# Cappucciyes/ViT-With-OpenCL

Measured on AMD Instinct MI355X. Metric: images/sec ViT-B/16 224x224 bs512, higher is better.
Workload: dtype f32

## Files before the change

### include/kernelHandler.h

```cpp
#ifndef VIT_HIP_KERNELHANDLER_H
#define VIT_HIP_KERNELHANDLER_H

#include <stddef.h>
#include <stdio.h>
#include <stdlib.h>

#ifdef __cplusplus
extern "C" {
#endif

typedef void *vh_stream_t;
typedef void *vh_event_t;

#define VH_CHECK(err)                                                          \
    do {                                                                       \
        int vh_check_err_ = (err);                                             \
        if (vh_check_err_ != 0) {                                              \
            printf("[%s:%d] HIP error %d: %s\n", __FILE__, __LINE__,           \
                   vh_check_err_, vh_last_error());                            \
            exit(EXIT_FAILURE);                                                \
        }                                                                      \
    } while (0)

int vh_device_count(void);
int vh_init(int device);
const char *vh_last_error(void);
int vh_set_error(int code, const char *message);
const char *vh_device_name(void);
int vh_set_device(int device);

int vh_stream_create(vh_stream_t *out);
int vh_stream_destroy(vh_stream_t s);
int vh_stream_sync(vh_stream_t s);
int vh_device_sync(void);

int vh_event_create(vh_event_t *out);
int vh_event_destroy(vh_event_t e);
int vh_event_record(vh_event_t e, vh_stream_t s);
int vh_stream_wait_event(vh_stream_t s, vh_event_t e);
int vh_event_sync(vh_event_t e);
int vh_event_elapsed_ms(float *ms, vh_event_t start, vh_event_t stop);

int vh_malloc(void **out, size_t bytes);
int vh_free(void *p);
int vh_host_alloc(void **out, size_t bytes);
int vh_host_free(void *p);
int vh_memset(void *dst, int value, size_t bytes, vh_stream_t s);
int vh_h2d(void *dst, const void *src, size_t bytes, vh_stream_t s);
int vh_d2h(void *dst, const void *src, size_t bytes, vh_stream_t s);
int vh_d2d(void *dst, const void *src, size_t bytes, vh_stream_t s);


int vh_launch_patch_embed(vh_stream_t s, const float *images, const float *conv_w,
                          const float *conv_b, const float *cls_token, const float *pos_embed,
                          float *tokens, int n_images, int in_chans, int img_size,
                          int patch_size, int embed_dim);

size_t vh_patch_embed_workspace(int n_images, int in_chans, int img_size, int patch_size, int embed_dim);
int vh_launch_patch_embed_ws(vh_stream_t s, const float *images, const float *conv_w,
                             const float *conv_b, const float *cls_token, const float *pos_embed,
                             float *tokens, int n_images, int in_chans, int img_size,
                             int patch_size, int embed_dim, void *workspace, size_t workspace_bytes);

int vh_patch_planes_k(int in_chans, int patch_size);
int vh_launch_conv_weight_planes(vh_stream_t s, const float *conv_w, void *planes, int embed_dim, int in_chans, int patch_size);
int vh_launch_conv_weight_planes_parts(vh_stream_t s, const float *conv_w, void *planes, int embed_dim, int in_chans, int patch_size,
                                       int parts);
int vh_launch_patch_embed_planes3(vh_stream_t s, const float *images, const void *conv_w_planes3, const float *conv_b,
                                  const float *cls_token, const float *pos_embed, float *tokens, int n_images, int in_chans,
                                  int img_size, int patch_size, int embed_dim, void *workspace, size_t workspace_bytes);
int vh_launch_patch_embed_planes(vh_stream_t s, const float *images, const void *conv_w_planes, const float *conv_b,
                                 const float *cls_token, const float *pos_embed, float *tokens, int n_images,
                                 int in_chans, int img_size, int patch_size, int embed_dim, void *workspace,
                                 size_t workspace_bytes);

int vh_launch_layer_norm(vh_stream_t s, const float *input, const float *weight,
                         const float *bias, float *output, int rows, int embed_dim,
                         long in_row_stride, long out_row_stride, double eps);

int vh_launch_linear(vh_stream_t s, float *output, const float *weight, const float *input,
                     const float *bias, int rowA, int colA, int colB, int doGelu,
                     const float *residual);
enum { VH_FP32_SPLIT3 = 0, VH_FP32_NATIVE = 1 };
int vh_launch_linear_math(vh_stream_t s, float *output, const float *weight, const float *input, const float *bias,
                          int rowA, int colA, int colB, int doGelu, const float *residual, int fp32_math);
int vh_launch_patch_embed_ws_math(vh_stream_t s, const float *images, const float *conv_w, const float *conv_b,
                                  const float *cls_token, const float *pos_embed, float *tokens, int n_images, int in_chans,
                                  int img_size, int patch_size, int embed_dim, void *workspace, size_t workspace_bytes,
                                  int fp32_math);

int vh_launch_split3_planes(vh_stream_t s, const float *weight, void *planes, int rows, int cols);
int vh_launch_linear_w3(vh_stream_t s, float *output, const void *weight_planes, const float *input,
                        const float *bias, int rowA, int colA, int colB, int doGelu,
                        const float *residual);

int vh_launch_split3_rows(vh_stream_t s, const float *input, void *planes, int rows, int cols);
int vh_launch_merge3_rows(vh_stream_t s, const void *planes, float *output, int rows, int cols);
int vh_launch_split_rows(vh_stream_t s, const float *input, void *planes, int rows, int cols, int parts);
int vh_launch_merge_rows(vh_stream_t s, const void *planes, float *output, int rows, int cols, int parts);
int vh_layer_norm_planes_max_embed(int parts);
int vh_launch_layer_norm_planes(vh_stream_t s, const float *input, const float *weight, const float *bias,
                                void *out_planes, int parts, int rows, int embed_dim, long in_row_stride, double eps);
int vh_launch_attention_planes_bf16(vh_stream_t s, const float *qkv, void *out_planes, int n_images, int tokens,
                                    int embed_dim, int num_heads);
int vh_launch_linear_planes(vh_stream_t s, void *output, int output_planes, const void *weight_planes,
                            const void *input_planes, int parts, const float *bias, int rowA, int colA, int colB,
                            int doGelu, const float *residual);
int vh_launch_layer_norm_p3(vh_stream_t s, const float *input, const float *weight, const float *bias,
                            void *out_planes, int rows, int embed_dim, long in_row_stride, double eps);
int vh_launch_attention_p3(vh_stream_t s, const float *qkv, void *out_planes, int n_images, int tokens,
                           int embed_dim, int num_heads);
int vh_launch_attention_planes(vh_stream_t s, const void *qkv_planes, void *out_planes, int n_images, int tokens,
                               int embed_dim, int num_heads);
int vh_launch_attention_planes_f16(vh_stream_t s, const void *qkv_planes_f16, void *output, int output_planes,
                                   int n_images, int tokens, int embed_dim, int num_heads);
int vh_launch_attention_planes_f16_hd80(vh_stream_t s, const void *qkv_planes_f16, float *output, int n_images,
                                        int tokens, int embed_dim, int num_heads);
int vh_launch_attention_planes_f16_hd80_operand(vh_stream_t s, const void *qkv_planes_f16, void *output, void *out_scales,
                                                int output_kind, int n_images, int tokens, int embed_dim, int num_heads);
int vh_launch_attention_long(vh_stream_t s, const void *qkv_planes, int parts, float *output, int n_images, int tokens,
                             int embed_dim, int num_heads);
int vh_launch_linear_p3(vh_stream_t s, void *output, int output_planes, const void *weight_planes,
                        const void *input_planes, const float *bias, int rowA, int colA, int colB,
                        int doGelu, const float *residual);

int vh_launch_split2h_planes(vh_stream_t s, const float *weight, void *planes, int rows, int cols, float scale);
int vh_launch_linear_h2(vh_stream_t s, float *output, const void *weight_planes, float weight_scale,
                        const float *input, const float *bias, int rowA, int colA, int colB,
                        int doGelu, const float *residual);
int vh_launch_attention_h2(vh_stream_t s, const float *qkv, float *output, int n_images, int tokens,
                           int embed_dim, int num_heads);

int vh_launch_attention(vh_stream_t s, const float *qkv, float *output, int n_images,
                        int tokens, int embed_dim, int num_heads);
enum { VH_ATTN_NATIVE = 0, VH_ATTN_FP16 = 1, VH_ATTN_FP16X2 = 2, VH_ATTN_SPLIT3 = 3 };
enum { VH_ATTN_AUTO = 0, VH_ATTN_STREAMING = 1 };
int vh_launch_attention_rows(vh_stream_t s, const float *qkv, void *output, int out_kind, int arith, int kernel, int n_images,
                             int tokens, int embed_dim, int num_heads);

int vh_launch_gather_rows(vh_stream_t s, const void *src, void *dst, int n_planes, int src_rows, int dst_rows,
                          int row_bytes, int row_stride);

int vh_launch_softmax(vh_stream_t s, const float *input, float *output, int rows, int length);

enum { VIT_TOPK_PROBS = 0, VIT_TOPK_LOGITS = 1 };
int vh_launch_topk(vh_stream_t s, const float *logits, int rows, int length, int k, int score_kind, int *labels, float *scores);

enum { VH_QKV_ROWS_F32 = 0, VH_QKV_PLANES3 = 1, VH_QKV_PLANES_F16 = 2 };
int vh_cls_attention_head_dim_ok(int head_dim);
int vh_launch_cls_attention(vh_stream_t s, const void *qkv, int qkv_form, int n_images, int tokens, int embed_dim,
                            int num_heads, int tap_index, int n_taps, float *heads, float *mean);

int vh_launch_attention_f16(vh_stream_t s, const float *qkv, float *output, int n_images,
                            int tokens, int embed_dim, int num_heads);

int vh_launch_absmax(vh_stream_t s, const float *input, size_t count, float *amax);

int vh_launch_quantize_mx_rows(vh_stream_t s, const float *input, void *values, void *scales, int rows, int cols);
int vh_launch_quantize_mx_act(vh_stream_t s, const float *input, void *values, void *scales, int rows, int cols);
size_t vh_mx_act_scale_bytes(int rows, int cols);
int vh_launch_layer_norm_mx(vh_stream_t s, const float *input, const float *weight, const float *bias,
                            void *out_values, void *out_scales, int rows, int embed_dim, long in_row_stride, double eps);
int vh_launch_linear_mx(vh_stream_t s, void *output, void *output_scales, const void *weight_values,
                        const void *weight_scales, const void *input_values, const void *input_scales,
                        const float *bias, int rowA, int colA, int colB, int doGelu, const float *residual);
int vh_launch_attention_planes_f16_mx(vh_stream_t s, const void *qkv_planes_f16, void *out_values, void *out_scales,
                                      int n_images, int tokens, int embed_dim, int num_heads);
int vh_launch_linear_mx_planes_f16(vh_stream_t s, void *output_planes_f16, const void *weight_values,
                                   const void *weight_scales, const void *input_values, const void *input_scales,
                                   const float *bias, int rowA, int colA, int colB);

int vh_launch_fold_gamma(vh_stream_t s, const float *weight, const float *gamma, float *out, int out_features, int in_features);
int vh_launch_fold_bias(vh_stream_t s, const float *weight, const float *beta, const float *bias, float *out, int out_features,
                        int in_features);
int vh_launch_colsum_operand(vh_stream_t s, const void *values, const void *scales, float *out, int out_features, int in_features);
int vh_launch_patch_embed_planes_norm(vh_stream_t s, const float *images, const void *conv_w_planes, const float *conv_b,
                                      const float *cls_token, const float *pos_embed, float *tokens, int n_images, int in_chans,
                                      int img_size, int patch_size, int embed_dim, void *workspace, size_t workspace_bytes,
                                      void *operand_out, void *operand_scales_out, float *row_stats_out);
int vh_launch_linear_planes_norm(vh_stream_t s, void *output, int output_planes, const void *weight_planes,
                                 const void *input_planes, const float *row_stats, const float *colsum, const float *bias_folded,
                                 double eps, int rowA, int colA, int colB, int doGelu);
int vh_launch_linear_planes_resid_norm(vh_stream_t s, float *output, const void *weight_planes, const void *input_planes,
                                       const float *bias, const float *residual, int rowA, int colA, int colB,
                                       void *operand_out, void *operand_scales_out, float *row_stats_out);
int vh_launch_colsum_planes3(vh_stream_t s, const void *planes3, float *out, int out_features, int in_features);
int vh_launch_patch_embed_planes3_norm(vh_stream_t s, const float *images, const void *conv_w_planes3, const float *conv_b,
                                       const float *cls_token, const float *pos_embed, float *tokens, int n_images, int in_chans,
                                       int img_size, int patch_size, int embed_dim, void *workspace, size_t workspace_bytes,
                                       void *operand_planes3_out, float *row_stats_out);
int vh_launch_linear_p3_norm(vh_stream_t s, void *output, int output_planes, const void *weight_planes3, const void *input_planes3,
                             const float *row_stats, const float *colsum, const float *bias_folded, double eps, int rowA, int colA,
                             int colB, int doGelu);
int vh_launch_linear_p3_resid_norm(vh_stream_t s, float *output, const void *weight_planes3, const void *input_planes3, const float *bias,
                                   const float *residual, int rowA, int colA, int colB, void *operand_planes3_out, float *row_stats_out);
int vh_launch_linear_mx_norm(vh_stream_t s, void *output, void *output_scales, int output_kind, const void *weight_values,
                             const void *weight_scales, const void *input_values, const void *input_scales, const float *row_stats,
                             const float *colsum, const float *bias_folded, double eps, int rowA, int colA, int colB, int doGelu);
int vh_launch_linear_mx_resid_norm(vh_stream_t s, float *output, const void *weight_values, const void *weight_scales,
                                   const void *input_values, const void *input_scales, const float *bias, const float *residual,
                                   int rowA, int colA, int colB, void *operand_values, void *operand_scales, float *row_stats_out);

int vh_launch_patch_embed_planes_u8(vh_stream_t s, const unsigned char *images, int layout, const float *scale, const float *bias,
                                    const void *conv_w_planes, const float *conv_b, const float *cls_token, const float *pos_embed,
                                    float *tokens, int n_images, int in_chans, int img_size, int patch_size, int embed_dim,
                                    void *workspace, size_t workspace_bytes, int parts, void *operand_out, void *operand_scales_out,
                                    float *row_stats_out);
int vh_launch_expand_u8(vh_stream_t s, const unsigned char *images, int layout, const float *scale, const float *bias, float *out,
                        int n_images, int in_chans, int img_size);

typedef struct vh_resize_desc
{
    const unsigned char *data;
    long row_stride;
    long plane_stride;
    int height, width;
    int row0;
    float x0, x1, y0, y1;
    int out_w, out_h;
    int left, top;
    int kx, ky;
    long coef_offset;
} vh_resize_desc;
#define VH_RESIZE_MAX_ROW_BYTES 3072
int vh_launch_resize_crop_u8(vh_stream_t s, const vh_resize_desc *desc, int n, int chans, int layout, int filter, int crop,
                             void *coef, size_t coef_bytes, unsigned char *out);

size_t vh_feature_readout_scratch(int n_images, int tokens, int embed_dim);
int vh_launch_feature_readout(vh_stream_t s, const float *x, const float *cls_rows, long cls_row_stride, const float *gamma,
                              const float *beta, double eps, int final_norm, int l2_normalize, int dtype, int token_layout,
                              int n_images, int tokens, int embed_dim, int tap_index, int n_taps, void *cls, void *pooled,
                              void *tokens_out, void *scratch, size_t scratch_bytes);

#ifdef __cplusplus
}
#endif

#endif
```

### vit-with-opencl_amd/csrc/ViT_hip.c

```c
#include "ViT_opencl.h"

#include <math.h>
#include <pthread.h>
#include <stddef.h>
#include <stdint.h>
#include <stdio.h>
#include <stdlib.h>
#include <string.h>
#include <time.h>

#define TRY(expr)                 \
    do {                          \
        int try_rc_ = (expr);     \
        if (try_rc_ != 0) {       \
            rc = try_rc_;         \
            goto fail;            \
        }                         \
    } while (0)

struct operand
{
    void *w;
    void *scales;
    float pair_scale;
    float *colsum, *bias_folded;
};

enum { SLAB_F32, SLAB_OPERAND, SLAB_CONV, SLAB_FOLD, N_SLABS };

enum { ATTN_STREAMING, ATTN_HD64, ATTN_HD80, ATTN_LONG };

enum { STREAMING_MAX_TOKENS = 512 };

enum { MAX_DEPTH = 256, MAX_TENSORS = 4 + 12 * MAX_DEPTH + 4 };

enum { DESC_RING = 8, RESIZE_MAX_SIDE = 16384 };

enum { FEAT_NONE, FEAT_DEVICE, FEAT_HOST };

struct staged
{
    void *dev, *pinned[2];
    char *host;
    size_t per_image;
};

struct vit_hip_ctx
{
    vit_config cfg;
    int device;
    int max_batch;
    int tokens;
    int n_tensors;
    vh_stream_t stream;

    int precision;
    int ln_fold;
    int use_p3;
    int cls_only_last;
    int attn_form;
    int fp32_native;
    int attn_rows_streaming;

    void *slab[N_SLABS];
    size_t slab_bytes[N_SLABS];
    float **w;
    struct operand *op;

    float *x;
    float *y;
    float *attn;
    float *qkv;
    float *hid;
    size_t ws_bytes;
    float *stats;
    float *cls;
    float *d_logits;
    float *d_probs;
    float *d_images[2];
    float *h_images[2];
    float *h_logits[2];
    float *h_probs[2];
    vh_stream_t copy_stream;
    vh_event_t up_done[2], comp_done[2], out_done[2];

    size_t crop_off;
    vh_resize_desc *h_desc[DESC_RING];
    vh_resize_desc *d_desc[DESC_RING];
    vh_event_t desc_done[DESC_RING];
    int desc_live[DESC_RING];
    int desc_next;

    struct feature_req
    {
        int form;
        vit_feature_spec spec;
        int layer[4];
        vit_feature_buffers out;
        struct staged st[2];
    } feat;

    struct topk_req
    {
        int form;
        vit_topk_spec spec;
        vit_topk_buffers out;
        struct staged st[2];
    } topk;

    struct attn_req
    {
        int form;
        vit_attn_spec spec;
        int layer[4];
        vit_attn_buffers out;
        struct staged st[2];
    } amap;
    const struct attn_req *attn_serving;

    vh_event_t *prof_ev;
    int *prof_class;
    int prof_cap;
    int prof_used;
    unsigned prof_mask;
};

static int prof_begin(vit_hip_ctx *ctx, vh_stream_t s, int op_class)
{
    if (!ctx->prof_ev || ctx->prof_used >= ctx->prof_cap)
        return -1;
    if (ctx->prof_mask && !(ctx->prof_mask & (1u << op_class)))
        return -1;
    const int slot = ctx->prof_used++;
    ctx->prof_class[slot] = op_class;
    vh_event_record(ctx->prof_ev[2 * slot], s);
    return slot;
}

static void prof_end(vit_hip_ctx *ctx, vh_stream_t s, int slot)
{
    if (slot >= 0)
        vh_event_record(ctx->prof_ev[2 * slot + 1], s);
}

#define OP(op_class, call)                                  \
    do {                                                    \
        const int op_slot_ = prof_begin(ctx, s, op_class);  \
        TRY(call);                                          \
        prof_end(ctx, s, op_slot_);                         \
    } while (0)

static void prof_release(vit_hip_ctx *ctx)
{
    if (ctx->prof_ev) {
        for (int i = 0; i < 2 * ctx->prof_cap; ++i)
            if (ctx->prof_ev[i])
                vh_event_destroy(ctx->prof_ev[i]);
        free(ctx->prof_ev);
        free(ctx->prof_class);
    }
    ctx->prof_ev = NULL;
    ctx->prof_class = NULL;
    ctx->prof_cap = ctx->prof_used = 0;
}

static double wall_seconds(void)
{
    struct timespec ts;
    clock_gettime(CLOCK_MONOTONIC, &ts);
    return (double)ts.tv_sec + 1e-9 * (double)ts.tv_nsec;
}

static size_t align_up(size_t v, size_t a) { return (v + a - 1) / a * a; }

const vit_config *vit_hip_config(const vit_hip_ctx *ctx) { return &ctx->cfg; }
int vit_hip_device(const vit_hip_ctx *ctx) { return ctx->device; }
float *vit_hip_logits_buffer(vit_hip_ctx *ctx) { return ctx->d_logits; }
vh_stream_t vit_hip_stream(const vit_hip_ctx *ctx) { return ctx->stream; }
int vit_hip_max_batch(const vit_hip_ctx *ctx) { return ctx->max_batch; }
const float *vit_hip_weight(const vit_hip_ctx *ctx, int idx)
{
    return (idx >= 0 && idx < ctx->n_tensors) ? ctx->w[idx] : NULL;
}

static int staged_alloc(const vit_hip_ctx *ctx, struct staged *st)
{
    const size_t bytes = (size_t)ctx->max_batch * st->per_image;
    int rc = vh_malloc(&st->dev, bytes);
    for (int slot = 0; slot < 2 && rc == 0; ++slot)
        rc = vh_host_alloc(&st->pinned[slot], bytes);
    return rc;
}

static void staged_release(struct staged *st)
{
    if (st->dev) vh_free(st->dev);
    st->dev = NULL;
    for (int slot = 0; slot < 2; ++slot) {
        if (st->pinned[slot]) vh_host_free(st->pinned[slot]);
        st->pinned[slot] = NULL;
    }
}

static int staged_d2h(const vit_hip_ctx *ctx, const struct staged *st, int slot, int m)
{
    return vh_d2h(st->pinned[slot], st->dev, (size_t)m * st->per_image, ctx->stream);
}

static void staged_scatter(const struct staged *st, int slot, int first, int m)
{
    memcpy(st->host + (size_t)first * st->per_image, st->pinned[slot], (size_t)m * st->per_image);
}

static void request_release(struct staged st[2])
{
    staged_release(&st[0]);
    staged_release(&st[1]);
}

void vit_hip_destroy(vit_hip_ctx *ctx)
{
    if (!ctx)
        return;
    if (ctx->stream) {
        vh_set_device(ctx->device);
        vh_stream_sync(ctx->stream);
    }
    prof_release(ctx);
    request_release(ctx->feat.st);
    request_release(ctx->topk.st);
    request_release(ctx->amap.st);
    for (int i = 0; i < N_SLABS; ++i)
        if (ctx->slab[i])
            vh_free(ctx->slab[i]);
    float *dev[] = {ctx->x, ctx->y, ctx->attn, ctx->qkv, ctx->hid, ctx->stats,
                    ctx->cls, ctx->d_logits, ctx->d_probs, ctx->d_images[0], ctx->d_images[1]};
    for (size_t i = 0; i < sizeof(dev) / sizeof(dev[0]); ++i)
        if (dev[i])
            vh_free(dev[i]);
    float *host[] = {ctx->h_images[0], ctx->h_images[1], ctx->h_logits[0], ctx->h_logits[1],
                     ctx->h_probs[0], ctx->h_probs[1]};
    for (size_t i = 0; i < sizeof(host) / sizeof(host[0]); ++i)
        if (host[i])
            vh_host_free(host[i]);
    for (int i = 0; i < DESC_RING; ++i) {
        if (ctx->d_desc[i]) vh_free(ctx->d_desc[i]);
        if (ctx->h_desc[i]) vh_host_free(ctx->h_desc[i]);
        if (ctx->desc_done[i]) vh_event_destroy(ctx->desc_done[i]);
    }
    for (int i = 0; i < 2; ++i) {
        if (ctx->up_done[i]) vh_event_destroy(ctx->up_done[i]);
        if (ctx->comp_done[i]) vh_event_destroy(ctx->comp_done[i]);
        if (ctx->out_done[i]) vh_event_destroy(ctx->out_done[i]);
    }
    if (ctx->copy_stream)
        vh_stream_destroy(ctx->copy_stream);
    if (ctx->stream)
        vh_stream_destroy(ctx->stream);
    free(ctx->w);
    free(ctx->op);
    free(ctx);
}

static const int BIG[4] = {2, 4, 8, 10};

static float **layer_tensors(const vit_hip_ctx *ctx, int l) { return ctx->w + 4 + 12 * l; }

static int operand_tensor(int m) { return 4 + 12 * (m / 4) + BIG[m % 4]; }

static void *place(void *slab, size_t *off, size_t bytes)
{
    void *p = slab ? (char *)slab + *off : NULL;
    *off += align_up(bytes, 256);
    return p;
}

static void layout_weights(vit_hip_ctx *ctx, size_t bytes[N_SLABS])
{
    const vit_config *cfg = &ctx->cfg;
    const int p = ctx->precision;
    const int f32_planes = p == VIT_PRECISION_F32 && cfg->embed_dim % 128 == 0 && cfg->mlp_hidden % 128 == 0;
    const size_t per = p == VIT_PRECISION_BF16_GEMM ? 2 : p == VIT_PRECISION_FP8_GEMM ? 1 : p == VIT_PRECISION_F32_FP16X2 ? 4
                     : f32_planes ? 6 : 0;
    const size_t conv_parts = (p == VIT_PRECISION_BF16_GEMM || p == VIT_PRECISION_FP8_GEMM) ? 1 : f32_planes ? 3 : 0;
    size_t off[N_SLABS] = {0};
    for (int i = 0; i < ctx->n_tensors; ++i)
        ctx->w[i] = (float *)place(ctx->slab[SLAB_F32], &off[SLAB_F32], vit_config_tensor_size(cfg, i) * sizeof(float));
    for (int m = 0; m < 4 * cfg->depth; ++m) {
        struct operand *o = &ctx->op[m];
        const size_t cnt = vit_config_tensor_size(cfg, operand_tensor(m));
        o->w = place(ctx->slab[SLAB_OPERAND], &off[SLAB_OPERAND], cnt * per);
        if (p == VIT_PRECISION_FP8_GEMM)
            o->scales = place(ctx->slab[SLAB_OPERAND], &off[SLAB_OPERAND], cnt / 32);
    }
    place(ctx->slab[SLAB_CONV], &off[SLAB_CONV],
          (size_t)vh_patch_planes_k(cfg->in_chans, cfg->patch_size) * (size_t)cfg->embed_dim * 2 * conv_parts);
    for (int m = 0; ctx->ln_fold && m < 4 * cfg->depth; m += 2) {
        const size_t nb = vit_config_tensor_size(cfg, operand_tensor(m) + 1) * sizeof(float);
        ctx->op[m].colsum = (float *)place(ctx->slab[SLAB_FOLD], &off[SLAB_FOLD], nb);
        ctx->op[m].bias_folded = (float *)place(ctx->slab[SLAB_FOLD], &off[SLAB_FOLD], nb);
    }
    memcpy(bytes, off, sizeof(off));
}

static int alloc_weights(vit_hip_ctx *ctx)
{
    int rc = 0;
    layout_weights(ctx, ctx->slab_bytes);
    for (int i = 0; i < N_SLABS; ++i)
        if (ctx->slab_bytes[i])
            TRY(vh_malloc(&ctx->slab[i], ctx->slab_bytes[i]));
    layout_weights(ctx, ctx->slab_bytes);
    return 0;
fail:
    return rc;
}

static int fill_weights(vit_hip_ctx *ctx, const Network *networks)
{
    int rc = 0;
    const vit_config *cfg = &ctx->cfg;
    const int p = ctx->precision;
    float *d_amax = NULL, *d_scaled = NULL;
    for (int i = 0; i < ctx->n_tensors; ++i)
        TRY(vh_h2d(ctx->w[i], networks[i].data, networks[i].size * sizeof(float), ctx->stream));
    if (p == VIT_PRECISION_F32_FP16X2)
        TRY(vh_malloc((void **)&d_amax, sizeof(float)));
    if (ctx->ln_fold)
        TRY(vh_malloc((void **)&d_scaled, (size_t)cfg->embed_dim * (size_t)(cfg->mlp_hidden > 3 * cfg->embed_dim ? cfg->mlp_hidden : 3 * cfg->embed_dim) * sizeof(float)));
    for (int m = 0; m < 4 * cfg->depth; ++m) {
        struct operand *o = &ctx->op[m];
        float **lw = layer_tensors(ctx, m / 4);
        const int idx = operand_tensor(m), k = m % 4, fold = o->colsum != NULL;
        const int out_f = (int)networks[idx + 1].size, in_f = (int)(networks[idx].size / networks[idx + 1].size);
        const float *src = ctx->w[idx];
        if (fold) {
            TRY(vh_launch_fold_gamma(ctx->stream, ctx->w[idx], lw[k == 0 ? 0 : 6], d_scaled, out_f, in_f));
            src = d_scaled;
        }
        switch (p) {
        case VIT_PRECISION_BF16_GEMM:
            TRY(vh_launch_split_rows(ctx->stream, src, o->w, out_f, in_f, 1));
            break;
        case VIT_PRECISION_FP8_GEMM:
            TRY(vh_launch_quantize_mx_rows(ctx->stream, src, o->w, o->scales, out_f, in_f));
            break;
        case VIT_PRECISION_F32:
            if (o->w)
                TRY(vh_launch_split3_planes(ctx->stream, src, o->w, out_f, in_f));
            break;
        case VIT_PRECISION_F32_FP16X2: {
            float amax = 0.0f;
            TRY(vh_memset(d_amax, 0, sizeof(float), ctx->stream));
            TRY(vh_launch_absmax(ctx->stream, src, networks[idx].size, d_amax));
            TRY(vh_d2h(&amax, d_amax, sizeof(float), ctx->stream));
            TRY(vh_stream_sync(ctx->stream));
            int e = 0;
            o->pair_scale = 1.0f;
            if (amax > 0.0f && amax < 3.0e38f) {
                (void)frexpf(amax, &e);
                o->pair_scale = ldexpf(1.0f, 14 - e);
            }
            TRY(vh_launch_split2h_planes(ctx->stream, src, o->w, out_f, in_f, o->pair_scale));
            break;
        }
        }
        if (fold) {
            TRY(p == VIT_PRECISION_F32 ? vh_launch_colsum_planes3(ctx->stream, o->w, o->colsum, out_f, in_f)
                                       : vh_launch_colsum_operand(ctx->stream, o->w, o->scales, o->colsum, out_f, in_f));
            TRY(vh_launch_fold_bias(ctx->stream, ctx->w[idx], lw[k == 0 ? 1 : 7], ctx->w[idx + 1], o->bias_folded, out_f, in_f));
        }
    }
    if (d_scaled)
        TRY(vh_stream_sync(ctx->stream));
    if (ctx->slab[SLAB_CONV])
        TRY(vh_launch_conv_weight_planes_parts(ctx->stream, ctx->w[1], ctx->slab[SLAB_CONV], cfg->embed_dim, cfg->in_chans,
                                               cfg->patch_size, p == VIT_PRECISION_F32 ? 3 : 1));
fail:
    if (d_amax)
        vh_free(d_amax);
    if (d_scaled)
        vh_free(d_scaled);
    return rc;
}

static int alloc_arena(vit_hip_ctx *ctx);

static int env_precision(void)
{
    const char *env = getenv("VIT_HIP_PRECISION");
    return (env && env[0] == 'b') ? VIT_PRECISION_BF16_GEMM
         : (env && strncmp(env, "fp16x2", 6) == 0) ? VIT_PRECISION_F32_FP16X2
         : (env && strncmp(env, "fp8", 3) == 0) ? VIT_PRECISION_FP8_GEMM : VIT_PRECISION_F32;
}

int vit_hip_create(vit_hip_ctx **out, const vit_config *cfg, const Network *networks,
                   int n_tensors, int device, int max_batch)
{
    return vit_hip_create_ex(out, cfg, networks, n_tensors, device, max_batch, env_precision());
}

int vit_hip_precision(const vit_hip_ctx *ctx) { return ctx->precision; }
int vit_hip_ln_fold(const vit_hip_ctx *ctx) { return ctx ? ctx->ln_fold : 0; }

static int ctx_new(vit_hip_ctx **out, const vit_config *cfg, int n_tensors, int device, int max_batch, int precision, int ln_fold)
{
    if (!out)
        return 1;
    *out = NULL;
    if (!cfg || max_batch <= 0)
        return 1;
    if (precision != VIT_PRECISION_F32 && precision != VIT_PRECISION_BF16_GEMM && precision != VIT_PRECISION_FP8_GEMM &&
        precision != VIT_PRECISION_F32_FP16X2)
        return 1;
    if (precision == VIT_PRECISION_F32_FP16X2 && (cfg->embed_dim % 128 != 0 || cfg->mlp_hidden % 128 != 0))
        return 2;
    if (precision == VIT_PRECISION_FP8_GEMM && (cfg->embed_dim % 256 != 0 || cfg->mlp_hidden % 256 != 0))
        return 2;
    if (precision == VIT_PRECISION_BF16_GEMM && (cfg->embed_dim % 128 != 0 || cfg->mlp_hidden % 128 != 0))
        return 2;
    if (cfg->depth <= 0 || cfg->embed_dim <= 0 || cfg->num_heads <= 0 || cfg->patch_size <= 0 || cfg->img_size <= 0 ||
        cfg->in_chans <= 0 || cfg->num_classes <= 0 || cfg->mlp_hidden <= 0)
        return 2;
    if (cfg->depth > MAX_DEPTH || cfg->embed_dim > 16384 || cfg->mlp_hidden > 65536 || cfg->img_size > 4096 || cfg->in_chans > 64 ||
        cfg->num_classes > (1 << 20) || cfg->num_heads > 1024 || max_batch > (1 << 20))
        return 2;
    if (n_tensors != vit_config_num_tensors(cfg))
        return 2;
    if (cfg->embed_dim % cfg->num_heads != 0 || cfg->img_size % cfg->patch_size != 0)
        return 2;

    const int E = cfg->embed_dim, F = cfg->mlp_hidden, H = cfg->num_heads, T = vit_config_tokens(cfg);
    const int reduced = precision == VIT_PRECISION_BF16_GEMM || precision == VIT_PRECISION_FP8_GEMM;
    const char *env_p3 = getenv("VIT_HIP_P3"), *env_native = getenv("VIT_HIP_GEMM_FP32");
    const int fp32_native = env_native && env_native[0] == 'n';
    const int planes_wanted = !(env_p3 && env_p3[0] == '0') && !fp32_native;
    const int use_p3 = precision == VIT_PRECISION_F32 && E % 128 == 0 && F % 128 == 0 && planes_wanted &&
                       (size_t)max_batch * (size_t)T * 64 <= 0xffffffffull;
    const int fold_fits = E % 128 == 0 && E / 128 <= 16 && (reduced || (precision == VIT_PRECISION_F32 && F % 128 == 0));
    if (ln_fold < 0) {
        const char *env = getenv("VIT_HIP_LN_FOLD");
        ln_fold = fold_fits && (reduced ? !(env && env[0] == '0') : env && env[0] == '1' && planes_wanted);
    }
    if (ln_fold && (!fold_fits || (precision == VIT_PRECISION_F32 && !use_p3)))
        return vh_set_error(2, "vit_hip_create: this shape, precision and batch cannot fold the LayerNorms (the fp32 path "
                               "needs the planes path)");
    if (use_p3 && !ln_fold && E > vh_layer_norm_planes_max_embed(3)) {
        char msg[320];
        snprintf(msg, sizeof msg, "vit_hip_create: embed_dim=%d: the fp32 planes path's LayerNorm (three-part planes, 96 bytes of "
                 "LDS per column) takes a LayerNorm width of at most %d",
                 E, vh_layer_norm_planes_max_embed(3));
        return vh_set_error(2, msg);
    }
    const char *env_ll = getenv("VIT_HIP_LAST_LAYER");
    const char *env_attn = getenv("VIT_HIP_ATTN");
    const int long_hd = E == 64 * H || E == 80 * H;
    const int long_wanted = T > STREAMING_MAX_TOKENS || (env_attn && strcmp(env_attn, "long") == 0);
    if (T > STREAMING_MAX_TOKENS && (precision == VIT_PRECISION_F32_FP16X2 || (precision == VIT_PRECISION_F32 && !use_p3) || !long_hd)) {
        char msg[320];
        snprintf(msg, sizeof msg, "vit_hip_create: %d tokens: above %d tokens attention runs on the planes paths (F32 with "
                 "embed_dim and mlp_hidden multiples of 128 and neither $VIT_HIP_P3=0 nor $VIT_HIP_GEMM_FP32=native, BF16_GEMM, "
                 "FP8_GEMM; not F32_FP16X2) with head_dim 64 or 80 (precision %d, head_dim %d)",
                 T, STREAMING_MAX_TOKENS, precision, E / H);
        return vh_set_error(2, msg);
    }

    vit_hip_ctx *ctx = (vit_hip_ctx *)calloc(1, sizeof(*ctx));
    if (!ctx)
        return 4;
    ctx->cfg = *cfg;
    ctx->device = device;
    ctx->max_batch = max_batch;
    ctx->tokens = T;
    ctx->n_tensors = n_tensors;
    ctx->precision = precision;
    ctx->ln_fold = ln_fold ? 1 : 0;
    ctx->use_p3 = use_p3;
    ctx->cls_only_last = use_p3 && !ln_fold && env_ll && strcmp(env_ll, "cls") == 0;
    ctx->attn_form = !(use_p3 || reduced) ? ATTN_STREAMING
              : (long_wanted && long_hd) ? ATTN_LONG
              : (E == 64 * H && T <= 208) ? ATTN_HD64
              : (reduced && E == 80 * H && T <= 272) ? ATTN_HD80 : ATTN_STREAMING;
    ctx->fp32_native = fp32_native;
    ctx->attn_rows_streaming = env_attn && env_attn[0] == 't';
    ctx->w = (float **)calloc((size_t)n_tensors, sizeof(float *));
    ctx->op = (struct operand *)calloc((size_t)4 * cfg->depth, sizeof(struct operand));
    if (!ctx->w || !ctx->op) {
        free(ctx->w);
        free(ctx->op);
        free(ctx);
        return 4;
    }
    *out = ctx;
    return 0;
}

int vit_hip_create_ex(vit_hip_ctx **out, const vit_config *cfg, const Network *networks,
                      int n_tensors, int device, int max_batch, int precision)
{
    int rc = 0;
    if (!out)
        return 1;
    *out = NULL;
    if (!networks || !cfg)
        return 1;
    if (n_tensors != vit_config_num_tensors(cfg))
        return 2;
    for (int i = 0; i < n_tensors; ++i)
        if (!networks[i].data || networks[i].size != vit_config_tensor_size(cfg, i)) {
            fprintf(stderr, "vit_hip_create: tensor %d has %zu elements, expected %zu\n", i,
                    networks[i].data ? networks[i].size : (size_t)0, vit_config_tensor_size(cfg, i));
            return 3;
        }
    vit_hip_ctx *ctx = NULL;
    if ((rc = ctx_new(&ctx, cfg, n_tensors, device, max_batch, precision, -1)) != 0)
        return rc;
    TRY(vh_init(device));
    TRY(vh_stream_create(&ctx->stream));
    TRY(alloc_weights(ctx));
    TRY(fill_weights(ctx, networks));
    TRY(alloc_arena(ctx));
    *out = ctx;
    return 0;
fail:
    vit_hip_destroy(ctx);
    return rc;
}

#define VIT_PLANES_LAYOUT_VERSION 2

struct planes_header
{
    char magic[8];
    unsigned header_bytes;
    int precision, n_tensors;
    int cfg_ints[8];
    double eps;
    unsigned long long w_slab_bytes, planes_bytes, wconv16_bytes, scale_floats;
    unsigned long long fold_bytes;
    int ln_fold, layout_version;
    unsigned long long checksum;
};

static unsigned long long planes_hash(unsigned long long h, const void *data, size_t bytes)
{
    const unsigned long long *w = (const unsigned long long *)data;
    for (size_t i = 0; i < bytes / 8; ++i)
        h = (h ^ w[i]) * 0x100000001b3ull;
    const unsigned char *t = (const unsigned char *)data + (bytes & ~(size_t)7);
    for (size_t i = 0; i < (bytes & 7); ++i)
        h = (h ^ t[i]) * 0x100000001b3ull;
    return h;
}
#define PLANES_HASH_SEED 0xcbf29ce484222325ull

static int copy_file_and_device(vit_hip_ctx *ctx, FILE *fp, void *dev, size_t bytes, int to_file, unsigned long long *hash)
{
    enum { CHUNK = 64 << 20 };
    int rc = 0;
    void *host = NULL;
    if (bytes == 0)
        return 0;
    TRY(vh_host_alloc(&host, bytes < CHUNK ? bytes : (size_t)CHUNK));
    for (size_t off = 0; off < bytes && rc == 0; off += CHUNK) {
        const size_t n = bytes - off < CHUNK ? bytes - off : (size_t)CHUNK;
        if (to_file) {
            if ((rc = vh_d2h(host, (char *)dev + off, n, ctx->stream)) != 0 || (rc = vh_stream_sync(ctx->stream)) != 0)
                break;
            *hash = planes_hash(*hash, host, n);
            if (fwrite(host, 1, n, fp) != n)
                rc = vh_set_error(120, "vit_hip_export_planes: short write");
        } else {
            if (fread(host, 1, n, fp) != n) {
                rc = vh_set_error(121, "vit_hip_create_from_planes: file is shorter than its header says");
                break;
            }
            *hash = planes_hash(*hash, host, n);
            if ((rc = vh_h2d((char *)dev + off, host, n, ctx->stream)) != 0 || (rc = vh_stream_sync(ctx->stream)) != 0)
                break;
        }
    }
fail:
    if (host)
        vh_host_free(host);
    return rc;
}

static void pair_scales(const vit_hip_ctx *ctx, float scales[MAX_TENSORS])
{
    memset(scales, 0, sizeof(float) * (size_t)ctx->n_tensors);
    for (int m = 0; m < 4 * ctx->cfg.depth; ++m)
        scales[operand_tensor(m)] = ctx->op[m].pair_scale;
}

int vit_hip_export_planes(vit_hip_ctx *ctx, const char *path)
{
    int rc = 0;
    if (!ctx || !path)
        return vh_set_error(1, "vit_hip_export_planes: null argument");
    TRY(vh_set_device(ctx->device));
    const size_t plen = strlen(path);
    char *tmp = (char *)malloc(plen + 5);
    if (!tmp)
        return vh_set_error(4, "vit_hip_export_planes: out of host memory");
    memcpy(tmp, path, plen);
    memcpy(tmp + plen, ".tmp", 5);
    FILE *fp = fopen(tmp, "wb");
    if (!fp) {
        free(tmp);
        return vh_set_error(122, "vit_hip_export_planes: cannot open the file for writing");
    }
    struct planes_header h;
    memset(&h, 0, sizeof(h));
    memcpy(h.magic, "VITPLN02", 8);
    h.header_bytes = (unsigned)sizeof(h);
    h.precision = ctx->precision;
    h.n_tensors = ctx->n_tensors;
    const vit_config *c = &ctx->cfg;
    const int ints[8] = {c->img_size, c->patch_size, c->in_chans, c->num_classes, c->embed_dim, c->depth, c->num_heads, c->mlp_hidden};
    memcpy(h.cfg_ints, ints, sizeof(ints));
    h.eps = c->eps;
    h.w_slab_bytes = ctx->slab_bytes[SLAB_F32];
    h.planes_bytes = ctx->slab_bytes[SLAB_OPERAND];
    h.wconv16_bytes = ctx->slab_bytes[SLAB_CONV];
    h.fold_bytes = ctx->slab_bytes[SLAB_FOLD];
    h.ln_fold = ctx->ln_fold;
    h.layout_version = VIT_PLANES_LAYOUT_VERSION;
    h.scale_floats = (unsigned long long)ctx->n_tensors;
    float scales[MAX_TENSORS];
    pair_scales(ctx, scales);
    unsigned long long hash = planes_hash(PLANES_HASH_SEED, scales, sizeof(float) * (size_t)ctx->n_tensors);
    if (fwrite(&h, sizeof(h), 1, fp) != 1 || fwrite(scales, sizeof(float), (size_t)ctx->n_tensors, fp) != (size_t)ctx->n_tensors)
        rc = vh_set_error(120, "vit_hip_export_planes: short write");
    for (int i = 0; i < N_SLABS && rc == 0; ++i)
        rc = copy_file_and_device(ctx, fp, ctx->slab[i], ctx->slab_bytes[i], 1, &hash);
    if (rc == 0) {
        h.checksum = hash;
        if (fseek(fp, 0, SEEK_SET) != 0 || fwrite(&h, sizeof(h), 1, fp) != 1)
            rc = vh_set_error(120, "vit_hip_export_planes: short write");
    }
    if (fclose(fp) != 0 && rc == 0)
        rc = vh_set_error(120, "vit_hip_export_planes: short write");
    if (rc == 0 && rename(tmp, path) != 0)
        rc = vh_set_error(122, "vit_hip_export_planes: cannot move the finished file into place");
    if (rc != 0)
        remove(tmp);
    free(tmp);
    return rc;
fail:
    return rc;
}

int vit_hip_create_from_planes(vit_hip_ctx **out, const char *path, int device, int max_batch)
{
    int rc = 0;
    if (!out)
        return 1;
    *out = NULL;
    if (!path)
        return vh_set_error(1, "vit_hip_create_from_planes: null path");
    FILE *fp = fopen(path, "rb");
    if (!fp)
        return vh_set_error(123, "vit_hip_create_from_planes: cannot open the file");
    struct planes_header h;
    vit_hip_ctx *ctx = NULL;
    if (fread(&h, sizeof(h), 1, fp) != 1 || memcmp(h.magic, "VITPLN02", 8) != 0 || h.header_bytes != sizeof(h) ||
        h.layout_version != VIT_PLANES_LAYOUT_VERSION) {
        fclose(fp);
        return vh_set_error(124, "vit_hip_create_from_planes: not a planes file of this library version (magic, header size or operand-layout version)");
    }
    vit_config cfg = {h.cfg_ints[0], h.cfg_ints[1], h.cfg_ints[2], h.cfg_ints[3], h.cfg_ints[4], h.cfg_ints[5], h.cfg_ints[6],
                      h.cfg_ints[7], h.eps};
    if (h.n_tensors <= 0 || h.n_tensors > MAX_TENSORS ||
        (rc = ctx_new(&ctx, &cfg, h.n_tensors, device, max_batch, h.precision, h.ln_fold ? 1 : 0)) != 0) {
        fclose(fp);
        return vh_set_error(rc ? rc : 2, "vit_hip_create_from_planes: the header's model shape or precision is not one this library takes");
    }
    size_t sizes[N_SLABS];
    layout_weights(ctx, sizes);
    if (h.w_slab_bytes != sizes[SLAB_F32] || h.planes_bytes != sizes[SLAB_OPERAND] || h.wconv16_bytes != sizes[SLAB_CONV] ||
        h.fold_bytes != sizes[SLAB_FOLD] || h.scale_floats != (unsigned long long)ctx->n_tensors) {
        rc = vh_set_error(125, "vit_hip_create_from_planes: slab sizes in the file do not match this library's layout");
        goto fail;
    }
    float scales[MAX_TENSORS];
    if (fread(scales, sizeof(float), (size_t)ctx->n_tensors, fp) != (size_t)ctx->n_tensors) {
        rc = vh_set_error(124, "vit_hip_create_from_planes: truncated header");
        goto fail;
    }
    unsigned long long hash = planes_hash(PLANES_HASH_SEED, scales, sizeof(float) * (size_t)ctx->n_tensors);
    for (int m = 0; m < 4 * cfg.depth; ++m)
        ctx->op[m].pair_scale = scales[operand_tensor(m)];
    TRY(vh_init(device));
    TRY(vh_stream_create(&ctx->stream));
    TRY(alloc_weights(ctx));
    for (int i = 0; i < N_SLABS; ++i)
        TRY(copy_file_and_device(ctx, fp, ctx->slab[i], ctx->slab_bytes[i], 0, &hash));
    if (hash != h.checksum) {
        rc = vh_set_error(126, "vit_hip_create_from_planes: payload checksum mismatch (corrupt file)");
        goto fail;
    }
    TRY(alloc_arena(ctx));
    fclose(fp);
    *out = ctx;
    return 0;
fail:
    fclose(fp);
    vit_hip_destroy(ctx);
    return rc;
}

static int planes_patch_embed(const vit_hip_ctx *ctx)
{
    return ctx->ln_fold || ctx->use_p3 || ctx->precision == VIT_PRECISION_BF16_GEMM || ctx->precision == VIT_PRECISION_FP8_GEMM;
}

static int span_taps(float in0, float in1, int out, int filter)
{
    const double scale = (double)(in1 - in0) / out;
    const double support = (filter == VIT_RESIZE_BICUBIC ? 2.0 : 1.0) * (scale < 1.0 ? 1.0 : scale);
    return (int)ceil(support) * 2 + 1;
}

static int resize_taps(int in, int out, int filter)
{
    return span_taps(0.0f, (float)in, out, filter);
}

static int resize_max_taps(int crop)
{
    return resize_taps(RESIZE_MAX_SIDE, crop > 1 ? crop - 1 : 1, VIT_RESIZE_BICUBIC);
}

static size_t resize_table_bytes(int crop, int kx, int ky)
{
    return align_up((size_t)crop * 16 + ((size_t)kx + ky) * crop * 4, 16);
}

static int alloc_arena(vit_hip_ctx *ctx)
{
    int rc = 0;
    const vit_config *cfg = &ctx->cfg;
    const int precision = ctx->precision, max_batch = ctx->max_batch;
    const size_t E = (size_t)cfg->embed_dim, F = (size_t)cfg->mlp_hidden, NC = (size_t)cfg->num_classes;
    const size_t rows = (size_t)max_batch * ctx->tokens;
    const size_t img = (size_t)cfg->in_chans * cfg->img_size * cfg->img_size;
    const size_t act = ctx->use_p3 ? 6 : sizeof(float);
    TRY(vh_malloc((void **)&ctx->x, rows * E * sizeof(float)));
    TRY(vh_malloc((void **)&ctx->y, rows * E * act));
    TRY(vh_malloc((void **)&ctx->attn, rows * E * act));
    {
        const size_t qkv_bytes = rows * 3 * E * act, expanded = planes_patch_embed(ctx) ? 0 : (size_t)max_batch * img * sizeof(float);
        ctx->crop_off = align_up(expanded, 256);
        const size_t crops = cfg->in_chans <= 4 ? ctx->crop_off + (size_t)max_batch * img : 0;
        size_t bytes = qkv_bytes > expanded ? qkv_bytes : expanded;
        bytes = bytes > crops ? bytes : crops;
        TRY(vh_malloc((void **)&ctx->qkv, bytes));
    }
    {
        size_t ws = vh_patch_embed_workspace(max_batch, cfg->in_chans, cfg->img_size, cfg->patch_size, cfg->embed_dim);
        if (ctx->slab[SLAB_CONV]) {
            const size_t grid = (size_t)(cfg->img_size / cfg->patch_size);
            const size_t planes = (size_t)max_batch * grid * grid * (size_t)vh_patch_planes_k(cfg->in_chans, cfg->patch_size) * 2 *
                                  (precision == VIT_PRECISION_F32 ? 3 : 1);
            ws = ws > planes ? ws : planes;
        }
        const size_t hid_bytes = rows * F * act;
        if (cfg->in_chans <= 4) {
            const size_t tables = (size_t)max_batch * resize_table_bytes(cfg->img_size, resize_max_taps(cfg->img_size),
                                                                          resize_max_taps(cfg->img_size));
            ws = ws > tables ? ws : tables;
        }
        ctx->ws_bytes = ws > hid_bytes ? ws : hid_bytes;
        TRY(vh_malloc((void **)&ctx->hid, ctx->ws_bytes));
    }
    if (ctx->ln_fold)
        TRY(vh_malloc((void **)&ctx->stats, rows * (E / 128) * 2 * sizeof(float)));
    TRY(vh_malloc((void **)&ctx->cls, (size_t)max_batch * E * sizeof(float)));
    TRY(vh_malloc((void **)&ctx->d_logits, (size_t)max_batch * NC * sizeof(float)));
    TRY(vh_malloc((void **)&ctx->d_probs, (size_t)max_batch * NC * sizeof(float)));
    TRY(vh_stream_create(&ctx->copy_stream));
    for (int i = 0; i < 2; ++i) {
        TRY(vh_malloc((void **)&ctx->d_images[i], (size_t)max_batch * img * sizeof(float)));
        TRY(vh_host_alloc((void **)&ctx->h_images[i], (size_t)max_batch * img * sizeof(float)));
        TRY(vh_host_alloc((void **)&ctx->h_logits[i], (size_t)max_batch * NC * sizeof(float)));
        TRY(vh_host_alloc((void **)&ctx->h_probs[i], (size_t)max_batch * NC * sizeof(float)));
        TRY(vh_event_create(&ctx->up_done[i]));
        TRY(vh_event_create(&ctx->comp_done[i]));
        TRY(vh_event_create(&ctx->out_done[i]));
    }
    for (int i = 0; i < DESC_RING; ++i) {
        TRY(vh_malloc((void **)&ctx->d_desc[i], (size_t)max_batch * sizeof(vh_resize_desc)));
        TRY(vh_host_alloc((void **)&ctx->h_desc[i], (size_t)max_batch * sizeof(vh_resize_desc)));
        TRY(vh_event_create(&ctx->desc_done[i]));
    }
    TRY(vh_stream_sync(ctx->stream));
    return 0;
fail:
    return rc;
}


static int fp32_math(const vit_hip_ctx *ctx) { return ctx->fp32_native ? VH_FP32_NATIVE : VH_FP32_SPLIT3; }

static int attention_rows(const vit_hip_ctx *ctx, vh_stream_t s, float *out, int arith, int n)
{
    return vh_launch_attention_rows(s, ctx->qkv, out, 0, arith, ctx->attn_rows_streaming ? VH_ATTN_STREAMING : VH_ATTN_AUTO, n,
                                    ctx->tokens, ctx->cfg.embed_dim, ctx->cfg.num_heads);
}

static int attention_tap(vit_hip_ctx *ctx, vh_stream_t s, int n, int l)
{
    int rc = 0;
    const struct attn_req *ar = ctx->attn_serving;
    if (!ar)
        return 0;
    const vit_config *c = &ctx->cfg;
    const int reduced = ctx->precision == VIT_PRECISION_BF16_GEMM || ctx->precision == VIT_PRECISION_FP8_GEMM;
    const int form = reduced ? (ctx->attn_form == ATTN_STREAMING ? VH_QKV_ROWS_F32 : VH_QKV_PLANES_F16)
                   : ctx->precision == VIT_PRECISION_F32 && ctx->use_p3 && (ctx->attn_form == ATTN_HD64 || ctx->attn_form == ATTN_LONG)
                       ? VH_QKV_PLANES3 : VH_QKV_ROWS_F32;
    for (int k = 0; k < ar->spec.n_taps; ++k)
        if (ar->layer[k] == l)
            OP(VIT_OP_ATTENTION, vh_launch_cls_attention(s, ctx->qkv, form, n, ctx->tokens, c->embed_dim, c->num_heads, k,
                                                         ar->spec.n_taps, ar->out.heads, ar->out.mean));
    return 0;
fail:
    return rc;
}

static int attention_reduced(vit_hip_ctx *ctx, vh_stream_t s, int n, char *attn_scales)
{
    int rc = 0;
    const vit_config *c = &ctx->cfg;
    const int E = c->embed_dim, T = ctx->tokens, H = c->num_heads, rows = n * T;
    if (ctx->attn_form == ATTN_HD64)
        OP(VIT_OP_ATTENTION, attn_scales ? vh_launch_attention_planes_f16_mx(s, ctx->qkv, ctx->attn, attn_scales, n, T, E, H)
                                         : vh_launch_attention_planes_f16(s, ctx->qkv, ctx->attn, 1, n, T, E, H));
    else if (ctx->attn_form == ATTN_HD80)
        OP(VIT_OP_ATTENTION, vh_launch_attention_planes_f16_hd80_operand(s, ctx->qkv, ctx->attn, attn_scales, attn_scales ? 2 : 1, n, T, E, H));
    else if (ctx->attn_form == ATTN_LONG)
        OP(VIT_OP_ATTENTION, (rc = vh_launch_attention_long(s, ctx->qkv, 1, ctx->hid, n, T, E, H)) != 0 ? rc :
                             attn_scales ? vh_launch_quantize_mx_act(s, ctx->hid, ctx->attn, attn_scales, rows, E)
                                         : vh_launch_split_rows(s, ctx->hid, ctx->attn, rows, E, 1));
    else
        OP(VIT_OP_ATTENTION, (rc = attention_rows(ctx, s, ctx->hid, VH_ATTN_FP16, n)) != 0 ? rc :
                             attn_scales ? vh_launch_quantize_mx_act(s, ctx->hid, ctx->attn, attn_scales, rows, E)
                                         : vh_launch_split_rows(s, ctx->hid, ctx->attn, rows, E, 1));
    return 0;
fail:
    return rc;
}

static int layer_fp8(vit_hip_ctx *ctx, vh_stream_t s, int n, int l)
{
    int rc = 0;
    const vit_config *c = &ctx->cfg;
    const int E = c->embed_dim, F = c->mlp_hidden, rows = n * ctx->tokens, fold = ctx->ln_fold, last = l == c->depth - 1;
    float **lw = layer_tensors(ctx, l);
    const struct operand *op = ctx->op + 4 * l;
    char *ys = (char *)ctx->y + align_up((size_t)rows * E, 256), *as_ = (char *)ctx->attn + align_up((size_t)rows * E, 256);
    char *hs = (char *)ctx->hid + align_up((size_t)rows * F, 256);
    const int kind = ctx->attn_form == ATTN_STREAMING ? 0 : 2;
    if (!fold)
        OP(VIT_OP_LAYER_NORM, vh_launch_layer_norm_mx(s, ctx->x, lw[0], lw[1], ctx->y, ys, rows, E, E, c->eps));
    OP(VIT_OP_QKV, fold ? vh_launch_linear_mx_norm(s, ctx->qkv, NULL, kind, op[0].w, op[0].scales, ctx->y, ys, ctx->stats, op[0].colsum, op[0].bias_folded, c->eps, rows, E, 3 * E, 0)
                 : kind ? vh_launch_linear_mx_planes_f16(s, ctx->qkv, op[0].w, op[0].scales, ctx->y, ys, lw[3], rows, E, 3 * E)
                        : vh_launch_linear_mx(s, ctx->qkv, NULL, op[0].w, op[0].scales, ctx->y, ys, lw[3], rows, E, 3 * E, 0, NULL));
    TRY(attention_tap(ctx, s, n, l));
    TRY(attention_reduced(ctx, s, n, as_));
    OP(VIT_OP_OUT_PROJ, fold ? vh_launch_linear_mx_resid_norm(s, ctx->x, op[1].w, op[1].scales, ctx->attn, as_, lw[5], ctx->x, rows, E, E, ctx->y, ys, ctx->stats)
                             : vh_launch_linear_mx(s, ctx->x, NULL, op[1].w, op[1].scales, ctx->attn, as_, lw[5], rows, E, E, 0, ctx->x));
    if (!fold)
        OP(VIT_OP_LAYER_NORM, vh_launch_layer_norm_mx(s, ctx->x, lw[6], lw[7], ctx->y, ys, rows, E, E, c->eps));
    OP(VIT_OP_FC1, fold ? vh_launch_linear_mx_norm(s, ctx->hid, hs, 1, op[2].w, op[2].scales, ctx->y, ys, ctx->stats, op[2].colsum, op[2].bias_folded, c->eps, rows, E, F, 1)
                        : vh_launch_linear_mx(s, ctx->hid, hs, op[2].w, op[2].scales, ctx->y, ys, lw[9], rows, E, F, 1, NULL));
    OP(VIT_OP_FC2, fold && !last ? vh_launch_linear_mx_resid_norm(s, ctx->x, op[3].w, op[3].scales, ctx->hid, hs, lw[11], ctx->x, rows, F, E, ctx->y, ys, ctx->stats)
                                 : vh_launch_linear_mx(s, ctx->x, NULL, op[3].w, op[3].scales, ctx->hid, hs, lw[11], rows, F, E, 0, ctx->x));
    return 0;
fail:
    return rc;
}

static int layer_bf16(vit_hip_ctx *ctx, vh_stream_t s, int n, int l)
{
    int rc = 0;
    const vit_config *c = &ctx->cfg;
    const int E = c->embed_dim, F = c->mlp_hidden, rows = n * ctx->tokens, fold = ctx->ln_fold, last = l == c->depth - 1;
    float **lw = layer_tensors(ctx, l);
    const struct operand *op = ctx->op + 4 * l;
    const int kind = ctx->attn_form == ATTN_STREAMING ? 0 : 2;
    if (!fold)
        OP(VIT_OP_LAYER_NORM, vh_launch_layer_norm_planes(s, ctx->x, lw[0], lw[1], ctx->y, 1, rows, E, E, c->eps));
    OP(VIT_OP_QKV, fold ? vh_launch_linear_planes_norm(s, ctx->qkv, kind, op[0].w, ctx->y, ctx->stats, op[0].colsum, op[0].bias_folded, c->eps, rows, E, 3 * E, 0)
                        : vh_launch_linear_planes(s, ctx->qkv, kind, op[0].w, ctx->y, 1, lw[3], rows, E, 3 * E, 0, NULL));
    TRY(attention_tap(ctx, s, n, l));
    TRY(attention_reduced(ctx, s, n, NULL));
    OP(VIT_OP_OUT_PROJ, fold ? vh_launch_linear_planes_resid_norm(s, ctx->x, op[1].w, ctx->attn, lw[5], ctx->x, rows, E, E, ctx->y, NULL, ctx->stats)
                             : vh_launch_linear_planes(s, ctx->x, 0, op[1].w, ctx->attn, 1, lw[5], rows, E, E, 0, ctx->x));
    if (!fold)
        OP(VIT_OP_LAYER_NORM, vh_launch_layer_norm_planes(s, ctx->x, lw[6], lw[7], ctx->y, 1, rows, E, E, c->eps));
    OP(VIT_OP_FC1, fold ? vh_launch_linear_planes_norm(s, ctx->hid, 1, op[2].w, ctx->y, ctx->stats, op[2].colsum, op[2].bias_folded, c->eps, rows, E, F, 1)
                        : vh_launch_linear_planes(s, ctx->hid, 1, op[2].w, ctx->y, 1, lw[9], rows, E, F, 1, NULL));
    OP(VIT_OP_FC2, fold && !last ? vh_launch_linear_planes_resid_norm(s, ctx->x, op[3].w, ctx->hid, lw[11], ctx->x, rows, F, E, ctx->y, NULL, ctx->stats)
                                 : vh_launch_linear_planes(s, ctx->x, 0, op[3].w, ctx->hid, 1, lw[11], rows, F, E, 0, ctx->x));
    return 0;
fail:
    return rc;
}

static int layer_fp16x2(vit_hip_ctx *ctx, vh_stream_t s, int n, int l)
{
    int rc = 0;
    const vit_config *c = &ctx->cfg;
    const int E = c->embed_dim, F = c->mlp_hidden, T = ctx->tokens, rows = n * T;
    float **lw = layer_tensors(ctx, l);
    const struct operand *op = ctx->op + 4 * l;
    OP(VIT_OP_LAYER_NORM, vh_launch_layer_norm(s, ctx->x, lw[0], lw[1], ctx->y, rows, E, E, E, c->eps));
    OP(VIT_OP_QKV, vh_launch_linear_h2(s, ctx->qkv, op[0].w, op[0].pair_scale, ctx->y, lw[3], rows, E, 3 * E, 0, NULL));
    TRY(attention_tap(ctx, s, n, l));
    OP(VIT_OP_ATTENTION, attention_rows(ctx, s, ctx->attn, VH_ATTN_FP16X2, n));
    OP(VIT_OP_OUT_PROJ, vh_launch_linear_h2(s, ctx->x, op[1].w, op[1].pair_scale, ctx->attn, lw[5], rows, E, E, 0, ctx->x));
    OP(VIT_OP_LAYER_NORM, vh_launch_layer_norm(s, ctx->x, lw[6], lw[7], ctx->y, rows, E, E, E, c->eps));
    OP(VIT_OP_FC1, vh_launch_linear_h2(s, ctx->hid, op[2].w, op[2].pair_scale, ctx->y, lw[9], rows, E, F, 1, NULL));
    OP(VIT_OP_FC2, vh_launch_linear_h2(s, ctx->x, op[3].w, op[3].pair_scale, ctx->hid, lw[11], rows, F, E, 0, ctx->x));
    return 0;
fail:
    return rc;
}

static int layer_f32_planes(vit_hip_ctx *ctx, vh_stream_t s, int n, int l, int *cls_rows)
{
    int rc = 0;
    const vit_config *c = &ctx->cfg;
    const int E = c->embed_dim, F = c->mlp_hidden, T = ctx->tokens, rows = n * T, fold = ctx->ln_fold, last = l == c->depth - 1;
    float **lw = layer_tensors(ctx, l);
    const struct operand *op = ctx->op + 4 * l;
    const int planes_attn = ctx->attn_form == ATTN_HD64 || ctx->attn_form == ATTN_LONG;
    if (!fold)
        OP(VIT_OP_LAYER_NORM, vh_launch_layer_norm_p3(s, ctx->x, lw[0], lw[1], ctx->y, rows, E, E, c->eps));
    OP(VIT_OP_QKV, fold ? vh_launch_linear_p3_norm(s, ctx->qkv, planes_attn, op[0].w, ctx->y, ctx->stats, op[0].colsum, op[0].bias_folded, c->eps, rows, E, 3 * E, 0)
                        : vh_launch_linear_p3(s, ctx->qkv, planes_attn, op[0].w, ctx->y, lw[3], rows, E, 3 * E, 0, NULL));
    TRY(attention_tap(ctx, s, n, l));
    OP(VIT_OP_ATTENTION, ctx->attn_form == ATTN_HD64 ? vh_launch_attention_planes(s, ctx->qkv, ctx->attn, n, T, E, c->num_heads)
                         : (rc = ctx->attn_form == ATTN_LONG ? vh_launch_attention_long(s, ctx->qkv, 3, ctx->hid, n, T, E, c->num_heads)
                                                             : attention_rows(ctx, s, ctx->hid, VH_ATTN_SPLIT3, n)) != 0 ? rc
                         : vh_launch_split3_rows(s, ctx->hid, ctx->attn, rows, E));
    if (last && ctx->cls_only_last && T >= 4) {
        char *scratch = (char *)ctx->qkv;
        float *x_cls = (float *)scratch;
        char *attn_cls = scratch + align_up((size_t)n * E * 4, 256);
        char *y_cls = attn_cls + align_up((size_t)n * E * 6, 256);
        char *hid_cls = y_cls + align_up((size_t)n * E * 6, 256);
        OP(VIT_OP_OUT_PROJ, (rc = vh_launch_gather_rows(s, ctx->attn, attn_cls, 3 * (E / 32), rows, n, 64, T)) != 0 ? rc :
                            (rc = vh_launch_gather_rows(s, ctx->x, x_cls, 1, rows, n, 4 * E, T)) != 0 ? rc :
                            vh_launch_linear_p3(s, x_cls, 0, op[1].w, attn_cls, lw[5], n, E, E, 0, x_cls));
        OP(VIT_OP_LAYER_NORM, vh_launch_layer_norm_p3(s, x_cls, lw[6], lw[7], y_cls, n, E, E, c->eps));
        OP(VIT_OP_FC1, vh_launch_linear_p3(s, hid_cls, 1, op[2].w, y_cls, lw[9], n, E, F, 1, NULL));
        OP(VIT_OP_FC2, vh_launch_linear_p3(s, x_cls, 0, op[3].w, hid_cls, lw[11], n, F, E, 0, x_cls));
        *cls_rows = 1;
        return 0;
    }
    OP(VIT_OP_OUT_PROJ, fold ? vh_launch_linear_p3_resid_norm(s, ctx->x, op[1].w, ctx->attn, lw[5], ctx->x, rows, E, E, ctx->y, ctx->stats)
                             : vh_launch_linear_p3(s, ctx->x, 0, op[1].w, ctx->attn, lw[5], rows, E, E, 0, ctx->x));
    if (!fold)
        OP(VIT_OP_LAYER_NORM, vh_launch_layer_norm_p3(s, ctx->x, lw[6], lw[7], ctx->y, rows, E, E, c->eps));
    OP(VIT_OP_FC1, fold ? vh_launch_linear_p3_norm(s, ctx->hid, 1, op[2].w, ctx->y, ctx->stats, op[2].colsum, op[2].bias_folded, c->eps, rows, E, F, 1)
                        : vh_launch_linear_p3(s, ctx->hid, 1, op[2].w, ctx->y, lw[9], rows, E, F, 1, NULL));
    OP(VIT_OP_FC2, fold && !last ? vh_launch_linear_p3_resid_norm(s, ctx->x, op[3].w, ctx->hid, lw[11], ctx->x, rows, F, E, ctx->y, ctx->stats)
                                 : vh_launch_linear_p3(s, ctx->x, 0, op[3].w, ctx->hid, lw[11], rows, F, E, 0, ctx->x));
    return 0;
fail:
    return rc;
}

static int layer_f32_rows(vit_hip_ctx *ctx, vh_stream_t s, int n, int l)
{
    int rc = 0;
    const vit_config *c = &ctx->cfg;
    const int E = c->embed_dim, F = c->mlp_hidden, T = ctx->tokens, rows = n * T;
    float **lw = layer_tensors(ctx, l);
    const struct operand *op = ctx->op + 4 * l;
    const int math = fp32_math(ctx);
    OP(VIT_OP_LAYER_NORM, vh_launch_layer_norm(s, ctx->x, lw[0], lw[1], ctx->y, rows, E, E, E, c->eps));
    OP(VIT_OP_QKV, op[0].w ? vh_launch_linear_w3(s, ctx->qkv, op[0].w, ctx->y, lw[3], rows, E, 3 * E, 0, NULL)
                         : vh_launch_linear_math(s, ctx->qkv, lw[2], ctx->y, lw[3], rows, E, 3 * E, 0, NULL, math));
    TRY(attention_tap(ctx, s, n, l));
    OP(VIT_OP_ATTENTION, attention_rows(ctx, s, ctx->attn, ctx->fp32_native ? VH_ATTN_NATIVE : VH_ATTN_SPLIT3, n));
    OP(VIT_OP_OUT_PROJ, op[1].w ? vh_launch_linear_w3(s, ctx->x, op[1].w, ctx->attn, lw[5], rows, E, E, 0, ctx->x)
                              : vh_launch_linear_math(s, ctx->x, lw[4], ctx->attn, lw[5], rows, E, E, 0, ctx->x, math));
    OP(VIT_OP_LAYER_NORM, vh_launch_layer_norm(s, ctx->x, lw[6], lw[7], ctx->y, rows, E, E, E, c->eps));
    OP(VIT_OP_FC1, op[2].w ? vh_launch_linear_w3(s, ctx->hid, op[2].w, ctx->y, lw[9], rows, E, F, 1, NULL)
                         : vh_launch_linear_math(s, ctx->hid, lw[8], ctx->y, lw[9], rows, E, F, 1, NULL, math));
    OP(VIT_OP_FC2, op[3].w ? vh_launch_linear_w3(s, ctx->x, op[3].w, ctx->hid, lw[11], rows, F, E, 0, ctx->x)
                          : vh_launch_linear_math(s, ctx->x, lw[10], ctx->hid, lw[11], rows, F, E, 0, ctx->x, math));
    return 0;
fail:
    return rc;
}

struct row_origin
{
    int row0;
    long plane_stride;
};

struct pixel_src
{
    const float *f32;
    const unsigned char *u8;
    int layout;
    const vit_pixel_norm *norm;
    const vit_image_u8 *resize;
    const vit_resize_crop *rc;
    const vit_box_u8 *boxes;
    int filter;
    const struct row_origin *origin;
};

static int resize_crop_launch(vit_hip_ctx *ctx, vh_stream_t s, const struct pixel_src *src, int n, unsigned char *out)
{
    int rc_ = 0;
    const vit_config *c = &ctx->cfg;
    const int layout = src->layout, filter = src->boxes ? src->filter : src->rc->filter;
    const int S = c->img_size, C = c->in_chans, slot = ctx->desc_next;
    ctx->desc_next = (slot + 1) % DESC_RING;
    if (ctx->desc_live[slot] && (rc_ = vh_event_sync(ctx->desc_done[slot])) != 0)
        return rc_;
    ctx->desc_live[slot] = 0;
    vh_resize_desc *d = ctx->h_desc[slot];
    size_t off = 0;
    for (int i = 0; i < n; ++i) {
        const int which = src->boxes ? src->boxes[i].image : i;
        const vit_image_u8 *im = &src->resize[which];
        vh_resize_desc *e = &d[i];
        e->data = im->data;
        e->row_stride = im->row_stride;
        e->plane_stride = src->origin ? src->origin[which].plane_stride : (long)im->height * im->row_stride;
        e->height = im->height;
        e->width = im->width;
        e->row0 = src->origin ? src->origin[which].row0 : 0;
        if (src->boxes) {
            const float *b = src->boxes[i].box;
            e->x0 = b[0], e->y0 = b[1], e->x1 = b[2], e->y1 = b[3];
            e->out_w = e->out_h = S;
            e->left = e->top = 0;
        } else {
            vit_resize_crop_geometry(im->height, im->width, src->rc, S, &e->out_h, &e->out_w, &e->top, &e->left);
            e->x0 = e->y0 = 0.0f;
            e->x1 = (float)im->width, e->y1 = (float)im->height;
        }
        e->kx = span_taps(e->x0, e->x1, e->out_w, filter);
        e->ky = span_taps(e->y0, e->y1, e->out_h, filter);
        e->coef_offset = (long)off;
        off += resize_table_bytes(S, e->kx, e->ky);
    }
    if (off > ctx->ws_bytes)
        return vh_set_error(1, "resize: coefficient tables exceed the scratch");
    if ((rc_ = vh_h2d(ctx->d_desc[slot], d, (size_t)n * sizeof(*d), s)) != 0)
        return rc_;
    rc_ = vh_launch_resize_crop_u8(s, ctx->d_desc[slot], n, C, layout, filter, S, ctx->hid, ctx->ws_bytes, out);
    const int rec = vh_event_record(ctx->desc_done[slot], s);
    ctx->desc_live[slot] = rec == 0;
    return rc_ ? rc_ : rec;
}

static int patch_embed_launches(vit_hip_ctx *ctx, vh_stream_t s, const struct pixel_src *src, int n)
{
    const vit_config *c = &ctx->cfg;
    const int E = c->embed_dim;
    float **w = ctx->w;
    void *conv = ctx->slab[SLAB_CONV];
    const int reduced = ctx->precision == VIT_PRECISION_BF16_GEMM || ctx->precision == VIT_PRECISION_FP8_GEMM;
    char *const y_scales = ctx->precision == VIT_PRECISION_FP8_GEMM ? (char *)ctx->y + align_up((size_t)n * ctx->tokens * E, 256) : NULL;
    if (src->u8 && planes_patch_embed(ctx))
        return vh_launch_patch_embed_planes_u8(s, src->u8, src->layout, src->norm->scale, src->norm->bias, conv, w[2], w[0], w[3],
                                               ctx->x, n, c->in_chans, c->img_size, c->patch_size, E, ctx->hid, ctx->ws_bytes,
                                               ctx->precision == VIT_PRECISION_F32 ? 3 : 1, ctx->ln_fold ? ctx->y : NULL,
                                               ctx->ln_fold ? y_scales : NULL, ctx->ln_fold ? ctx->stats : NULL);
    const float *images = src->f32;
    if (src->u8) {
        const int rc = vh_launch_expand_u8(s, src->u8, src->layout, src->norm->scale, src->norm->bias, ctx->qkv, n, c->in_chans,
                                           c->img_size);
        if (rc)
            return rc;
        images = ctx->qkv;
    }
    if (ctx->ln_fold && ctx->precision == VIT_PRECISION_F32)
        return vh_launch_patch_embed_planes3_norm(s, images, conv, w[2], w[0], w[3], ctx->x, n, c->in_chans, c->img_size,
                                                  c->patch_size, E, ctx->hid, ctx->ws_bytes, ctx->y, ctx->stats);
    if (ctx->ln_fold)
        return vh_launch_patch_embed_planes_norm(s, images, conv, w[2], w[0], w[3], ctx->x, n, c->in_chans, c->img_size,
                                                 c->patch_size, E, ctx->hid, ctx->ws_bytes, ctx->y, y_scales, ctx->stats);
    if (reduced)
        return vh_launch_patch_embed_planes(s, images, conv, w[2], w[0], w[3], ctx->x, n, c->in_chans, c->img_size, c->patch_size,
                                            E, ctx->hid, ctx->ws_bytes);
    if (ctx->use_p3)
        return vh_launch_patch_embed_planes3(s, images, conv, w[2], w[0], w[3], ctx->x, n, c->in_chans, c->img_size, c->patch_size,
                                             E, ctx->hid, ctx->ws_bytes);
    return vh_launch_patch_embed_ws_math(s, images, w[1], w[2], w[0], w[3], ctx->x, n, c->in_chans, c->img_size, c->patch_size, E,
                                         ctx->hid, ctx->ws_bytes, fp32_math(ctx));
}

static int feature_tap(vit_hip_ctx *ctx, vh_stream_t s, const struct feature_req *fr, int k, int n, int cls_rows)
{
    int rc = 0;
    const vit_config *c = &ctx->cfg;
    float **tw = ctx->w + 4 + 12 * c->depth;
    OP(VIT_OP_LAYER_NORM, vh_launch_feature_readout(s, ctx->x, cls_rows ? (const float *)ctx->qkv : NULL, c->embed_dim, tw[0], tw[1],
                                                    c->eps, fr->spec.final_norm, fr->spec.l2_normalize, fr->spec.dtype,
                                                    fr->spec.token_layout, n, ctx->tokens, c->embed_dim, k, fr->spec.n_taps,
                                                    fr->out.cls, fr->out.pooled, fr->out.tokens, ctx->hid, ctx->ws_bytes));
    return 0;
fail:
    return rc;
}

static int forward_device(vit_hip_ctx *ctx, const struct pixel_src *src, int n, float *d_logits, float *d_probs, vh_stream_t stream,
                          const struct feature_req *fr, const struct topk_req *tk, const struct attn_req *ar)
{
    int rc = 0;
    const int cls_only_saved = ctx->cls_only_last;
    ctx->attn_serving = ar;
    TRY(vh_set_device(ctx->device));
    const vit_config *c = &ctx->cfg;
    const int E = c->embed_dim, T = ctx->tokens, NC = c->num_classes;
    vh_stream_t s = stream ? stream : ctx->stream;

    struct pixel_src crops;
    if (src->resize) {
        unsigned char *out = (unsigned char *)ctx->qkv + ctx->crop_off;
        OP(VIT_OP_PATCH_EMBED, resize_crop_launch(ctx, s, src, n, out));
        crops = (struct pixel_src){NULL, out, VIT_PIXELS_HWC, src->norm, NULL, NULL};
        src = &crops;
    }
    OP(VIT_OP_PATCH_EMBED, patch_embed_launches(ctx, s, src, n));
    int cls_rows = 0;
    if (fr && fr->layer[fr->spec.n_taps - 1] == c->depth - 1 && (fr->out.pooled || fr->out.tokens))
        ctx->cls_only_last = 0;
    for (int l = 0, k = 0; l < c->depth; ++l) {
        switch (ctx->precision) {
        case VIT_PRECISION_FP8_GEMM: TRY(layer_fp8(ctx, s, n, l)); break;
        case VIT_PRECISION_BF16_GEMM: TRY(layer_bf16(ctx, s, n, l)); break;
        case VIT_PRECISION_F32_FP16X2: TRY(layer_fp16x2(ctx, s, n, l)); break;
        default:
            if (ctx->use_p3)
                TRY(layer_f32_planes(ctx, s, n, l, &cls_rows));
            else
                TRY(layer_f32_rows(ctx, s, n, l));
        }
        if (fr && k < fr->spec.n_taps && fr->layer[k] == l)
            TRY(feature_tap(ctx, s, fr, k++, n, cls_rows));
    }
    ctx->cls_only_last = cls_only_saved;
    ctx->attn_serving = NULL;

    float **tw = ctx->w + 4 + 12 * c->depth;
    float *logits = d_logits ? d_logits : ctx->d_logits;
    const float *final_x = cls_rows ? (const float *)ctx->qkv : ctx->x;
    const long final_stride = cls_rows ? (long)E : (long)T * E;
    OP(VIT_OP_LAYER_NORM, vh_launch_layer_norm(s, final_x, tw[0], tw[1], ctx->cls, n, E, final_stride, E, c->eps));
    OP(VIT_OP_HEAD, vh_launch_linear_math(s, logits, tw[2], ctx->cls, tw[3], n, E, NC, 0, NULL, fp32_math(ctx)));
    if (d_probs)
        OP(VIT_OP_SOFTMAX, vh_launch_softmax(s, logits, d_probs, n, NC));
    if (tk)
        OP(VIT_OP_SOFTMAX, vh_launch_topk(s, logits, n, NC, tk->spec.k, tk->spec.score_kind, tk->out.labels, tk->out.scores));
    return 0;
fail:
    ctx->cls_only_last = cls_only_saved;
    ctx->attn_serving = NULL;
    return rc;
}

static int armed_requests(vit_hip_ctx *ctx, const char *who, int form, const struct feature_req **fr, const struct topk_req **tk,
                          const struct attn_req **ar)
{
    static const char *const what[3] = {"feature", "top-k", "attention"}, *const setter[3] = {"features", "topk", "attention"};
    const int armed[3] = {ctx->feat.form, ctx->topk.form, ctx->amap.form};
    *fr = NULL;
    *tk = NULL;
    *ar = NULL;
    if (form == FEAT_NONE)
        return 0;
    for (int r = 0; r < 3; ++r)
        if (armed[r] != FEAT_NONE && armed[r] != form) {
            char msg[200];
            const char *const is = armed[r] == FEAT_HOST ? "host" : "device";
            snprintf(msg, sizeof msg, "%s: the context is armed for %s %s buffers (vit_hip_set_%s%s); disarm it or use the %s forms", who, is,
                     what[r], setter[r], armed[r] == FEAT_HOST ? "_host" : "", is);
            return vh_set_error(1, msg);
        }
    *fr = armed[0] == form ? &ctx->feat : NULL;
    *tk = armed[1] == form ? &ctx->topk : NULL;
    *ar = armed[2] == form ? &ctx->amap : NULL;
    return 0;
}

static int forward_device_armed(vit_hip_ctx *ctx, const char *who, const struct pixel_src *src, int n, float *d_logits, float *d_probs,
                                vh_stream_t stream)
{
    const struct feature_req *fr;
    const struct topk_req *tk;
    const struct attn_req *ar;
    if (armed_requests(ctx, who, FEAT_DEVICE, &fr, &tk, &ar))
        return 1;
    return forward_device(ctx, src, n, d_logits, d_probs, stream, fr, tk, ar);
}

int vit_hip_forward_device_plain(vit_hip_ctx *ctx, const float *d_images, int n, float *d_logits, float *d_probs, vh_stream_t stream)
{
    if (!ctx || !d_images || n <= 0 || n > ctx->max_batch)
        return 1;
    const struct pixel_src src = {d_images, NULL, 0, NULL};
    return forward_device(ctx, &src, n, d_logits, d_probs, stream, NULL, NULL, NULL);
}

int vit_hip_forward_device(vit_hip_ctx *ctx, const float *d_images, int n, float *d_logits,
                           float *d_probs, vh_stream_t stream)
{
    if (!ctx || !d_images || n <= 0 || n > ctx->max_batch)
        return 1;
    const struct pixel_src src = {d_images, NULL, 0, NULL};
    return forward_device_armed(ctx, "vit_hip_forward_device", &src, n, d_logits, d_probs, stream);
}

int vit_pixel_norm_from_mean_std(vit_pixel_norm *out, const float *mean, const float *std, int chans)
{
    if (!out || !mean || !std || chans < 1 || chans > 4)
        return vh_set_error(1, "vit_pixel_norm_from_mean_std: NULL argument, or chans not in 1..4");
    for (int ch = 0; ch < chans; ++ch)
        if (!(std[ch] > 0.0f) || !isfinite(std[ch]) || !isfinite(mean[ch]))
            return vh_set_error(1, "vit_pixel_norm_from_mean_std: std must be positive and finite, mean finite");
    memset(out, 0, sizeof(*out));
    for (int ch = 0; ch < chans; ++ch) {
        out->scale[ch] = (float)(1.0 / (255.0 * (double)std[ch]));
        out->bias[ch] = (float)(-(double)mean[ch] / (double)std[ch]);
    }
    return 0;
}

static int u8_args(const char *who, const vit_hip_ctx *ctx, const unsigned char *images, int n, int layout, const vit_pixel_norm *norm,
                   int device_ptr)
{
    char msg[200];
    const char *why = !ctx || !images || !norm ? "NULL context, images or norm"
                      : n <= 0 ? "n must be positive"
                      : device_ptr && n > ctx->max_batch ? "n exceeds the context's max_batch"
                      : layout != VIT_PIXELS_HWC && layout != VIT_PIXELS_CHW ? "layout must be VIT_PIXELS_HWC or VIT_PIXELS_CHW"
                      : ctx->cfg.in_chans > 4 ? "8-bit images take at most 4 channels"
                      : device_ptr && ((uintptr_t)images & 15) ? "device images must be 16-byte aligned"
                      : NULL;
    if (!why)
        return 0;
    snprintf(msg, sizeof msg, "%s: %s", who, why);
    return vh_set_error(1, msg);
}

int vit_hip_forward_device_u8(vit_hip_ctx *ctx, const unsigned char *d_images, int n, int layout,
                              const vit_pixel_norm *norm, float *d_logits, float *d_probs, vh_stream_t stream)
{
    if (u8_args("vit_hip_forward_device_u8", ctx, d_images, n, layout, norm, 1))
        return 1;
    const struct pixel_src src = {NULL, d_images, layout, norm};
    return forward_device_armed(ctx, "vit_hip_forward_device_u8", &src, n, d_logits, d_probs, stream);
}

int vit_resize_crop_geometry(int height, int width, const vit_resize_crop *rc, int crop, int *resized_h, int *resized_w, int *top,
                             int *left)
{
    char msg[200];
    const char *why = !rc || !resized_h || !resized_w || !top || !left ? "NULL argument"
                      : crop <= 0 ? "crop must be positive"
                      : height < 1 || width < 1 || height > RESIZE_MAX_SIDE || width > RESIZE_MAX_SIDE ? "height and width must be in 1..16384"
// ... 1177 lines not shown
```

### vit-with-opencl_amd/csrc/gemm_p3.hip

```cpp
#include "kernelHandler.h"
#include "vit_kernels.h"
#include "fp32_split.h"
#include "gemm_common.h"
#include "norm_fold.h"

#include <cstdint>
#include <cstdlib>

namespace {

typedef const __attribute__((address_space(1))) void *gptr_t;
typedef __attribute__((address_space(3))) void *lptr_t;
typedef const __attribute__((address_space(1))) char *gchar_t;
typedef const __attribute__((address_space(1))) f32x4 *gvec_t;

#ifndef P1_KG
#define P1_KG 2
#endif
enum { EPI_NONE = 0, EPI_GELU = 1, EPI_RESID = 2, EPI_PATCH = 3, EPI_NORM = 4, EPI_NORM_GELU = 5 };
enum { OUT_F32 = 0, OUT_PLANES = 1, OUT_PLANES_H = 2, OUT_F32_OPER = 3, OUT_F32_OPER_MX = 4 };

struct P3Params {
    const char *A;
    const char *W;
    const float *bias;
    const float *R;
    void *C;
    int row_begin, row_end;
    int N, K;
    int a_rows;
    int mtiles, ntiles;
    const float *pos;
    int np, tokens;
    const float *colsum;
    const float *stats;
    double eps;
    void *oper, *oper_scales;
    float *stats_out;
    int c_rows;
};

template <int NW, int BN, int EPI, int OUTK, int NPL = 3>
__global__ __launch_bounds__(64 * NW, 2) void gemm_p3_kernel(const P3Params p)
{
    constexpr int BM = 32 * NW, JT = BN / 16;
    constexpr int KG = NPL == 3 ? 1 : P1_KG;
    constexpr int RING = NPL == 3 ? 2 : 4;
    constexpr int F = KG * JT;
    constexpr int NT = NPL == 3 ? 6 : 1;
    constexpr int GROUP = NPL * BN * 64;
    constexpr int STAGE = KG * GROUP;
    constexpr int PW = KG * NPL * BN / 16 / NW;
    constexpr bool NORM = EPI == EPI_NORM || EPI == EPI_NORM_GELU;
    constexpr bool GELU = EPI == EPI_GELU || EPI == EPI_NORM_GELU;
    constexpr bool OPER = OUTK == OUT_F32_OPER || OUTK == OUT_F32_OPER_MX;
    static_assert(NPL == 1 || NPL == 3, "parts per value");
    static_assert(JT % 2 == 0 && (KG * NPL * BN / 16) % NW == 0 && F % RING == 0, "tile shape");
    static_assert(OUTK != OUT_F32_OPER_MX || NPL == 1, "an MX operand follows one-part operands only");
    static_assert(!OPER || (BN % 128 == 0 && (EPI == EPI_RESID || EPI == EPI_PATCH)), "operand producers: residual-stream epilogues");
    typedef bf16x8 frag_t;

    extern __shared__ __attribute__((aligned(16))) char smem[];

    const int tile = xcd_tile(blockIdx.x, p.mtiles * p.ntiles);
    const int m0 = p.row_begin + (tile / p.ntiles) * BM;
    const int n0 = (tile % p.ntiles) * BN;
    const int tid = threadIdx.x, lane = tid & 63;
    const int wave = __builtin_amdgcn_readfirstlane(tid >> 6);
    const int l15 = lane & 15, q = lane >> 4;

    unsigned aoff[2];
#pragma unroll
    for (int i = 0; i < 2; ++i)
        aoff[i] = (unsigned)min(m0 + 32 * wave + 16 * i + l15, p.row_end - 1) * 64u + 16u * q;
    const size_t a_plane = (size_t)p.a_rows * 64, w_plane = (size_t)p.N * 64;

    const unsigned wlane = (unsigned)(lane >> 2) * 64u + 16u * ((lane & 3) ^ swz64(lane >> 4));
    const gchar_t wtile = (gchar_t)p.W + (size_t)n0 * 64;

    constexpr bool NATURAL = OUTK == OUT_F32;
    const int rl = NATURAL ? l15 : 8 * (l15 >> 2) + (l15 & 3);
    const unsigned woff_e = (unsigned)rl * 64u + 16u * (q ^ swz64(NATURAL ? (l15 >> 2) : 2 * (l15 >> 2)));
    const unsigned woff_o = NATURAL ? woff_e + 16u * 64u
                                    : (unsigned)(rl + 4) * 64u + 16u * (q ^ swz64(2 * (l15 >> 2) + 1));
    auto frag_col = [&](int j) { return NATURAL ? 16 * j + 4 * q : 32 * (j >> 1) + 8 * q + 4 * (j & 1); };

    constexpr bool R_IN_ACC = EPI == EPI_RESID && NPL == 1;
    f32x4 acc[2][JT];
#pragma unroll
    for (int j = 0; j < JT; ++j) {
        const int col = n0 + frag_col(j);
        const f32x4 bv = NORM ? f32x4{0.0f, 0.0f, 0.0f, 0.0f} : *reinterpret_cast<const f32x4 *>(p.bias + col);
#pragma unroll
        for (int i = 0; i < 2; ++i) {
            acc[i][j] = bv;
            if (R_IN_ACC) {
                const int row = min(m0 + 32 * wave + 16 * i + l15, p.row_end - 1);
                acc[i][j] = *reinterpret_cast<const f32x4 *>(p.R + (size_t)row * p.N + col) + bv;
            }
        }
    }
    float n_rstd[2] = {1.0f, 1.0f}, n_shift[2] = {0.0f, 0.0f};
    if (NORM) {
#pragma unroll
        for (int i = 0; i < 2; ++i)
            row_norm_terms(p.stats, p.K >> 7, p.a_rows, min(m0 + 32 * wave + 16 * i + l15, p.row_end - 1), q, p.K, p.eps, n_rstd[i], n_shift[i]);
    }

    frag_t a0[KG][2][NPL], a1[KG][2][NPL], w[RING][NPL];

    auto load_a = [&](frag_t (&a)[KG][2][NPL], int kt) {
#pragma unroll
        for (int kg = 0; kg < KG; ++kg)
#pragma unroll
            for (int pl = 0; pl < NPL; ++pl) {
                gchar_t base = (gchar_t)p.A + (size_t)((kt * KG + kg) * NPL + pl) * a_plane;
                asm volatile("" : "+s"(base));
#pragma unroll
                for (int i = 0; i < 2; ++i)
                    a[kg][i][pl] = __builtin_bit_cast(frag_t, *reinterpret_cast<gvec_t>(base + aoff[i]));
            }
    };
    auto dma_w = [&](int stage, int kt) {
#pragma unroll
        for (int i = 0; i < PW; ++i) {
            const int pc = wave * PW + i, gp = pc / (BN / 16), rb = pc - gp * (BN / 16);
            gchar_t src = wtile + ((size_t)(kt * KG * NPL + gp) * w_plane + (size_t)rb * 1024);
            asm volatile("" : "+s"(src));
            __builtin_amdgcn_global_load_lds((gptr_t)(src + wlane), (lptr_t)(smem + stage * STAGE + pc * 1024), 16, 0, 0);
        }
    };
    auto read_w = [&](frag_t (&wf)[NPL], const char *stage, int f) {
        const int kg = f / JT, j = f % JT;
#pragma unroll
        for (int o = 0; o < NPL; ++o) {
            const int pl = (NPL - o) % NPL;
            wf[pl] = __builtin_bit_cast(frag_t, *reinterpret_cast<const f32x4 *>(
                                                    stage + kg * GROUP + ((j & 1) ? woff_o : woff_e) + (j >> 1) * 2048 + pl * (BN * 64)));
        }
    };
    auto mfma_frag = [&](const frag_t (&a)[KG][2][NPL], const frag_t (&wf)[NPL], int f) {
        const int kg = f / JT, j = f % JT;
#pragma unroll
        for (int t = 0; t < NT; ++t)
#pragma unroll
            for (int i = 0; i < 2; ++i)
                acc[i][j] = mfma_part(wf[term_w<NPL>(t)], a[kg][i][term_a<NPL>(t)], acc[i][j]);
    };
    auto interleave = [&]() {
#pragma unroll
        for (int r = 0; r < NPL; ++r) {
            __builtin_amdgcn_sched_group_barrier(0x100, 1, 0);
            __builtin_amdgcn_sched_group_barrier(0x008, 2, 0);
        }
        if (2 * NT > 2 * NPL)
            __builtin_amdgcn_sched_group_barrier(0x008, 2 * NT - 2 * NPL, 0);
        __builtin_amdgcn_sched_barrier(0);
    };

    const int nk = p.K / (32 * KG);
    auto step = [&](const frag_t (&au)[KG][2][NPL], frag_t (&al)[KG][2][NPL], int kt) {
        const char *cur = smem + (kt & 1) * STAGE, *nxt = smem + ((kt + 1) & 1) * STAGE;
        const bool more1 = kt + 1 < nk, more2 = kt + 2 < nk;
        load_a(al, more1 ? kt + 1 : kt);
#pragma unroll
        for (int f = 0; f <= F - RING; ++f) {
            read_w(w[(f + RING - 1) % RING], cur, f + RING - 1);
            mfma_frag(au, w[f % RING], f);
            interleave();
        }
        __syncthreads();
        if (more2)
            dma_w(kt & 1, kt + 2);
#pragma unroll
        for (int f = F - RING + 1; f < F; ++f) {
            if (more1)
                read_w(w[(f + RING - 1) % RING], nxt, f + RING - 1 - F);
            mfma_frag(au, w[f % RING], f);
            interleave();
        }
    };

    dma_w(0, 0);
    load_a(a0, 0);
    float *const ncol = reinterpret_cast<float *>(smem + 2 * STAGE);
    if (NORM && tid < 2 * BN / 4) {
        const int which = tid / (BN / 4), c4 = tid - which * (BN / 4);
        *reinterpret_cast<f32x4 *>(ncol + which * BN + 4 * c4) = *reinterpret_cast<const f32x4 *>((which ? p.bias : p.colsum) + n0 + 4 * c4);
    }
    __syncthreads();
    if (nk > 1)
        dma_w(1, 1);
#pragma unroll
    for (int f = 0; f < RING - 1; ++f)
        read_w(w[f], smem, f);
    for (int kt = 0; kt < nk; kt += 2) {
        step(a0, a1, kt);
        step(a1, a0, kt + 1);
    }

    int rows_[2];
    size_t orow_[2];
    const float *posrow_[2] = {nullptr, nullptr};
#pragma unroll
    for (int i = 0; i < 2; ++i) {
        rows_[i] = m0 + 32 * wave + 16 * i + l15;
        orow_[i] = (size_t)rows_[i];
        if (EPI == EPI_PATCH) {
            const int b = rows_[i] / p.np, pp = rows_[i] - b * p.np;
            orow_[i] = (size_t)b * p.tokens + 1 + pp;
            posrow_[i] = p.pos + (size_t)(1 + pp) * p.N;
        }
    }
    f32x2 psum[2] = {{0.0f, 0.0f}, {0.0f, 0.0f}}, psq[2] = {{0.0f, 0.0f}, {0.0f, 0.0f}};
    auto emit = [&](int i, int s, const f32x4 (&nb)[4]) {
        const int row = rows_[i];
        const int col = n0 + frag_col(2 * s), col_hi = n0 + frag_col(2 * s + 1);
        f32x4 lo = acc[i][2 * s], hi = acc[i][2 * s + 1];
        if (NORM) {
            const f32x4 r4 = {n_rstd[i], n_rstd[i], n_rstd[i], n_rstd[i]}, s4 = {n_shift[i], n_shift[i], n_shift[i], n_shift[i]};
            lo = __builtin_elementwise_fma(lo, r4, __builtin_elementwise_fma(nb[0], s4, nb[2]));
            hi = __builtin_elementwise_fma(hi, r4, __builtin_elementwise_fma(nb[1], s4, nb[3]));
        }
        if (EPI == EPI_PATCH) {
            lo = lo + *reinterpret_cast<const f32x4 *>(posrow_[i] + col);
            hi = hi + *reinterpret_cast<const f32x4 *>(posrow_[i] + col_hi);
        }
        if (GELU) {
            auto gelu2 = [](f32x2 v) { return (NPL == 1 && OUTK == OUT_PLANES) ? gelu_lowp2<0>(v) : gelu_exact2(v); };
            const f32x2 g0 = gelu2(f32x2{lo[0], lo[1]}), g1 = gelu2(f32x2{lo[2], lo[3]});
            const f32x2 g2 = gelu2(f32x2{hi[0], hi[1]}), g3 = gelu2(f32x2{hi[2], hi[3]});
            lo = f32x4{g0[0], g0[1], g1[0], g1[1]};
            hi = f32x4{g2[0], g2[1], g3[0], g3[1]};
        }
        if (EPI == EPI_RESID && !R_IN_ACC) {
            const float *rp = p.R + (size_t)row * p.N;
            lo = *reinterpret_cast<const f32x4 *>(rp + col) + lo;
            hi = *reinterpret_cast<const f32x4 *>(rp + col_hi) + hi;
        }
        if (OUTK == OUT_PLANES || OUTK == OUT_PLANES_H) {
            frag_t part[3];
            if (NPL == 3) {
                split8(lo, hi, part[0], part[1], part[2]);
            } else if (OUTK == OUT_PLANES_H) {
                half8 hv;
#pragma unroll
                for (int e = 0; e < 8; ++e)
                    hv[e] = (_Float16)(e < 4 ? lo[e] : hi[e - 4]);
                part[0] = __builtin_bit_cast(frag_t, hv);
            } else {
#pragma unroll
                for (int e = 0; e < 8; ++e)
                    part[0][e] = (__bf16)(e < 4 ? lo[e] : hi[e - 4]);
            }
            char *dst = static_cast<char *>(p.C) + ((size_t)((n0 >> 5) + s) * NPL * p.a_rows + row) * 64 + 16 * q;
#pragma unroll
            for (int pl = 0; pl < NPL; ++pl)
                *reinterpret_cast<f32x4 *>(dst + pl * a_plane) = __builtin_bit_cast(f32x4, part[pl]);
        } else {
            float *cp = static_cast<float *>(p.C) + orow_[i] * p.N;
            *reinterpret_cast<f32x4 *>(cp + col) = lo;
            *reinterpret_cast<f32x4 *>(cp + col_hi) = hi;
        }
        if (OPER) {
#pragma unroll
            for (int e = 0; e < 4; ++e) {
                const f32x2 v = e < 2 ? f32x2{lo[2 * e], lo[2 * e + 1]} : f32x2{hi[2 * e - 4], hi[2 * e - 3]};
                psum[i] = psum[i] + v;
                psq[i] = __builtin_elementwise_fma(v, v, psq[i]);
            }
            if (OUTK == OUT_F32_OPER) {
                frag_t part[3];
                if (NPL == 3) {
                    split8(lo, hi, part[0], part[1], part[2]);
                } else {
#pragma unroll
                    for (int e = 0; e < 8; ++e)
                        part[0][e] = (__bf16)(e < 4 ? lo[e] : hi[e - 4]);
                }
                char *dst = static_cast<char *>(p.oper) + ((size_t)((n0 >> 5) + s) * NPL * p.c_rows + orow_[i]) * 64 + 16 * q;
#pragma unroll
                for (int pl = 0; pl < NPL; ++pl)
                    *reinterpret_cast<f32x4 *>(dst + (size_t)pl * p.c_rows * 64) = __builtin_bit_cast(f32x4, part[pl]);
            } else {
                mx_store_block8(lo, hi, static_cast<char *>(p.oper), static_cast<unsigned char *>(p.oper_scales), p.c_rows, orow_[i],
                                n0 + 32 * s, q, true);
            }
            if ((s & 3) == 3) {
                float su = psum[i][0] + psum[i][1], sq2 = psq[i][0] + psq[i][1];
                su += __shfl_xor(su, 16);
                sq2 += __shfl_xor(sq2, 16);
                su += __shfl_xor(su, 32);
                sq2 += __shfl_xor(sq2, 32);
                if (q == 0)
                    *reinterpret_cast<f32x2 *>(p.stats_out + ((size_t)((n0 >> 7) + (s >> 2)) * p.c_rows + orow_[i]) * 2) = f32x2{su, sq2};
                psum[i] = psq[i] = f32x2{0.0f, 0.0f};
            }
        }
    };
    if (NORM) {
        auto column_terms = [&](int s, f32x4 (&nb)[4]) {
            const int c_lo = frag_col(2 * s), c_hi = frag_col(2 * s + 1);
            nb[0] = *reinterpret_cast<const f32x4 *>(ncol + c_lo);
            nb[1] = *reinterpret_cast<const f32x4 *>(ncol + c_hi);
            nb[2] = *reinterpret_cast<const f32x4 *>(ncol + BN + c_lo);
            nb[3] = *reinterpret_cast<const f32x4 *>(ncol + BN + c_hi);
        };
        if (m0 + BM <= p.row_end) {
#pragma unroll
            for (int s = 0; s < JT / 2; ++s) {
                f32x4 nb[4];
                column_terms(s, nb);
#pragma unroll
                for (int i = 0; i < 2; ++i)
                    emit(i, s, nb);
            }
        } else {
#pragma unroll
            for (int i = 0; i < 2; ++i) {
                if (rows_[i] >= p.row_end)
                    continue;
#pragma unroll
                for (int s = 0; s < JT / 2; ++s) {
                    f32x4 nb[4];
                    column_terms(s, nb);
                    emit(i, s, nb);
                }
            }
        }
    } else {
        const f32x4 none[4] = {};
#pragma unroll
        for (int i = 0; i < 2; ++i) {
            if (rows_[i] >= p.row_end)
                continue;
#pragma unroll
            for (int s = 0; s < JT / 2; ++s)
                emit(i, s, none);
        }
    }
}

template <int NW, int BN, int EPI, int OUTK, int NPL>
int launch_p3_tile(hipStream_t st, P3Params p)
{
    constexpr int LDS = 2 * (NPL == 3 ? 1 : P1_KG) * NPL * BN * 64 + ((EPI == EPI_NORM || EPI == EPI_NORM_GELU) ? 2 * BN * 4 : 0);
    VH_SET_LDS_ONCE((gemm_p3_kernel<NW, BN, EPI, OUTK, NPL>), LDS);
    p.mtiles = (p.row_end - p.row_begin + 32 * NW - 1) / (32 * NW);
    p.ntiles = p.N / BN;
    hipLaunchKernelGGL((gemm_p3_kernel<NW, BN, EPI, OUTK, NPL>), dim3(p.mtiles * p.ntiles), dim3(64 * NW), LDS, st, p);
    VH_LAUNCH_CHECK("gemm_p3_kernel");
    return 0;
}

template <int EPI, int OUTK, int NPL>
int launch_p3(hipStream_t st, const P3Params &p, int small_only)
{
    const int rows = p.row_end - p.row_begin;
    const int num_cus = vh_device_cus(vh_current_device());
    const int ntiles = p.N / 256, mtiles = (rows + 255) / 256;
    const long tiles = (long)mtiles * ntiles;
    if ((EPI == EPI_RESID || EPI == EPI_PATCH) && NPL == 1 && p.N % 256 == 0 && tiles >= num_cus)
        return launch_p3_tile<4, 256, EPI, OUTK, NPL>(st, p);
    if (p.N % 256 != 0 || small_only || 2 * tiles < 5 * (long)num_cus)
        return launch_p3_tile<4, 128, EPI, OUTK, NPL>(st, p);
    const long full = tiles / num_cus, rem = tiles % num_cus;
    const int rows_big = (int)(full * num_cus / ntiles) * 256;
    auto big_tiles = [&](const P3Params &q) { return launch_p3_tile<8, 256, EPI, OUTK, NPL>(st, q); };
    if (rem == 0 || 4 * rem > 3 * num_cus || rows_big <= 0 || rows_big >= rows)
        return big_tiles(p);
    P3Params big = p, rest = p;
    big.row_end = p.row_begin + rows_big;
    rest.row_begin = big.row_end;
    const int rc = big_tiles(big);
    return rc ? rc : launch_p3_tile<4, 128, EPI, OUTK, NPL>(st, rest);
}

template <int NPL>
__global__ void split_rows_kernel(const float *__restrict__ in, char *__restrict__ planes, int rows, int K)
{
    const size_t idx = (size_t)blockIdx.x * blockDim.x + threadIdx.x;
    const int k8 = K >> 3;
    if (idx >= (size_t)rows * k8)
        return;
    const int row = (int)(idx / k8), c8 = (int)(idx - (size_t)row * k8);
    const float *src = in + (size_t)row * K + 8 * c8;
    const f32x4 u = *reinterpret_cast<const f32x4 *>(src), v = *reinterpret_cast<const f32x4 *>(src + 4);
    bf16x8 part[3];
    if (NPL == 3) {
        split8(u, v, part[0], part[1], part[2]);
    } else {
#pragma unroll
        for (int e = 0; e < 8; ++e)
            part[0][e] = (__bf16)(e < 4 ? u[e] : v[e - 4]);
    }
    char *dst = planes + ((size_t)(c8 >> 2) * NPL * rows + row) * 64 + 16 * (c8 & 3);
#pragma unroll
    for (int pl = 0; pl < NPL; ++pl)
        *reinterpret_cast<f32x4 *>(dst + (size_t)pl * rows * 64) = __builtin_bit_cast(f32x4, part[pl]);
}

template <int NPL>
__global__ void merge_rows_kernel(const char *__restrict__ planes, float *__restrict__ out, int rows, int K)
{
    const size_t idx = (size_t)blockIdx.x * blockDim.x + threadIdx.x;
    const int k8 = K >> 3;
    if (idx >= (size_t)rows * k8)
        return;
    const int row = (int)(idx / k8), c8 = (int)(idx - (size_t)row * k8);
    const char *src = planes + ((size_t)(c8 >> 2) * NPL * rows + row) * 64 + 16 * (c8 & 3);
    bf16x8 part[3];
#pragma unroll
    for (int pl = 0; pl < NPL; ++pl)
        part[pl] = __builtin_bit_cast(bf16x8, *reinterpret_cast<const f32x4 *>(src + (size_t)pl * rows * 64));
    float *dst = out + (size_t)row * K + 8 * c8;
#pragma unroll
    for (int e = 0; e < 8; ++e)
        dst[e] = NPL == 3 ? ((float)part[0][e] + (float)part[1][e]) + (float)part[2][e] : (float)part[0][e];
}

int check_planes_args(const char *who, const void *a, const void *b, int rows, int cols, int parts)
{
    if (!a || !b || rows <= 0 || cols <= 0 || cols % 32 != 0 || (((uintptr_t)a | (uintptr_t)b) & 15) || (parts != 1 && parts != 3))
        return vh_fail(1, "%s: bad argument (cols %% 32 == 0, 16-byte aligned pointers, parts 1 or 3)", who);
    return 0;
}

}

extern "C" int vh_launch_split_rows(vh_stream_t s, const float *input, void *planes, int rows, int cols, int parts)
{
    if (int rc = check_planes_args("vh_launch_split_rows", input, planes, rows, cols, parts))
        return rc;
    const size_t threads = (size_t)rows * (cols / 8);
    const dim3 grid((unsigned)((threads + 255) / 256));
    if (parts == 3)
        hipLaunchKernelGGL(split_rows_kernel<3>, grid, dim3(256), 0, (hipStream_t)s, input, static_cast<char *>(planes), rows, cols);
    else
        hipLaunchKernelGGL(split_rows_kernel<1>, grid, dim3(256), 0, (hipStream_t)s, input, static_cast<char *>(planes), rows, cols);
    VH_LAUNCH_CHECK("split_rows_kernel");
    return 0;
}

extern "C" int vh_launch_merge_rows(vh_stream_t s, const void *planes, float *output, int rows, int cols, int parts)
{
    if (int rc = check_planes_args("vh_launch_merge_rows", planes, output, rows, cols, parts))
        return rc;
    const size_t threads = (size_t)rows * (cols / 8);
    const dim3 grid((unsigned)((threads + 255) / 256));
    if (parts == 3)
        hipLaunchKernelGGL(merge_rows_kernel<3>, grid, dim3(256), 0, (hipStream_t)s, static_cast<const char *>(planes), output, rows, cols);
    else
        hipLaunchKernelGGL(merge_rows_kernel<1>, grid, dim3(256), 0, (hipStream_t)s, static_cast<const char *>(planes), output, rows, cols);
    VH_LAUNCH_CHECK("merge_rows_kernel");
    return 0;
}

extern "C" int vh_launch_split3_rows(vh_stream_t s, const float *input, void *planes, int rows, int cols)
{
    return vh_launch_split_rows(s, input, planes, rows, cols, 3);
}

extern "C" int vh_launch_merge3_rows(vh_stream_t s, const void *planes, float *output, int rows, int cols)
{
    return vh_launch_merge_rows(s, planes, output, rows, cols, 3);
}

extern "C" int vh_launch_linear_planes(vh_stream_t s, void *output, int output_planes, const void *weight_planes,
                                       const void *input_planes, int parts, const float *bias, int rowA, int colA,
                                       int colB, int doGelu, const float *residual)
{
    if (!output || !weight_planes || !input_planes || !bias)
        return vh_fail(1, "vh_launch_linear_planes: null pointer argument");
    if (parts != 1 && parts != 3)
        return vh_fail(1, "vh_launch_linear_planes: parts must be 3 (exact fp32 split) or 1 (bf16 operands)");
    const int kstep = parts == 3 ? 64 : 64 * P1_KG;
    if (rowA <= 0 || colA <= 0 || colB <= 0 || colA % kstep != 0 || colB % 128 != 0)
        return vh_fail(1, "vh_launch_linear_planes: needs colA %% %d == 0 and colB %% 128 == 0 (%d,%d,%d)", kstep, rowA, colA, colB);
    if ((doGelu && residual) || (residual && output_planes) || output_planes < 0 || output_planes > 2 ||
        (output_planes == 2 && (parts != 1 || doGelu)))
        return vh_fail(1, "vh_launch_linear_planes: unsupported epilogue combination");
    if ((((uintptr_t)output | (uintptr_t)weight_planes | (uintptr_t)input_planes | (uintptr_t)bias | (uintptr_t)residual) & 15) != 0)
        return vh_fail(1, "vh_launch_linear_planes: pointers must be 16-byte aligned");
    if ((size_t)rowA * 64 > 0xffffffffull)
        return vh_fail(1, "vh_launch_linear_planes: rowA=%d too large", rowA);
    P3Params p = {};
    p.A = static_cast<const char *>(input_planes);
    p.W = static_cast<const char *>(weight_planes);
    p.bias = bias; p.R = residual; p.C = output;
    p.row_begin = 0; p.row_end = rowA; p.a_rows = rowA;
    p.N = colB; p.K = colA;
    hipStream_t st = (hipStream_t)s;
    const int small_only = residual && colA < 2048;
#define VH_P3_DISPATCH(NPL)                                                                                          \
    do {                                                                                                             \
        if (doGelu)                                                                                                  \
            return output_planes ? launch_p3<EPI_GELU, OUT_PLANES, NPL>(st, p, small_only)                           \
                                 : launch_p3<EPI_GELU, OUT_F32, NPL>(st, p, small_only);                             \
        if (residual)                                                                                                \
            return launch_p3<EPI_RESID, OUT_F32, NPL>(st, p, small_only);                                            \
        return output_planes ? launch_p3<EPI_NONE, OUT_PLANES, NPL>(st, p, small_only)                               \
                             : launch_p3<EPI_NONE, OUT_F32, NPL>(st, p, small_only);                                 \
    } while (0)
    if (parts == 3)
        VH_P3_DISPATCH(3);
    if (output_planes == 2)
        return launch_p3<EPI_NONE, OUT_PLANES_H, 1>(st, p, small_only);
    VH_P3_DISPATCH(1);
#undef VH_P3_DISPATCH
}

extern "C" int vh_launch_linear_p3(vh_stream_t s, void *output, int output_planes, const void *weight_planes,
                                   const void *input_planes, const float *bias, int rowA, int colA, int colB,
                                   int doGelu, const float *residual)
{
    return vh_launch_linear_planes(s, output, output_planes, weight_planes, input_planes, 3, bias, rowA, colA, colB,
                                   doGelu, residual);
}


static int linear_planes_norm(vh_stream_t s, void *output, int output_planes, const void *weight_planes, const void *input_planes,
                              const float *row_stats, const float *colsum, const float *bias_folded, double eps, int rowA, int colA,
                              int colB, int doGelu, int parts)
{
    if (!output || !weight_planes || !input_planes || !row_stats || !colsum || !bias_folded)
        return vh_fail(1, "vh_launch_linear_planes_norm: null pointer argument");
    const int kstep = parts == 3 ? 64 : 64 * P1_KG;
    if (rowA <= 0 || colA <= 0 || colB <= 0 || colA % kstep != 0 || colB % 128 != 0)
        return vh_fail(1, "vh_launch_linear_planes_norm: needs colA %% %d == 0 and colB %% 128 == 0 (%d,%d,%d)", kstep, rowA, colA, colB);
    if (output_planes < 0 || output_planes > 2 || (output_planes == 2 && (doGelu || parts == 3)) || (output_planes == 0 && doGelu))
        return vh_fail(1, "vh_launch_linear_planes_norm: unsupported epilogue combination");
    if (colA > 16 * 128 || colA % 128 != 0)
        return vh_fail(1, "vh_launch_linear_planes_norm: colA=%d: one partial sum per 128 columns, at most 16 per row", colA);
    if ((((uintptr_t)output | (uintptr_t)weight_planes | (uintptr_t)input_planes | (uintptr_t)colsum | (uintptr_t)bias_folded) & 15) != 0 ||
        ((uintptr_t)row_stats & 7) != 0)
        return vh_fail(1, "vh_launch_linear_planes_norm: pointers must be 16-byte aligned (row_stats: 8)");
    if ((size_t)rowA * 64 > 0xffffffffull)
        return vh_fail(1, "vh_launch_linear_planes_norm: rowA=%d too large", rowA);
    P3Params p = {};
    p.A = static_cast<const char *>(input_planes);
    p.W = static_cast<const char *>(weight_planes);
    p.bias = bias_folded; p.colsum = colsum; p.stats = row_stats; p.eps = eps; p.C = output;
    p.row_begin = 0; p.row_end = rowA; p.a_rows = rowA; p.c_rows = rowA;
    p.N = colB; p.K = colA;
    hipStream_t st = (hipStream_t)s;
    if (parts == 3) {
        if (doGelu)
            return launch_p3<EPI_NORM_GELU, OUT_PLANES, 3>(st, p, 0);
        return output_planes == 1 ? launch_p3<EPI_NORM, OUT_PLANES, 3>(st, p, 0) : launch_p3<EPI_NORM, OUT_F32, 3>(st, p, 0);
    }
    if (doGelu)
        return launch_p3<EPI_NORM_GELU, OUT_PLANES, 1>(st, p, 0);
    return output_planes == 2 ? launch_p3<EPI_NORM, OUT_PLANES_H, 1>(st, p, 0)
         : output_planes == 1 ? launch_p3<EPI_NORM, OUT_PLANES, 1>(st, p, 0) : launch_p3<EPI_NORM, OUT_F32, 1>(st, p, 0);
}

extern "C" int vh_launch_linear_planes_norm(vh_stream_t s, void *output, int output_planes, const void *weight_planes,
                                            const void *input_planes, const float *row_stats, const float *colsum,
                                            const float *bias_folded, double eps, int rowA, int colA, int colB, int doGelu)
{
    return linear_planes_norm(s, output, output_planes, weight_planes, input_planes, row_stats, colsum, bias_folded, eps, rowA, colA, colB,
                              doGelu, 1);
}

extern "C" int vh_launch_linear_p3_norm(vh_stream_t s, void *output, int output_planes, const void *weight_planes3,
                                        const void *input_planes3, const float *row_stats, const float *colsum,
                                        const float *bias_folded, double eps, int rowA, int colA, int colB, int doGelu)
{
    return linear_planes_norm(s, output, output_planes, weight_planes3, input_planes3, row_stats, colsum, bias_folded, eps, rowA, colA, colB,
                              doGelu, 3);
}

static int linear_planes_resid_norm(vh_stream_t s, float *output, const void *weight_planes, const void *input_planes, const float *bias,
                                    const float *residual, int rowA, int colA, int colB, void *operand_out, void *operand_scales_out,
                                    float *row_stats_out, int parts)
{
    if (!output || !weight_planes || !input_planes || !bias || !residual || !operand_out || !row_stats_out)
        return vh_fail(1, "vh_launch_linear_planes_resid_norm: null pointer argument");
    const int kstep = parts == 3 ? 64 : 64 * P1_KG;
    if (rowA <= 0 || colA <= 0 || colB <= 0 || colA % kstep != 0 || colB % 128 != 0 || (parts == 3 && operand_scales_out))
        return vh_fail(1, "vh_launch_linear_planes_resid_norm: needs colA %% %d == 0 and colB %% 128 == 0 (%d,%d,%d)", kstep, rowA, colA, colB);
    if ((((uintptr_t)output | (uintptr_t)weight_planes | (uintptr_t)input_planes | (uintptr_t)bias | (uintptr_t)residual | (uintptr_t)operand_out) & 15) != 0 ||
        ((uintptr_t)row_stats_out & 7) != 0)
        return vh_fail(1, "vh_launch_linear_planes_resid_norm: pointers must be 16-byte aligned (row_stats_out: 8)");
    if ((size_t)rowA * 128 > 0xffffffffull)
        return vh_fail(1, "vh_launch_linear_planes_resid_norm: rowA=%d too large", rowA);
    P3Params p = {};
    p.A = static_cast<const char *>(input_planes);
    p.W = static_cast<const char *>(weight_planes);
    p.bias = bias; p.R = residual; p.C = output;
    p.oper = operand_out; p.oper_scales = operand_scales_out; p.stats_out = row_stats_out;
    p.row_begin = 0; p.row_end = rowA; p.a_rows = rowA; p.c_rows = rowA;
    p.N = colB; p.K = colA;
    hipStream_t st = (hipStream_t)s;
    const int small_only = colA < 2048;
    if (parts == 3)
        return launch_p3<EPI_RESID, OUT_F32_OPER, 3>(st, p, small_only);
    return operand_scales_out ? launch_p3<EPI_RESID, OUT_F32_OPER_MX, 1>(st, p, small_only)
                              : launch_p3<EPI_RESID, OUT_F32_OPER, 1>(st, p, small_only);
}

extern "C" int vh_launch_linear_planes_resid_norm(vh_stream_t s, float *output, const void *weight_planes, const void *input_planes,
                                                  const float *bias, const float *residual, int rowA, int colA, int colB,
                                                  void *operand_out, void *operand_scales_out, float *row_stats_out)
{
    return linear_planes_resid_norm(s, output, weight_planes, input_planes, bias, residual, rowA, colA, colB, operand_out,
                                    operand_scales_out, row_stats_out, 1);
}

extern "C" int vh_launch_linear_p3_resid_norm(vh_stream_t s, float *output, const void *weight_planes3, const void *input_planes3,
                                              const float *bias, const float *residual, int rowA, int colA, int colB,
                                              void *operand_planes3_out, float *row_stats_out)
{
    return linear_planes_resid_norm(s, output, weight_planes3, input_planes3, bias, residual, rowA, colA, colB, operand_planes3_out,
                                    nullptr, row_stats_out, 3);
}

namespace {

template <int NPL>
__device__ __forceinline__ void store_parts8(char *planes, size_t kt, int rows, int m, int c, const f32x4 &u, const f32x4 &v)
{
    bf16x8 part[3];
    if (NPL == 3) {
        split8(u, v, part[0], part[1], part[2]);
    } else {
#pragma unroll
        for (int e = 0; e < 8; ++e)
            part[0][e] = (__bf16)(e < 4 ? u[e] : v[e - 4]);
    }
#pragma unroll
    for (int pl = 0; pl < NPL; ++pl)
        *reinterpret_cast<f32x4 *>(planes + ((kt * NPL + pl) * rows + m) * 64 + 16 * c) = __builtin_bit_cast(f32x4, part[pl]);
}

template <int MODE>
__global__ __launch_bounds__(256) void fold_rows_kernel(const float *__restrict__ w, const float *__restrict__ vec, const float *__restrict__ bias,
                                                        float *__restrict__ out, int N, int K)
{
    const int lane = threadIdx.x & 63, n = blockIdx.x * 4 + (threadIdx.x >> 6);
    if (n >= N)
        return;
    const float *row = w + (size_t)n * K;
    if (MODE == 0) {
        for (int k = lane; k < K; k += 64)
            out[(size_t)n * K + k] = row[k] * vec[k];
    } else {
        double acc = 0.0;
        for (int k = lane; k < K; k += 64)
            acc += (double)vec[k] * (double)row[k];
#pragma unroll
        for (int m = 32; m >= 1; m >>= 1)
            acc += __shfl_xor(acc, m);
        if (lane == 0)
            out[n] = (float)((double)bias[n] + acc);
    }
}

__global__ __launch_bounds__(256) void colsum_operand_kernel(const char *__restrict__ values, const unsigned char *__restrict__ scales,
                                                            float *__restrict__ out, int N, int K, int parts)
{
    const int lane = threadIdx.x & 63, n = blockIdx.x * 4 + (threadIdx.x >> 6);
    if (n >= N)
        return;
    double acc = 0.0;
    if (!scales) {
        for (int k = lane; k < K; k += 64)
            for (int pl = 0; pl < parts; ++pl)
                acc += (double)(float)*reinterpret_cast<const __bf16 *>(values + (((size_t)(k >> 5) * parts + pl) * N + n) * 64 + 2 * (k & 31));
    } else {
        for (int k = lane; k < K; k += 64) {
            const int ks = k >> 7, blk = (k >> 5) & 3;
            const unsigned sb = scales[((size_t)ks * 4 + 2 * (blk & 1) + (blk >> 1)) * N + n];
            const unsigned char byte = (unsigned char)values[((size_t)ks * N + n) * 128 + (k & 127)];
            const int e = (byte >> 3) & 15, m = byte & 7;
            float v = e ? ldexpf(1.0f + m * 0.125f, e - 7) : ldexpf(m * 0.125f, -6);
            if (byte & 0x80)
                v = -v;
            acc += (double)v * (double)ldexpf(1.0f, (int)sb - 127);
        }
    }
#pragma unroll
    for (int m = 32; m >= 1; m >>= 1)
        acc += __shfl_xor(acc, m);
    if (lane == 0)
        out[n] = (float)acc;
}

template <int NPL>
__global__ __launch_bounds__(64) void cls_rows_operand_kernel(const float *__restrict__ cls, const float *__restrict__ pos,
                                                             float *__restrict__ tokens, char *__restrict__ oper,
                                                             unsigned char *__restrict__ oper_scales, float *__restrict__ stats,
                                                             int n_images, int tokens_per_image, int E, int c_rows)
{
    const int lane = threadIdx.x, l15 = lane & 15, j = lane >> 4;
    const int g = blockIdx.y, b = blockIdx.x * 16 + l15;
    const bool live = b < n_images;
    const size_t row = (size_t)(live ? b : n_images - 1) * tokens_per_image;
    float su = 0.0f, sq = 0.0f;
#pragma unroll
    for (int s = 0; s < 4; ++s) {
        const int col = 128 * g + 32 * s + 8 * j;
        const f32x4 lo = *reinterpret_cast<const f32x4 *>(cls + col) + *reinterpret_cast<const f32x4 *>(pos + col);
        const f32x4 hi = *reinterpret_cast<const f32x4 *>(cls + col + 4) + *reinterpret_cast<const f32x4 *>(pos + col + 4);
#pragma unroll
        for (int e = 0; e < 8; ++e) {
            const float v = e < 4 ? lo[e] : hi[e - 4];
            su += v;
            sq += v * v;
        }
        if (live) {
            *reinterpret_cast<f32x4 *>(tokens + row * E + col) = lo;
            *reinterpret_cast<f32x4 *>(tokens + row * E + col + 4) = hi;
        }
        if (!oper_scales) {
            if (live)
                store_parts8<NPL>(oper, (size_t)(col >> 5), c_rows, (int)row, j, lo, hi);
        } else {
            mx_store_block8(lo, hi, oper, oper_scales, c_rows, row, 128 * g + 32 * s, j, live);
        }
    }
    su += __shfl_xor(su, 16);
    sq += __shfl_xor(sq, 16);
    su += __shfl_xor(su, 32);
    sq += __shfl_xor(sq, 32);
    if (j == 0 && live)
        *reinterpret_cast<f32x2 *>(stats + ((size_t)g * c_rows + row) * 2) = f32x2{su, sq};
}

}

extern "C" int vh_launch_fold_gamma(vh_stream_t s, const float *weight, const float *gamma, float *out, int out_features, int in_features)
{
    if (!weight || !gamma || !out || out_features <= 0 || in_features <= 0)
        return vh_fail(1, "vh_launch_fold_gamma: bad argument");
    hipLaunchKernelGGL(fold_rows_kernel<0>, dim3((out_features + 3) / 4), dim3(256), 0, (hipStream_t)s, weight, gamma, (const float *)nullptr, out,
                       out_features, in_features);
    VH_LAUNCH_CHECK("fold_rows_kernel");
    return 0;
}

extern "C" int vh_launch_fold_bias(vh_stream_t s, const float *weight, const float *beta, const float *bias, float *out, int out_features,
                                   int in_features)
{
    if (!weight || !beta || !bias || !out || out_features <= 0 || in_features <= 0)
        return vh_fail(1, "vh_launch_fold_bias: bad argument");
    hipLaunchKernelGGL(fold_rows_kernel<1>, dim3((out_features + 3) / 4), dim3(256), 0, (hipStream_t)s, weight, beta, bias, out, out_features,
                       in_features);
    VH_LAUNCH_CHECK("fold_rows_kernel");
    return 0;
}

static int colsum_operand(vh_stream_t s, const void *values, const void *scales, float *out, int out_features, int in_features, int parts)
{
    if (!values || !out || out_features <= 0 || in_features <= 0 || in_features % (scales ? 128 : 32) != 0)
        return vh_fail(1, "vh_launch_colsum_operand: bad argument");
    hipLaunchKernelGGL(colsum_operand_kernel, dim3((out_features + 3) / 4), dim3(256), 0, (hipStream_t)s, static_cast<const char *>(values),
                       static_cast<const unsigned char *>(scales), out, out_features, in_features, parts);
    VH_LAUNCH_CHECK("colsum_operand_kernel");
    return 0;
}

extern "C" int vh_launch_colsum_operand(vh_stream_t s, const void *values, const void *scales, float *out, int out_features, int in_features)
{
    return colsum_operand(s, values, scales, out, out_features, in_features, 1);
}

extern "C" int vh_launch_colsum_planes3(vh_stream_t s, const void *planes3, float *out, int out_features, int in_features)
{
    return colsum_operand(s, planes3, nullptr, out, out_features, in_features, 3);
}

namespace {

template <int NPL>
__global__ void im2row_planes_kernel(const float *__restrict__ images, char *__restrict__ planes, int n_rows, int chans,
                                     int img, int patch, int grid, int K, int Kp)
{
    const size_t i = (size_t)blockIdx.x * blockDim.x + threadIdx.x;
    if (i >= (size_t)n_rows * (Kp >> 3))
        return;
    const int c = (int)(i & 3);
    const size_t rm = i >> 2;
    const int kt = (int)(rm / n_rows), m = (int)(rm - (size_t)kt * n_rows);
    const int k0 = 32 * kt + 8 * c;
    const int np = grid * grid, b = m / np, pp = m - b * np, oh = pp / grid, ow = pp - oh * grid;
    const float *base = images + ((size_t)b * chans * img + (size_t)oh * patch) * img + (size_t)ow * patch;
    const int pp2 = patch * patch;
    f32x4 u = {0.0f, 0.0f, 0.0f, 0.0f}, v = u;
    if ((patch & 7) == 0 && (img & 3) == 0 && k0 + 8 <= K) {
        const int ic = k0 / pp2, rem = k0 - ic * pp2, kh = rem / patch, kw = rem - kh * patch;
        const float *src = base + ((size_t)ic * img + kh) * img + kw;
        u = *reinterpret_cast<const f32x4 *>(src);
        v = *reinterpret_cast<const f32x4 *>(src + 4);
    } else {
#pragma unroll
        for (int e = 0; e < 8; ++e) {
            const int k = k0 + e;
            float x = 0.0f;
            if (k < K) {
                const int ic = k / pp2, rem = k - ic * pp2, kh = rem / patch, kw = rem - kh * patch;
                x = base[((size_t)ic * img + kh) * img + kw];
            }
            if (e < 4)
                u[e] = x;
            else
                v[e - 4] = x;
        }
    }
    store_parts8<NPL>(planes, (size_t)kt, n_rows, m, c, u, v);
}

enum { PIXELS_HWC = 0, PIXELS_CHW = 1 };

struct PixelNorm
{
    float scale[4], bias[4];
};

__device__ __forceinline__ float pick4(const float (&a)[4], int i) { return i == 0 ? a[0] : i == 1 ? a[1] : i == 2 ? a[2] : a[3]; }
// ... 319 lines not shown
```

### vit-with-opencl_amd/csrc/rowops.hip

```cpp
#include "kernelHandler.h"
#include "vit_kernels.h"
#include "fp32_split.h"

namespace {

__device__ __forceinline__ float wave_max(float v)
{
#pragma unroll
    for (int m = 32; m >= 1; m >>= 1)
        v = fmaxf(v, __shfl_xor(v, m));
    return v;
}

template <int NV, int OUTK>
__global__ __launch_bounds__(256) void layernorm_kernel(const float *__restrict__ in,
                                                        const float *__restrict__ gamma,
                                                        const float *__restrict__ beta,
                                                        void *__restrict__ out, int rows, int E,
                                                        long in_stride, long out_stride, double eps,
                                                        float out_mult)
{
    const int lane = threadIdx.x & 63;
    const int row = blockIdx.x * 4 + (threadIdx.x >> 6);
    if (row >= rows)
        return;
    const int nvec = E >> 2;
    const f32x4 *src = reinterpret_cast<const f32x4 *>(in + (size_t)row * in_stride);
    f32x4 x[NV];
    float sum = 0.0f, sq = 0.0f;
#pragma unroll
    for (int c = 0; c < NV; ++c) {
        const int idx = c * 64 + lane;
        if (idx < nvec) {
            x[c] = src[idx];
#pragma unroll
            for (int e = 0; e < 4; ++e) {
                sum += x[c][e];
                sq += x[c][e] * x[c][e];
            }
        }
    }
    sum = wave_sum(sum);
    sq = wave_sum(sq);
    const float mean = sum / (float)E;
    const float var = sq / (float)E - mean * mean;
    const float inv_std = 1.0f / sqrtf((float)((double)var + eps));

    const f32x4 *g4 = reinterpret_cast<const f32x4 *>(gamma);
    const f32x4 *b4 = reinterpret_cast<const f32x4 *>(beta);
    f32x4 *dst = reinterpret_cast<f32x4 *>(static_cast<float *>(out) + (size_t)row * out_stride);
#pragma unroll
    for (int c = 0; c < NV; ++c) {
        const int idx = c * 64 + lane;
        if (idx < nvec) {
            const f32x4 g = g4[idx], bb = b4[idx];
            f32x4 y;
#pragma unroll
            for (int e = 0; e < 4; ++e)
                y[e] = (x[c][e] - mean) * inv_std * g[e] + bb[e];
            dst[idx] = y;
        }
    }
}

constexpr int LN3_ROWS = 16;

template <int NV, int NPL, bool FULL>
__global__ __launch_bounds__(64 * LN3_ROWS) void layernorm_p3_kernel(const float *__restrict__ in,
                                                                    const float *__restrict__ gamma,
                                                                    const float *__restrict__ beta,
                                                                    char *__restrict__ planes, int rows, int E,
                                                                    long in_stride, double eps)
{
    extern __shared__ __attribute__((aligned(16))) char ln_lds[];
    const int lane = threadIdx.x & 63, wave = threadIdx.x >> 6;
    const int nvec = E >> 2;
    const int ngroups = (rows + LN3_ROWS - 1) / LN3_ROWS, stride = gridDim.x;
    const f32x4 *g4 = reinterpret_cast<const f32x4 *>(gamma);
    const f32x4 *b4 = reinterpret_cast<const f32x4 *>(beta);

    auto load_rows = [&](f32x4 (&x)[NV], int group) {
        const int r = min(group * LN3_ROWS + wave, rows - 1);
        const f32x4 *src = reinterpret_cast<const f32x4 *>(in + (size_t)r * in_stride);
#pragma unroll
        for (int c = 0; c < NV; ++c)
            x[c] = src[FULL ? c * 64 + lane : min(c * 64 + lane, nvec - 1)];
    };
    auto process = [&](const f32x4 (&x)[NV], int group) {
        const int row0 = group * LN3_ROWS;
        float sum = 0.0f, sq = 0.0f;
#pragma unroll
        for (int c = 0; c < NV; ++c) {
            if (FULL || c * 64 + lane < nvec) {
#pragma unroll
                for (int e = 0; e < 4; ++e) {
                    sum += x[c][e];
                    sq += x[c][e] * x[c][e];
                }
            }
        }
        sum = wave_sum(sum);
        sq = wave_sum(sq);
        const float mean = sum / (float)E;
        const float var = sq / (float)E - mean * mean;
        const float inv_std = 1.0f / sqrtf((float)((double)var + eps));
#pragma unroll
        for (int c = 0; c < NV; ++c) {
            const int idx = c * 64 + lane;
            if (FULL || idx < nvec) {
                const f32x4 g = g4[idx], bb = b4[idx];
                f32x4 y;
#pragma unroll
                for (int e = 0; e < 4; ++e)
                    y[e] = (x[c][e] - mean) * inv_std * g[e] + bb[e];
                bf16x4 part[3];
                if (NPL == 3)
                    split4(y, part[0], part[1], part[2]);
                else
                    part[0] = bf16x4{(__bf16)y[0], (__bf16)y[1], (__bf16)y[2], (__bf16)y[3]};
                char *d = ln_lds + ((size_t)(idx >> 3) * NPL * LN3_ROWS + wave) * 64 + 8 * (idx & 7);
#pragma unroll
                for (int pl = 0; pl < NPL; ++pl)
                    *reinterpret_cast<bf16x4 *>(d + pl * LN3_ROWS * 64) = part[pl];
            }
        }
        lds_barrier();
        const int pieces = (E >> 5) * NPL;
        if (row0 + (lane >> 2) < rows)
            for (int pc = wave; pc < pieces; pc += LN3_ROWS)
                *reinterpret_cast<f32x4 *>(planes + ((size_t)pc * rows + row0) * 64 + 16 * lane) =
                    *reinterpret_cast<const f32x4 *>(ln_lds + pc * 1024 + 16 * lane);
        lds_barrier();
    };

    f32x4 xa[NV], xb[NV];
    int g0 = blockIdx.x;
    if (g0 >= ngroups)
        return;
    load_rows(xa, g0);
    for (;;) {
        const int g1 = g0 + stride;
        load_rows(xb, min(g1, ngroups - 1));
        process(xa, g0);
        if (g1 >= ngroups)
            break;
        const int g2 = g1 + stride;
        load_rows(xa, min(g2, ngroups - 1));
        process(xb, g1);
        if (g2 >= ngroups)
            break;
        g0 = g2;
    }
}

template <int NV, bool FULL>
__global__ __launch_bounds__(64 * LN3_ROWS) void layernorm_mx_kernel(const float *__restrict__ in, const float *__restrict__ gamma,
                                                                    const float *__restrict__ beta, char *__restrict__ values,
                                                                    unsigned char *__restrict__ scales, int rows, int E,
                                                                    long in_stride, double eps)
{
    extern __shared__ __attribute__((aligned(16))) char ln_lds[];
    const int lane = threadIdx.x & 63, wave = threadIdx.x >> 6;
    const int nvec = E >> 2, ksteps = E >> 7, sgroups = (ksteps + 3) >> 2;
    char *lds_scales = ln_lds + ksteps * LN3_ROWS * 128;
    for (int i = threadIdx.x; i < sgroups * 4 * LN3_ROWS; i += blockDim.x)
        reinterpret_cast<unsigned *>(lds_scales)[i] = 0u;
    __syncthreads();
    const int ngroups = (rows + LN3_ROWS - 1) / LN3_ROWS, stride = gridDim.x;
    const f32x4 *g4 = reinterpret_cast<const f32x4 *>(gamma);
    const f32x4 *b4 = reinterpret_cast<const f32x4 *>(beta);

    auto load_rows = [&](f32x4 (&x)[NV], int group) {
        const int r = min(group * LN3_ROWS + wave, rows - 1);
        const f32x4 *src = reinterpret_cast<const f32x4 *>(in + (size_t)r * in_stride);
#pragma unroll
        for (int c = 0; c < NV; ++c)
            x[c] = src[FULL ? c * 64 + lane : min(c * 64 + lane, nvec - 1)];
    };
    auto process = [&](const f32x4 (&x)[NV], int group) {
        const int row0 = group * LN3_ROWS;
        float sum = 0.0f, sq = 0.0f;
#pragma unroll
        for (int c = 0; c < NV; ++c) {
            if (FULL || c * 64 + lane < nvec) {
#pragma unroll
                for (int e = 0; e < 4; ++e) {
                    sum += x[c][e];
                    sq += x[c][e] * x[c][e];
                }
            }
        }
        sum = wave_sum(sum);
        sq = wave_sum(sq);
        const float mean = sum / (float)E;
        const float var = sq / (float)E - mean * mean;
        const float inv_std = 1.0f / sqrtf((float)((double)var + eps));
#pragma unroll
        for (int c = 0; c < NV; ++c) {
            const int idx = c * 64 + lane;
            if (FULL || idx < nvec) {
                const f32x4 g = g4[idx], bb = b4[idx];
                f32x4 y;
                float amax = 0.0f;
#pragma unroll
                for (int e = 0; e < 4; ++e) {
                    y[e] = (x[c][e] - mean) * inv_std * g[e] + bb[e];
                    amax = fmaxf(amax, fabsf(y[e]));
                }
                amax = fmaxf(amax, __shfl_xor(amax, 1));
                amax = fmaxf(amax, __shfl_xor(amax, 2));
                amax = fmaxf(amax, __shfl_xor(amax, 4));
                unsigned sbyte;
                float mult;
                mx_block_scale(amax, sbyte, mult);
                const int k = 4 * idx, ks = k >> 7, blk = (k >> 5) & 3;
                *reinterpret_cast<unsigned *>(ln_lds + (ks * LN3_ROWS + wave) * 128 + (k & 127)) = pack_fp8x4(y * mult);
                if ((lane & 7) == 0)
                    lds_scales[((((ks >> 2) * 4 + 2 * (blk & 1) + (blk >> 1)) * LN3_ROWS + wave) << 2) + (ks & 3)] = (char)sbyte;
            }
        }
        lds_barrier();
        const int vpieces = ksteps * 2;
        for (int pc = wave; pc < vpieces; pc += LN3_ROWS) {
            const int ks = pc >> 1, r = 8 * (pc & 1) + (lane >> 3);
            if (row0 + r < rows)
                *reinterpret_cast<f32x4 *>(values + ((size_t)ks * rows + row0 + r) * 128 + 16 * (lane & 7)) =
                    *reinterpret_cast<const f32x4 *>(ln_lds + (ks * LN3_ROWS + r) * 128 + 16 * (lane & 7));
        }
        if ((int)threadIdx.x < sgroups * 4 * LN3_ROWS) {
            const int pair = threadIdx.x / LN3_ROWS, r = threadIdx.x % LN3_ROWS;
            if (row0 + r < rows)
                reinterpret_cast<unsigned *>(scales)[(size_t)pair * rows + row0 + r] = reinterpret_cast<const unsigned *>(lds_scales)[threadIdx.x];
        }
        lds_barrier();
    };

    f32x4 xa[NV], xb[NV];
    int g0 = blockIdx.x;
    if (g0 >= ngroups)
        return;
    load_rows(xa, g0);
    for (;;) {
        const int g1 = g0 + stride;
        load_rows(xb, min(g1, ngroups - 1));
        process(xa, g0);
        if (g1 >= ngroups)
            break;
        const int g2 = g1 + stride;
        load_rows(xa, min(g2, ngroups - 1));
        process(xb, g1);
        if (g2 >= ngroups)
            break;
        g0 = g2;
    }
}

__global__ void gather_rows_kernel(const char *__restrict__ src, char *__restrict__ dst, int n_planes, int dst_rows,
                                   size_t src_plane_bytes, int row_bytes, size_t src_row_stride_bytes)
{
    const size_t idx = (size_t)blockIdx.x * blockDim.x + threadIdx.x;
    const int per_row = row_bytes >> 4;
    const size_t total = (size_t)n_planes * dst_rows * per_row;
    if (idx >= total)
        return;
    const int c = (int)(idx % per_row);
    const size_t r = idx / per_row;
    const int plane = (int)(r / dst_rows), row = (int)(r % dst_rows);
    *reinterpret_cast<f32x4 *>(dst + ((size_t)plane * dst_rows + row) * row_bytes + 16 * c) =
        *reinterpret_cast<const f32x4 *>(src + plane * src_plane_bytes + row * src_row_stride_bytes + 16 * c);
}

constexpr int SM_THREADS = 256;
constexpr int SM_MAX_PER_THREAD = 8;

__global__ __launch_bounds__(SM_THREADS) void softmax_kernel(const float *__restrict__ in,
                                                            float *__restrict__ out, int length)
{
    __shared__ float red[SM_THREADS / 64];
    const int tid = threadIdx.x, lane = tid & 63, wave = tid >> 6;
    const float *src = in + (size_t)blockIdx.x * length;
    float *dst = out + (size_t)blockIdx.x * length;

    float v[SM_MAX_PER_THREAD];
    float mx = -INFINITY;
#pragma unroll
    for (int i = 0; i < SM_MAX_PER_THREAD; ++i) {
        const int idx = tid + i * SM_THREADS;
        v[i] = idx < length ? src[idx] : -INFINITY;
        mx = fmaxf(mx, v[i]);
    }
    mx = wave_max(mx);
    if (lane == 0)
        red[wave] = mx;
    __syncthreads();
    mx = fmaxf(fmaxf(red[0], red[1]), fmaxf(red[2], red[3]));
    __syncthreads();

    float sum = 0.0f;
#pragma unroll
    for (int i = 0; i < SM_MAX_PER_THREAD; ++i) {
        v[i] = expf(v[i] - mx);
        sum += v[i];
    }
    sum = wave_sum(sum);
    if (lane == 0)
        red[wave] = sum;
    __syncthreads();
    sum = (red[0] + red[1]) + (red[2] + red[3]);
#pragma unroll
    for (int i = 0; i < SM_MAX_PER_THREAD; ++i) {
        const int idx = tid + i * SM_THREADS;
        if (idx < length)
            dst[idx] = v[i] / sum;
    }
}

}

static int launch_layer_norm(vh_stream_t s, const float *input, const float *weight, const float *bias,
                             void *output, int out_kind, float out_mult, int rows, int embed_dim,
                             long in_row_stride, long out_row_stride, double eps)
{
    if (!input || !weight || !bias || !output)
        return vh_fail(1, "vh_launch_layer_norm: null pointer argument");
    if (rows <= 0 || embed_dim <= 0 || embed_dim % 4 != 0 || embed_dim > 2048)
        return vh_fail(1, "vh_launch_layer_norm: embed_dim=%d must be a multiple of 4, <= 2048", embed_dim);
    if (in_row_stride % 4 != 0 || out_row_stride % 4 != 0 || in_row_stride < embed_dim ||
        out_row_stride < embed_dim)
        return vh_fail(1, "vh_launch_layer_norm: row strides must be multiples of 4 floats and >= embed_dim");
    hipStream_t st = (hipStream_t)s;
    const dim3 grid((rows + 3) / 4), block(256);
    const int nv = (embed_dim / 4 + 63) / 64;
#define VH_LN_K(NV, OUTK)                                                                          \
    hipLaunchKernelGGL((layernorm_kernel<NV, OUTK>), grid, block, 0, st, input, weight, bias, output, \
                       rows, embed_dim, in_row_stride, out_row_stride, eps, out_mult)
#define VH_LN(NV)                                                                                   \
    do {                                                                                            \
        VH_LN_K(NV, 0);                                                                             \
    } while (0)
    if (nv <= 3) VH_LN(3);
    else if (nv <= 4) VH_LN(4);
    else if (nv <= 5) VH_LN(5);
    else VH_LN(8);
#undef VH_LN
#undef VH_LN_K
    VH_LAUNCH_CHECK("layernorm_kernel");
    return 0;
}

extern "C" int vh_launch_layer_norm(vh_stream_t s, const float *input, const float *weight,
                                    const float *bias, float *output, int rows, int embed_dim,
                                    long in_row_stride, long out_row_stride, double eps)
{
    return launch_layer_norm(s, input, weight, bias, output, 0, 1.0f, rows, embed_dim, in_row_stride,
                             out_row_stride, eps);
}

constexpr int LN3_LDS_LIMIT = 160 * 1024;

extern "C" int vh_layer_norm_planes_max_embed(int parts)
{
    if (parts != 1 && parts != 3)
        return 0;
    const int by_lds = LN3_LDS_LIMIT / (parts * LN3_ROWS * 64) * 32;
    return by_lds < 2048 ? by_lds : 2048;
}

extern "C" int vh_launch_layer_norm_planes(vh_stream_t s, const float *input, const float *weight, const float *bias,
                                           void *out_planes, int parts, int rows, int embed_dim, long in_row_stride,
                                           double eps)
{
    if (!input || !weight || !bias || !out_planes)
        return vh_fail(1, "vh_launch_layer_norm_planes: null pointer argument");
    if (rows <= 0 || embed_dim <= 0 || embed_dim % 32 != 0 || embed_dim > 2048 || ((uintptr_t)out_planes & 15) ||
        (parts != 1 && parts != 3))
        return vh_fail(1, "vh_launch_layer_norm_planes: embed_dim=%d must be a multiple of 32, <= 2048 with one part and "
                          "<= 1696 with three, planes 16-byte aligned, parts 1 or 3", embed_dim);
    if (embed_dim > vh_layer_norm_planes_max_embed(parts))
        return vh_fail(1, "vh_launch_layer_norm_planes: embed_dim=%d with %d parts needs %d bytes of LDS for its 16-row image, "
                          "a CU has %d: the largest embed_dim with %d parts is %d", embed_dim, parts,
                       32 * parts * embed_dim, LN3_LDS_LIMIT, parts, vh_layer_norm_planes_max_embed(parts));
    if (in_row_stride % 4 != 0 || in_row_stride < embed_dim)
        return vh_fail(1, "vh_launch_layer_norm_planes: row stride must be a multiple of 4 floats and >= embed_dim");
    const int nv = (embed_dim / 4 + 63) / 64;
    const size_t lds = (size_t)(embed_dim / 32) * parts * LN3_ROWS * 64;
    const int ngroups = (rows + LN3_ROWS - 1) / LN3_ROWS;
    const int resident = LN3_LDS_LIMIT / (int)lds < 2 ? 1 : 2;
    const int cap = resident * vh_device_cus(vh_current_device());
    const dim3 grid(ngroups < cap ? ngroups : cap), block(64 * LN3_ROWS);
    hipStream_t st = (hipStream_t)s;
#define VH_LN3_F(NV, NPL, FULL)                                                                           \
    do {                                                                                                  \
        VH_SET_LDS_ONCE((layernorm_p3_kernel<NV, NPL, FULL>), LN3_LDS_LIMIT);                             \
        hipLaunchKernelGGL((layernorm_p3_kernel<NV, NPL, FULL>), grid, block, lds, st, input, weight, bias, \
                           static_cast<char *>(out_planes), rows, embed_dim, in_row_stride, eps);         \
    } while (0)
#define VH_LN3_K(NV, NPL)                                                                                 \
    do {                                                                                                  \
        if (embed_dim == 256 * (NV))                                                                      \
            VH_LN3_F(NV, NPL, true);                                                                      \
        else                                                                                              \
            VH_LN3_F(NV, NPL, false);                                                                     \
    } while (0)
#define VH_LN3(NV)                                                                                        \
    do {                                                                                                  \
        if (parts == 3)                                                                                   \
            VH_LN3_K(NV, 3);                                                                              \
        else                                                                                              \
            VH_LN3_K(NV, 1);                                                                              \
    } while (0)
    if (nv <= 3) VH_LN3(3);
    else if (nv <= 4) VH_LN3(4);
    else if (nv <= 5) VH_LN3(5);
    else VH_LN3(8);
#undef VH_LN3
#undef VH_LN3_K
#undef VH_LN3_F
    VH_LAUNCH_CHECK("layernorm_p3_kernel");
    return 0;
}

extern "C" int vh_launch_layer_norm_p3(vh_stream_t s, const float *input, const float *weight, const float *bias,
                                       void *out_planes, int rows, int embed_dim, long in_row_stride, double eps)
{
    return vh_launch_layer_norm_planes(s, input, weight, bias, out_planes, 3, rows, embed_dim, in_row_stride, eps);
}

extern "C" int vh_launch_layer_norm_mx(vh_stream_t s, const float *input, const float *weight, const float *bias,
                                       void *out_values, void *out_scales, int rows, int embed_dim, long in_row_stride,
                                       double eps)
{
    if (!input || !weight || !bias || !out_values || !out_scales)
        return vh_fail(1, "vh_launch_layer_norm_mx: null pointer argument");
    if (rows <= 0 || embed_dim <= 0 || embed_dim % 128 != 0 || embed_dim > 2048 || ((uintptr_t)out_values & 15) || ((uintptr_t)out_scales & 3))
        return vh_fail(1, "vh_launch_layer_norm_mx: embed_dim=%d must be a multiple of 128, <= 2048, values 16-byte aligned", embed_dim);
    if (in_row_stride % 4 != 0 || in_row_stride < embed_dim)
        return vh_fail(1, "vh_launch_layer_norm_mx: row stride must be a multiple of 4 floats and >= embed_dim");
    const int nv = (embed_dim / 4 + 63) / 64;
    const size_t lds = (size_t)(embed_dim / 128) * LN3_ROWS * 128 + (size_t)((embed_dim / 128 + 3) / 4) * 4 * LN3_ROWS * 4;
    const int ngroups = (rows + LN3_ROWS - 1) / LN3_ROWS;
    const int cap = 2 * vh_device_cus(vh_current_device());
    const dim3 grid(ngroups < cap ? ngroups : cap), block(64 * LN3_ROWS);
    hipStream_t st = (hipStream_t)s;
#define VH_LNMX_F(NV, FULL)                                                                                    \
    hipLaunchKernelGGL((layernorm_mx_kernel<NV, FULL>), grid, block, lds, st, input, weight, bias,             \
                       static_cast<char *>(out_values), static_cast<unsigned char *>(out_scales), rows,      \
                       embed_dim, in_row_stride, eps)
#define VH_LNMX(NV)                                                                                            \
    do {                                                                                                       \
        if (embed_dim == 256 * (NV))                                                                           \
            VH_LNMX_F(NV, true);                                                                               \
        else                                                                                                   \
            VH_LNMX_F(NV, false);                                                                              \
    } while (0)
    if (nv <= 3) VH_LNMX(3);
    else if (nv <= 4) VH_LNMX(4);
    else if (nv <= 5) VH_LNMX(5);
    else VH_LNMX(8);
#undef VH_LNMX
#undef VH_LNMX_F
    VH_LAUNCH_CHECK("layernorm_mx_kernel");
    return 0;
}

extern "C" int vh_launch_gather_rows(vh_stream_t s, const void *src, void *dst, int n_planes, int src_rows, int dst_rows,
                                     int row_bytes, int row_stride)
{
    if (!src || !dst || n_planes <= 0 || src_rows <= 0 || dst_rows <= 0 || row_bytes <= 0 || row_bytes % 16 != 0 || row_stride <= 0 ||
        (size_t)(dst_rows - 1) * row_stride >= (size_t)src_rows || (((uintptr_t)src | (uintptr_t)dst) & 15))
        return vh_fail(1, "vh_launch_gather_rows: bad argument (row_bytes %% 16 == 0, (dst_rows-1)*row_stride < src_rows, 16-byte aligned)");
    const size_t threads = (size_t)n_planes * dst_rows * (row_bytes / 16);
    hipLaunchKernelGGL(gather_rows_kernel, dim3((unsigned)((threads + 255) / 256)), dim3(256), 0, (hipStream_t)s,
                       static_cast<const char *>(src), static_cast<char *>(dst), n_planes, dst_rows, (size_t)src_rows * row_bytes,
                       row_bytes, (size_t)row_stride * row_bytes);
    VH_LAUNCH_CHECK("gather_rows_kernel");
    return 0;
}

extern "C" int vh_launch_softmax(vh_stream_t s, const float *input, float *output, int rows,
                                 int length)
{
    if (!input || !output)
        return vh_fail(1, "vh_launch_softmax: null pointer argument");
    if (rows <= 0 || length <= 0 || length > SM_THREADS * SM_MAX_PER_THREAD)
        return vh_fail(1, "vh_launch_softmax: length=%d must be in 1..%d", length,
                       SM_THREADS * SM_MAX_PER_THREAD);
    hipLaunchKernelGGL(softmax_kernel, dim3(rows), dim3(SM_THREADS), 0, (hipStream_t)s, input, output,
                       length);
    VH_LAUNCH_CHECK("softmax_kernel");
    return 0;
}
```

### vit-with-opencl_amd/host/binding.py

```python
from __future__ import annotations

import ctypes as C
import os
import subprocess
from pathlib import Path

import numpy as np

PKG_DIR = Path(__file__).resolve().parent.parent
LIB_PATH = PKG_DIR / "libvit_hip.so"
CSRC = PKG_DIR / "csrc"

f32p = C.POINTER(C.c_float)
voidp = C.c_void_p

EXPORTS = [
    "vh_device_count", "vh_init", "vh_last_error", "vh_device_name",
    "vh_stream_create", "vh_stream_destroy", "vh_stream_sync", "vh_device_sync",
    "vh_event_create", "vh_event_destroy", "vh_event_record", "vh_stream_wait_event", "vh_event_sync",
    "vh_event_elapsed_ms",
    "vh_malloc", "vh_free", "vh_host_alloc", "vh_host_free", "vh_memset", "vh_h2d", "vh_d2h", "vh_d2d",
    "vh_launch_patch_embed", "vh_launch_layer_norm", "vh_launch_linear", "vh_launch_attention",
    "vh_launch_softmax",
    "vit_config_preset", "vit_config_tokens", "vit_config_num_tensors", "vit_config_tensor_size",
    "ViT_opencl", "vit_hip_last_call_seconds", "vit_hip_create", "vit_hip_destroy", "vit_hip_forward", "vit_hip_forward_device",
    "vit_hip_config", "vit_hip_stream", "vit_hip_max_batch", "vit_hip_weight", "vit_hip_read_tokens",
    "vit_hip_profile_enable", "vit_hip_profile_read", "vit_hip_profile_select", "vit_hip_create_ex", "vit_hip_precision",
    "vit_hip_export_planes", "vit_hip_create_from_planes",
    "vh_patch_embed_workspace", "vh_launch_patch_embed_ws", "vh_patch_planes_k", "vh_launch_conv_weight_planes",
    "vh_launch_patch_embed_planes", "vh_launch_split3_planes", "vh_launch_linear_w3",
    "vh_launch_split2h_planes", "vh_launch_linear_h2", "vh_launch_attention_h2", "vh_launch_attention_f16",
    "vh_launch_absmax",
    "vh_launch_split3_rows", "vh_launch_merge3_rows", "vh_launch_layer_norm_p3", "vh_launch_attention_p3",
    "vh_launch_linear_p3", "vh_launch_split_rows", "vh_launch_merge_rows", "vh_launch_layer_norm_planes", "vh_layer_norm_planes_max_embed",
    "vh_launch_attention_planes_bf16", "vh_launch_linear_planes", "vh_launch_attention_planes",
    "vh_launch_quantize_mx_rows", "vh_launch_quantize_mx_act", "vh_mx_act_scale_bytes", "vh_launch_linear_mx", "vh_launch_layer_norm_mx",
    "vh_launch_attention_planes_f16", "vh_launch_linear_mx_planes_f16", "vh_launch_attention_planes_f16_mx",
    "vh_launch_attention_planes_f16_hd80", "vh_launch_attention_planes_f16_hd80_operand", "vh_launch_attention_long",
    "vh_launch_gather_rows", "vit_hip_set_last_layer_cls_only",
    "vh_launch_conv_weight_planes_parts", "vh_launch_patch_embed_planes3",
    "vh_launch_colsum_planes3", "vh_launch_patch_embed_planes3_norm", "vh_launch_linear_p3_norm", "vh_launch_linear_p3_resid_norm",
    "vh_launch_fold_gamma", "vh_launch_fold_bias", "vh_launch_colsum_operand", "vh_launch_patch_embed_planes_norm",
    "vh_launch_linear_planes_norm", "vh_launch_linear_planes_resid_norm", "vh_launch_linear_mx_norm",
    "vh_launch_linear_mx_resid_norm", "vit_hip_ln_fold",
    "vh_set_device", "vit_hip_create_multi", "vit_hip_forward_multi", "vit_hip_destroy_multi", "vit_hip_multi_devices",
    "vit_hip_multi_ctx", "vit_shard_range", "vit_shard_run", "vit_shard_run_timed", "vit_hip_multi_last_enqueue_ms",
    "vit_hip_forward_device_multi", "vit_hip_device", "vh_set_error",
    "vit_synth_fill", "vit_synth_tensor", "vit_synth_image",
    "load_image_data", "load_weights", "vit_write_image_file", "vit_write_weight_file",
    "vit_write_result_file", "vit_compare_rows",
    "vh_launch_patch_embed_planes_u8", "vh_launch_expand_u8", "vit_pixel_norm_from_mean_std", "vit_hip_forward_device_u8",
    "vit_hip_forward_u8",
    "vh_launch_resize_crop_u8", "vit_resize_crop_geometry", "vit_hip_resize_crop_u8", "vit_hip_forward_device_u8_resized",
    "vit_hip_forward_u8_resized",
    "vit_box_check", "vit_box_rows", "vit_tile_boxes", "vit_hip_crop_boxes_u8", "vit_hip_forward_device_u8_boxes",
    "vit_hip_forward_u8_boxes",
    "vh_feature_readout_scratch", "vh_launch_feature_readout", "vit_feature_sizes", "vit_hip_set_features",
    "vit_hip_set_features_host",
    "vh_launch_linear_math", "vh_launch_patch_embed_ws_math", "vh_launch_attention_rows",
    "vh_launch_topk", "vit_topk_check", "vit_hip_set_topk", "vit_hip_set_topk_host", "vit_write_result_file_topk",
    "vh_cls_attention_head_dim_ok", "vh_launch_cls_attention", "vit_attn_sizes", "vit_hip_set_attention",
    "vit_hip_set_attention_host",
]

FP32_MATH = {"split3": 0, "native": 1}
ATTN_ARITH = {"native": 0, "fp16": 1, "fp16x2": 2, "split3": 3}
ATTN_KERNEL = {"auto": 0, "streaming": 1}


class VitConfig(C.Structure):

    _fields_ = [
        ("img_size", C.c_int), ("patch_size", C.c_int), ("in_chans", C.c_int),
        ("num_classes", C.c_int), ("embed_dim", C.c_int), ("depth", C.c_int),
        ("num_heads", C.c_int), ("mlp_hidden", C.c_int), ("eps", C.c_double),
    ]


class PixelNorm(C.Structure):

    _fields_ = [("scale", C.c_float * 4), ("bias", C.c_float * 4)]


PIXEL_LAYOUTS = {"hwc": 0, "chw": 1}


class ImageU8(C.Structure):

    _fields_ = [("data", C.c_void_p), ("height", C.c_int), ("width", C.c_int), ("row_stride", C.c_long)]


class ResizeCrop(C.Structure):

    _fields_ = [("resize_short", C.c_int), ("filter", C.c_int)]


RESIZE_FILTERS = {"bilinear": 0, "bicubic": 1}


class Box(C.Structure):

    _fields_ = [("image", C.c_int), ("box", C.c_float * 4)]


class FeatureSpecC(C.Structure):

    _fields_ = [("n_taps", C.c_int), ("taps", C.c_int * 4), ("final_norm", C.c_int), ("l2_normalize", C.c_int),
                ("dtype", C.c_int), ("token_layout", C.c_int)]


class FeatureBuffers(C.Structure):

    _fields_ = [("cls", C.c_void_p), ("pooled", C.c_void_p), ("tokens", C.c_void_p)]


FEATURE_DTYPES = {"f32": 0, "bf16": 1}
TOKEN_LAYOUTS = {"nlc": 0, "nchw": 1}


class FeatureSpec:

    def __init__(self, taps=(-1,), final_norm: bool = True, l2_normalize: bool = False, dtype: str = "f32",
                 token_layout: str = "nlc"):
        self.taps, self.final_norm, self.l2_normalize = tuple(int(t) for t in taps), bool(final_norm), bool(l2_normalize)
        self.dtype, self.token_layout = dtype, token_layout

    @property
    def np_dtype(self):
        return np.dtype(np.float32 if self.dtype == "f32" else np.uint16)

    def c_struct(self) -> FeatureSpecC:
        taps = list(self.taps[:4]) + [0] * (4 - min(len(self.taps), 4))
        return FeatureSpecC(len(self.taps), (C.c_int * 4)(*taps), int(self.final_norm), int(self.l2_normalize),
                            FEATURE_DTYPES[self.dtype], TOKEN_LAYOUTS[self.token_layout])


class TopKSpecC(C.Structure):

    _fields_ = [("k", C.c_int), ("score_kind", C.c_int)]


class TopKBuffers(C.Structure):

    _fields_ = [("labels", C.c_void_p), ("scores", C.c_void_p)]


TOPK_SCORES = {"probs": 0, "logits": 1}


class TopKSpec:

    def __init__(self, k: int = 5, scores: str = "probs"):
        self.k, self.scores = int(k), scores

    def c_struct(self) -> TopKSpecC:
        return TopKSpecC(self.k, TOPK_SCORES[self.scores])


class AttnSpecC(C.Structure):

    _fields_ = [("n_taps", C.c_int), ("taps", C.c_int * 4)]


class AttnBuffers(C.Structure):

    _fields_ = [("heads", C.c_void_p), ("mean", C.c_void_p)]


QKV_FORMS = {"rows_f32": 0, "planes3": 1, "planes_f16": 2}


class AttentionSpec:

    def __init__(self, taps=(-1,)):
        self.taps = tuple(int(t) for t in taps)

    def c_struct(self) -> AttnSpecC:
        taps = list(self.taps[:4]) + [0] * (4 - min(len(self.taps), 4))
        return AttnSpecC(len(self.taps), (C.c_int * 4)(*taps))


def attention_sizes(cfg: "VitConfig", spec: AttentionSpec):
    out = [C.c_size_t() for _ in range(2)]
    cs = spec.c_struct()
    check(lib().vit_attn_sizes(C.byref(cfg), C.byref(cs), *[C.byref(o) for o in out]), "vit_attn_sizes")
    return tuple(o.value for o in out)


def topk_check(cfg: "VitConfig", spec: TopKSpec) -> None:
    cs = spec.c_struct()
    check(lib().vit_topk_check(C.byref(cfg), C.byref(cs)), "vit_topk_check")


def feature_sizes(cfg: "VitConfig", spec: FeatureSpec):
    out = [C.c_size_t() for _ in range(3)]
    cs = spec.c_struct()
    check(lib().vit_feature_sizes(C.byref(cfg), C.byref(cs), *[C.byref(o) for o in out]), "vit_feature_sizes")
    return tuple(o.value for o in out)


def resize_crop(resize_short: int, filter: str = "bilinear") -> ResizeCrop:
    return ResizeCrop(int(resize_short), RESIZE_FILTERS[filter])


def resize_crop_geometry(height: int, width: int, resize_short: int, crop: int, filter: str = "bilinear"):
    out = [C.c_int() for _ in range(4)]
    rc = resize_crop(resize_short, filter)
    check(lib().vit_resize_crop_geometry(height, width, C.byref(rc), crop, *[C.byref(o) for o in out]), "vit_resize_crop_geometry")
    return tuple(o.value for o in out)


def box_array(boxes) -> C.Array:
    arr = (Box * len(boxes))()
    for i, b in enumerate(boxes):
        arr[i] = b if isinstance(b, Box) else Box(int(b[0]), (C.c_float * 4)(*[float(v) for v in b[1]]))
    return arr


def box_check(height: int, width: int, box) -> None:
    check(lib().vit_box_check(height, width, (C.c_float * 4)(*[float(v) for v in box])), "vit_box_check")


def box_rows(height: int, top: float, bottom: float, out: int, filter: str = "bilinear"):
    first, count = C.c_int(), C.c_int()
    check(lib().vit_box_rows(height, top, bottom, out, RESIZE_FILTERS[filter], C.byref(first), C.byref(count)), "vit_box_rows")
    return first.value, count.value


def tile_boxes(h: int, w: int, tile: int, stride: int, image: int = 0):
    n = lib().vit_tile_boxes(h, w, tile, stride, image, None, 0)
    if n < 0:
        check(1, "vit_tile_boxes")
    arr = (Box * n)()
    if lib().vit_tile_boxes(h, w, tile, stride, image, arr, n) != n:
        check(1, "vit_tile_boxes")
    return [(b.image, tuple(b.box)) for b in arr]


def image_descs(images) -> C.Array:
    arr = (ImageU8 * len(images))()
    for i, (ptr, h, w, stride) in enumerate(images):
        arr[i] = ImageU8(int(ptr.value if isinstance(ptr, C.c_void_p) else ptr), h, w, stride)
    return arr


def host_image_descs(images, layout: str):
    keep = []
    arr = (ImageU8 * len(images))()
    for i, a in enumerate(images):
        a = np.asarray(a)
        if a.dtype != np.uint8 or a.ndim != 3:
            raise ValueError(f"image {i}: need a 3-d uint8 array, got {a.dtype} {a.shape}")
        if layout == "hwc":
            h, w, ch = a.shape
            ok = a.strides[2] == 1 and a.strides[1] == ch and a.strides[0] >= w * ch
        else:
            ch, h, w = a.shape
            ok = a.strides[2] == 1 and a.strides[1] >= w and a.strides[0] == h * a.strides[1]
        if not ok:
            a = np.ascontiguousarray(a)
        keep.append(a)
        arr[i] = ImageU8(a.ctypes.data, h, w, a.strides[0] if layout == "hwc" else a.strides[1])
    return arr, keep


class CompareReport(C.Structure):
    _fields_ = [("rows", C.c_int), ("classes", C.c_int), ("max_abs_diff", C.c_double), ("mean_abs_diff", C.c_double),
                ("top1_equal", C.c_int), ("top1_equal_or_near_tie", C.c_int), ("top5_overlap", C.c_double),
                ("nonfinite", C.c_int)]


class ImageData(C.Structure):

    _fields_ = [("n", C.c_int), ("c", C.c_int), ("h", C.c_int), ("w", C.c_int), ("data", f32p)]


class Network(C.Structure):

    _fields_ = [("data", f32p), ("size", C.c_size_t)]


SHARD_FN = C.CFUNCTYPE(C.c_int, C.c_void_p, C.c_int, C.c_int, C.c_int)


class VitHipError(RuntimeError):
    pass


def build_library(force: bool = False) -> Path:
    srcs = list(CSRC.glob("*.hip")) + list(CSRC.glob("*.c")) + list(CSRC.glob("*.h")) + \
        list((PKG_DIR.parent / "include").glob("*.h"))
    stale = (not LIB_PATH.exists()) or any(s.stat().st_mtime > LIB_PATH.stat().st_mtime for s in srcs)
    if force or stale:
        r = subprocess.run(["make", "-C", str(CSRC), "-j8"], capture_output=True, text=True)
        if r.returncode != 0:
            raise VitHipError("building libvit_hip.so failed:\n" + r.stdout[-4000:] + r.stderr[-4000:])
    return LIB_PATH


_lib = None


def lib() -> C.CDLL:
    global _lib
    if _lib is not None:
        return _lib
    if not LIB_PATH.exists():
        raise VitHipError(f"{LIB_PATH} is missing: run __graft_entry__.build() (make -C {CSRC})")
    if os.environ.get("VIT_HIP_NO_TORCH", "0") != "1":
        try:
            import torch
        except ImportError:
            pass
    L = C.CDLL(os.environ.get("VIT_HIP_LIB") or str(LIB_PATH))
    i, sz = C.c_int, C.c_size_t
    L.vh_last_error.restype = C.c_char_p
    L.vh_device_name.restype = C.c_char_p
    L.vh_init.argtypes = [i]
    L.vh_stream_create.argtypes = [C.POINTER(voidp)]
    L.vh_stream_destroy.argtypes = [voidp]
    L.vh_stream_sync.argtypes = [voidp]
    L.vh_event_create.argtypes = [C.POINTER(voidp)]
    L.vh_event_destroy.argtypes = [voidp]
    L.vh_event_record.argtypes = [voidp, voidp]
    L.vh_stream_wait_event.argtypes = [voidp, voidp]
    L.vh_event_sync.argtypes = [voidp]
    L.vh_event_elapsed_ms.argtypes = [C.POINTER(C.c_float), voidp, voidp]
    L.vh_malloc.argtypes = [C.POINTER(voidp), sz]
    L.vh_free.argtypes = [voidp]
    L.vh_host_alloc.argtypes = [C.POINTER(voidp), sz]
    L.vh_host_free.argtypes = [voidp]
    L.vh_memset.argtypes = [voidp, i, sz, voidp]
    L.vh_h2d.argtypes = [voidp, voidp, sz, voidp]
    L.vh_d2h.argtypes = [voidp, voidp, sz, voidp]
    L.vh_d2d.argtypes = [voidp, voidp, sz, voidp]
    L.vh_launch_patch_embed.argtypes = [voidp] + [voidp] * 6 + [i] * 5
    L.vh_launch_patch_embed_ws.argtypes = [voidp] + [voidp] * 6 + [i] * 5 + [voidp, sz]
    L.vh_launch_patch_embed_ws_math.argtypes = [voidp] + [voidp] * 6 + [i] * 5 + [voidp, sz, i]
    L.vh_patch_embed_workspace.argtypes = [i] * 5
    L.vh_patch_planes_k.argtypes = [i, i]
    L.vh_launch_conv_weight_planes.argtypes = [voidp, voidp, voidp, i, i, i]
    L.vh_launch_patch_embed_planes.argtypes = [voidp] + [voidp] * 6 + [i] * 5 + [voidp, sz]
    L.vh_patch_embed_workspace.restype = sz
    L.vh_launch_layer_norm.argtypes = [voidp] + [voidp] * 4 + [i, i, C.c_long, C.c_long, C.c_double]
    L.vh_launch_linear.argtypes = [voidp] + [voidp] * 4 + [i, i, i, i, voidp]
    L.vh_launch_linear_math.argtypes = [voidp] + [voidp] * 4 + [i, i, i, i, voidp, i]
    L.vh_launch_attention.argtypes = [voidp, voidp, voidp, i, i, i, i]
    L.vh_launch_attention_rows.argtypes = [voidp, voidp, voidp, i, i, i, i, i, i, i]
    L.vh_launch_attention_h2.argtypes = [voidp, voidp, voidp, i, i, i, i]
    L.vh_launch_attention_f16.argtypes = [voidp, voidp, voidp, i, i, i, i]
    L.vh_launch_split3_planes.argtypes = [voidp, voidp, voidp, i, i]
    L.vh_launch_linear_w3.argtypes = [voidp] + [voidp] * 4 + [i, i, i, i, voidp]
    L.vh_launch_split2h_planes.argtypes = [voidp, voidp, voidp, i, i, C.c_float]
    L.vh_launch_linear_h2.argtypes = [voidp, voidp, voidp, C.c_float, voidp, voidp, i, i, i, i, voidp]
    L.vh_launch_softmax.argtypes = [voidp, voidp, voidp, i, i]
    L.vh_launch_split3_rows.argtypes = [voidp, voidp, voidp, i, i]
    L.vh_launch_merge3_rows.argtypes = [voidp, voidp, voidp, i, i]
    L.vh_launch_layer_norm_p3.argtypes = [voidp] + [voidp] * 4 + [i, i, C.c_long, C.c_double]
    L.vh_launch_attention_p3.argtypes = [voidp, voidp, voidp, i, i, i, i]
    L.vh_launch_linear_p3.argtypes = [voidp, voidp, i, voidp, voidp, voidp, i, i, i, i, voidp]
    L.vh_launch_split_rows.argtypes = [voidp, voidp, voidp, i, i, i]
    L.vh_launch_merge_rows.argtypes = [voidp, voidp, voidp, i, i, i]
    L.vh_launch_layer_norm_planes.argtypes = [voidp] + [voidp] * 4 + [i, i, i, C.c_long, C.c_double]
    L.vh_layer_norm_planes_max_embed.argtypes = [i]
    L.vh_launch_attention_planes_bf16.argtypes = [voidp, voidp, voidp, i, i, i, i]
    L.vh_launch_attention_planes.argtypes = [voidp, voidp, voidp, i, i, i, i]
    L.vh_launch_gather_rows.argtypes = [voidp, voidp, voidp, i, i, i, i, i]
    L.vit_hip_set_last_layer_cls_only.argtypes = [voidp, i]
    L.vh_launch_attention_planes_f16.argtypes = [voidp, voidp, voidp, i, i, i, i, i]
    L.vh_launch_attention_planes_f16_mx.argtypes = [voidp, voidp, voidp, voidp, i, i, i, i]
    L.vh_launch_attention_planes_f16_hd80.argtypes = [voidp, voidp, voidp, i, i, i, i]
    L.vh_launch_attention_planes_f16_hd80_operand.argtypes = [voidp, voidp, voidp, voidp, i, i, i, i, i]
    L.vh_launch_attention_long.argtypes = [voidp, voidp, i, voidp, i, i, i, i]
    L.vh_launch_linear_mx_planes_f16.argtypes = [voidp, voidp, voidp, voidp, voidp, voidp, voidp, i, i, i]
    L.vh_launch_quantize_mx_rows.argtypes = [voidp, voidp, voidp, voidp, i, i]
    L.vh_launch_layer_norm_mx.argtypes = [voidp] + [voidp] * 5 + [i, i, C.c_long, C.c_double]
    L.vh_launch_linear_mx.argtypes = [voidp, voidp, voidp, voidp, voidp, voidp, voidp, voidp, i, i, i, i, voidp]
    L.vh_launch_linear_planes.argtypes = [voidp, voidp, i, voidp, voidp, i, voidp, i, i, i, i, voidp]
    L.vh_launch_conv_weight_planes_parts.argtypes = [voidp, voidp, voidp, i, i, i, i]
    L.vh_launch_patch_embed_planes3.argtypes = [voidp] + [voidp] * 6 + [i] * 5 + [voidp, sz]
    L.vh_launch_colsum_planes3.argtypes = [voidp, voidp, voidp, i, i]
    L.vh_launch_patch_embed_planes3_norm.argtypes = [voidp] + [voidp] * 6 + [i] * 5 + [voidp, sz, voidp, voidp]
    L.vh_launch_linear_p3_norm.argtypes = [voidp, voidp, i, voidp, voidp, voidp, voidp, voidp, C.c_double, i, i, i, i]
    L.vh_launch_linear_p3_resid_norm.argtypes = [voidp, voidp, voidp, voidp, voidp, voidp, i, i, i, voidp, voidp]
    L.vh_launch_quantize_mx_act.argtypes = [voidp, voidp, voidp, voidp, i, i]
    L.vh_mx_act_scale_bytes.argtypes = [i, i]
    L.vh_mx_act_scale_bytes.restype = sz
    L.vh_launch_fold_gamma.argtypes = [voidp, voidp, voidp, voidp, i, i]
    L.vh_launch_fold_bias.argtypes = [voidp, voidp, voidp, voidp, voidp, i, i]
    L.vh_launch_colsum_operand.argtypes = [voidp, voidp, voidp, voidp, i, i]
    L.vh_launch_patch_embed_planes_norm.argtypes = [voidp] + [voidp] * 6 + [i] * 5 + [voidp, sz, voidp, voidp, voidp]
    L.vh_launch_linear_planes_norm.argtypes = [voidp, voidp, i, voidp, voidp, voidp, voidp, voidp, C.c_double, i, i, i, i]
    L.vh_launch_linear_planes_resid_norm.argtypes = [voidp, voidp, voidp, voidp, voidp, voidp, i, i, i, voidp, voidp, voidp]
    L.vh_launch_linear_mx_norm.argtypes = [voidp, voidp, voidp, i, voidp, voidp, voidp, voidp, voidp, voidp, voidp, C.c_double, i, i, i, i]
    L.vh_launch_linear_mx_resid_norm.argtypes = [voidp, voidp, voidp, voidp, voidp, voidp, voidp, voidp, i, i, i, voidp, voidp, voidp]
    L.vit_hip_ln_fold.argtypes = [voidp]
    L.vit_config_preset.argtypes = [C.POINTER(VitConfig), C.c_char_p]
    L.vit_config_tokens.argtypes = [C.POINTER(VitConfig)]
    L.vit_config_num_tensors.argtypes = [C.POINTER(VitConfig)]
    L.vit_config_tensor_size.argtypes = [C.POINTER(VitConfig), i]
    L.vit_config_tensor_size.restype = sz
    L.ViT_opencl.argtypes = [C.POINTER(ImageData), C.POINTER(Network), C.POINTER(f32p)]
    L.ViT_opencl.restype = None
    L.vit_hip_last_call_seconds.argtypes = [C.POINTER(C.c_double), C.POINTER(C.c_double)]
    L.vit_hip_last_call_seconds.restype = None
    L.vit_hip_create.argtypes = [C.POINTER(voidp), C.POINTER(VitConfig), C.POINTER(Network), i, i, i]
    L.vit_hip_create_ex.argtypes = [C.POINTER(voidp), C.POINTER(VitConfig), C.POINTER(Network), i, i, i, i]
    L.vit_hip_precision.argtypes = [voidp]
    L.vit_hip_export_planes.argtypes = [voidp, C.c_char_p]
    L.vit_hip_create_from_planes.argtypes = [C.POINTER(voidp), C.c_char_p, i, i]
    f = C.c_float
    L.vh_launch_absmax.argtypes = [voidp, voidp, sz, voidp]
    L.vit_hip_destroy.argtypes = [voidp]
    L.vit_hip_destroy.restype = None
    L.vh_set_device.argtypes = [i]
    L.vit_hip_create_multi.argtypes = [C.POINTER(voidp), C.POINTER(VitConfig), C.POINTER(Network), i, C.POINTER(i), i, i, i]
    L.vit_hip_forward_multi.argtypes = [voidp, C.POINTER(ImageData), i, f32p, C.POINTER(f32p)]
    L.vit_hip_destroy_multi.argtypes = [voidp]
    L.vit_hip_destroy_multi.restype = None
    L.vit_hip_multi_devices.argtypes = [voidp]
    L.vit_hip_multi_ctx.argtypes = [voidp, i]
    L.vit_hip_multi_ctx.restype = voidp
    L.vit_hip_device.argtypes = [voidp]
    L.vit_hip_forward_device_multi.argtypes = [voidp, C.POINTER(voidp), C.POINTER(i), voidp, voidp]
    L.vh_set_error.argtypes = [i, C.c_char_p]
    L.vit_shard_range.argtypes = [i, i, i, C.POINTER(i), C.POINTER(i)]
    L.vit_shard_range.restype = None
    L.vit_shard_run.argtypes = [i, i, SHARD_FN, voidp]
    L.vit_shard_run_timed.argtypes = [i, i, SHARD_FN, voidp, C.POINTER(C.c_double)]
    L.vit_hip_multi_last_enqueue_ms.argtypes = [voidp, C.POINTER(C.c_double), i]
    L.vit_hip_forward.argtypes = [voidp, C.POINTER(ImageData), i, f32p, C.POINTER(f32p)]
    L.vit_hip_forward_device.argtypes = [voidp, voidp, i, voidp, voidp, voidp]
    L.vit_hip_stream.argtypes = [voidp]
    L.vit_hip_stream.restype = voidp
    L.vit_hip_max_batch.argtypes = [voidp]
    L.vit_hip_weight.argtypes = [voidp, i]
    L.vit_hip_weight.restype = voidp
    L.vit_hip_read_tokens.argtypes = [voidp, i, f32p]
    L.vit_hip_profile_enable.argtypes = [voidp, i]
    L.vit_hip_profile_select.argtypes = [voidp, C.c_uint]
    L.vit_hip_profile_read.argtypes = [voidp, C.POINTER(C.c_double), C.POINTER(C.c_long)]
    L.vit_synth_fill.argtypes = [f32p, sz, C.c_ulonglong, C.c_float, C.c_float]
    L.vit_synth_fill.restype = None
    L.vit_synth_tensor.argtypes = [C.POINTER(VitConfig), i, C.c_ulonglong, f32p]
    L.vit_synth_tensor.restype = None
    L.vit_synth_image.argtypes = [C.POINTER(VitConfig), i, f32p]
    L.vit_synth_image.restype = None
    L.load_image_data.argtypes = [C.c_char_p]
    L.load_image_data.restype = C.POINTER(ImageData)
    L.load_weights.argtypes = [C.c_char_p, C.POINTER(Network), i]
    L.load_weights.restype = None
    L.vit_write_image_file.argtypes = [C.c_char_p, C.POINTER(ImageData), i]
    L.vit_write_weight_file.argtypes = [C.c_char_p, i, C.c_char_p, f32p, sz]
    L.vit_write_result_file.argtypes = [C.c_char_p, C.POINTER(f32p), i, i]
    L.vit_compare_rows.argtypes = [f32p, f32p, i, i, C.c_double, C.POINTER(CompareReport)]
    u8p = C.POINTER(C.c_ubyte)
    L.vh_launch_patch_embed_planes_u8.argtypes = [voidp, voidp, i, f32p, f32p] + [voidp] * 5 + [i] * 5 + [voidp, sz, i] + [voidp] * 3
    L.vh_launch_expand_u8.argtypes = [voidp, voidp, i, f32p, f32p, voidp, i, i, i]
    L.vit_pixel_norm_from_mean_std.argtypes = [C.POINTER(PixelNorm), f32p, f32p, i]
    L.vit_hip_forward_device_u8.argtypes = [voidp, voidp, i, i, C.POINTER(PixelNorm), voidp, voidp, voidp]
    L.vit_hip_forward_u8.argtypes = [voidp, u8p, i, i, C.POINTER(PixelNorm), f32p, C.POINTER(f32p)]
    imgp, rcp, ip = C.POINTER(ImageU8), C.POINTER(ResizeCrop), C.POINTER(C.c_int)
    L.vh_launch_resize_crop_u8.argtypes = [voidp, voidp, i, i, i, i, i, voidp, sz, voidp]
    L.vit_resize_crop_geometry.argtypes = [i, i, rcp, i, ip, ip, ip, ip]
    L.vit_hip_resize_crop_u8.argtypes = [voidp, imgp, i, i, rcp, voidp, voidp]
    L.vit_hip_forward_device_u8_resized.argtypes = [voidp, imgp, i, i, rcp, C.POINTER(PixelNorm), voidp, voidp, voidp]
    L.vit_hip_forward_u8_resized.argtypes = [voidp, imgp, i, i, rcp, C.POINTER(PixelNorm), f32p, C.POINTER(f32p)]
    boxp = C.POINTER(Box)
    L.vit_box_check.argtypes = [i, i, C.POINTER(C.c_float)]
    L.vit_box_rows.argtypes = [i, C.c_float, C.c_float, i, i, ip, ip]
    L.vit_tile_boxes.argtypes = [i, i, i, i, i, boxp, i]
    L.vit_hip_crop_boxes_u8.argtypes = [voidp, imgp, i, boxp, i, i, i, voidp, voidp]
    L.vit_hip_forward_device_u8_boxes.argtypes = [voidp, imgp, i, boxp, i, i, i, C.POINTER(PixelNorm), voidp, voidp, voidp]
    L.vit_hip_forward_u8_boxes.argtypes = [voidp, imgp, i, boxp, i, i, i, C.POINTER(PixelNorm), f32p, C.POINTER(f32p)]
    L.vh_feature_readout_scratch.argtypes = [i, i, i]
    L.vh_feature_readout_scratch.restype = sz
    L.vh_launch_feature_readout.argtypes = [voidp, voidp, voidp, C.c_long, voidp, voidp, C.c_double] + [i] * 9 + [voidp] * 4 + [sz]
    specp, bufp, szp = C.POINTER(FeatureSpecC), C.POINTER(FeatureBuffers), C.POINTER(sz)
    L.vit_feature_sizes.argtypes = [C.POINTER(VitConfig), specp, szp, szp, szp]
    L.vit_hip_set_features.argtypes = [voidp, specp, bufp]
    L.vit_hip_set_features_host.argtypes = [voidp, specp, bufp]
    ip32 = C.POINTER(C.c_int)
    L.vh_launch_topk.argtypes = [voidp, voidp, i, i, i, i, voidp, voidp]
    tkp, tbp = C.POINTER(TopKSpecC), C.POINTER(TopKBuffers)
    L.vit_topk_check.argtypes = [C.POINTER(VitConfig), tkp]
    L.vit_hip_set_topk.argtypes = [voidp, tkp, tbp]
    L.vit_hip_set_topk_host.argtypes = [voidp, tkp, tbp]
    L.vit_write_result_file_topk.argtypes = [C.c_char_p, ip32, f32p, i, i]
    L.vh_cls_attention_head_dim_ok.argtypes = [i]
    L.vh_launch_cls_attention.argtypes = [voidp, voidp] + [i] * 7 + [voidp, voidp]
    asp, abp = C.POINTER(AttnSpecC), C.POINTER(AttnBuffers)
    L.vit_attn_sizes.argtypes = [C.POINTER(VitConfig), asp, szp, szp]
    L.vit_hip_set_attention.argtypes = [voidp, asp, abp]
    L.vit_hip_set_attention_host.argtypes = [voidp, asp, abp]
    _lib = L
    return L


def check(rc: int, what: str = "") -> None:
    if rc != 0:
        raise VitHipError(f"{what} failed with status {rc}: {lib().vh_last_error().decode()}")


def fptr(a: np.ndarray):
    assert a.dtype == np.float32 and a.flags.c_contiguous, "need contiguous float32"
    return a.ctypes.data_as(f32p)


def preset(name: str) -> VitConfig:
    cfg = VitConfig()
    if lib().vit_config_preset(C.byref(cfg), name.encode()) != 0:
        raise ValueError(f"unknown preset {name}")
    return cfg


def tokens(cfg: VitConfig) -> int:
    return lib().vit_config_tokens(C.byref(cfg))


def synth_weights(cfg: VitConfig, seed_base: int = 0) -> list[np.ndarray]:
    L = lib()
    out = []
    for idx in range(L.vit_config_num_tensors(C.byref(cfg))):
        a = np.empty(L.vit_config_tensor_size(C.byref(cfg), idx), dtype=np.float32)
        L.vit_synth_tensor(C.byref(cfg), idx, seed_base, fptr(a))
        out.append(a)
    return out


def synth_images(cfg: VitConfig, first: int, count: int) -> np.ndarray:
    L = lib()
    a = np.empty((count, cfg.in_chans, cfg.img_size, cfg.img_size), dtype=np.float32)
    for i in range(count):
        L.vit_synth_image(C.byref(cfg), first + i, fptr(a[i]))
    return a


def pixel_norm(mean, std) -> PixelNorm:
    mean = np.ascontiguousarray(mean, dtype=np.float32)
    std = np.ascontiguousarray(std, dtype=np.float32)
    if mean.shape != std.shape or mean.ndim != 1:
        raise ValueError("mean and std: one value per channel each")
    out = PixelNorm()
    check(lib().vit_pixel_norm_from_mean_std(C.byref(out), fptr(mean), fptr(std), mean.size), "vit_pixel_norm_from_mean_std")
    return out


def networks(weights: list[np.ndarray]):
    arr = (Network * len(weights))()
    for i, w in enumerate(weights):
        arr[i].data = fptr(w)
        arr[i].size = w.size
    return arr


def image_array(images: np.ndarray):
    n, c, h, w = images.shape
    arr = (ImageData * n)()
    for i in range(n):
        arr[i].n, arr[i].c, arr[i].h, arr[i].w = n, c, h, w
        arr[i].data = fptr(images[i])
    return arr


class DeviceBuffer:

    def __init__(self, count: int, dtype=np.float32):
        self.count = int(count)
        self.dtype = np.dtype(dtype)
        self.ptr = voidp()
        check(lib().vh_malloc(C.byref(self.ptr), max(self.count, 1) * self.dtype.itemsize), "vh_malloc")

    @classmethod
    def from_numpy(cls, a: np.ndarray, dtype=np.float32) -> "DeviceBuffer":
        a = np.ascontiguousarray(a, dtype=dtype)
        d = cls(a.size, dtype)
        check(lib().vh_h2d(d.ptr, a.ctypes.data_as(voidp), a.nbytes, None), "vh_h2d")
        check(lib().vh_device_sync(), "vh_device_sync")
        return d

    def to_numpy(self, shape=None) -> np.ndarray:
        out = np.empty(self.count, dtype=self.dtype)
        check(lib().vh_d2h(out.ctypes.data_as(voidp), self.ptr, out.nbytes, None), "vh_d2h")
        check(lib().vh_device_sync(), "vh_device_sync")
        return out.reshape(shape) if shape is not None else out

    def free(self):
        if self.ptr:
            lib().vh_free(self.ptr)
            self.ptr = voidp()

    def __del__(self):
        try:
            self.free()
        except Exception:
            pass


def _device_ptr(b):
    return b.ptr if isinstance(b, DeviceBuffer) else b


def _host_ptr(a):
    return a.ctypes.data


class ViTHip:

    PRECISIONS = {"f32": 0, "bf16": 1, "fp8": 2, "f32_fp16x2": 3}

    def __init__(self, cfg: VitConfig, weights: list[np.ndarray], device: int = 0, max_batch: int = 64,
                 precision: str = "f32"):
        self.cfg = cfg
        self.L = lib()
        self._weights = weights
        self.ctx = voidp()
        self.precision = precision
        rc = self.L.vit_hip_create_ex(C.byref(self.ctx), C.byref(cfg), networks(weights), len(weights),
                                      device, max_batch, self.PRECISIONS[precision])
        check(rc, "vit_hip_create_ex")
        self.max_batch = max_batch
        self.tokens = tokens(cfg)

    @classmethod
    def from_planes(cls, path, device: int = 0, max_batch: int = 64) -> "ViTHip":
        self = cls.__new__(cls)
        self.L, self._weights, self.ctx = lib(), None, voidp()
        check(self.L.vit_hip_create_from_planes(C.byref(self.ctx), str(path).encode(), device, max_batch),
              "vit_hip_create_from_planes")
        self.L.vit_hip_config.restype = C.POINTER(VitConfig)
        self.L.vit_hip_config.argtypes = [voidp]
        self.cfg = VitConfig.from_buffer_copy(self.L.vit_hip_config(self.ctx).contents)
        self.precision = {v: k for k, v in cls.PRECISIONS.items()}[self.L.vit_hip_precision(self.ctx)]
        self.max_batch, self.tokens = max_batch, tokens(self.cfg)
        return self

    def export_planes(self, path) -> None:
        check(self.L.vit_hip_export_planes(self.ctx, str(path).encode()), "vit_hip_export_planes")

    @property
    def stream(self):
        return self.L.vit_hip_stream(self.ctx)

    def forward(self, images: np.ndarray):
        images = np.ascontiguousarray(images, dtype=np.float32)
        n, nc = images.shape[0], self.cfg.num_classes
        logits = np.empty((n, nc), dtype=np.float32)
        probs = np.empty((n, nc), dtype=np.float32)
        rows = (f32p * n)(*[fptr(probs[i]) for i in range(n)])
        check(self.L.vit_hip_forward(self.ctx, image_array(images), n, fptr(logits), rows), "vit_hip_forward")
        return logits, probs

    def forward_u8(self, images: np.ndarray, mean, std, layout: str = "hwc", logits: bool = True, probs: bool = True):
        cfg = self.cfg
        images = np.ascontiguousarray(images, dtype=np.uint8)
        n, S, Ch = images.shape[0], cfg.img_size, cfg.in_chans
        want = (n, S, S, Ch) if layout == "hwc" else (n, Ch, S, S)
        if images.shape != want:
            raise ValueError(f"forward_u8: images of shape {images.shape}, the context's config takes {want} ({layout})")
        norm = mean if isinstance(mean, PixelNorm) else pixel_norm(mean, std)
        nc = cfg.num_classes
        out_l = np.empty((n, nc), dtype=np.float32) if logits else None
        out_p = np.empty((n, nc), dtype=np.float32) if probs else None
# ... 221 lines not shown
```

Before: 6227.

## Store FC1 hidden activations as fp32 planes and split them inside the GEMM

Adds an A32 input path to the three-part GEMM: it loads raw fp32 activation tiles and splits them into three bf16 parts in registers, interleaved with the MFMA schedule, instead of reading pre-split planes. FC1 can now write its GELU output as fp32 planes (2/3 of the three-plane bytes), and FC2 consumes them directly. LayerNorm can optionally emit fp32 planes too, off by default. This cuts the memory traffic of the large hidden activation, in exchange for extra VALU split work and register pressure inside the GEMM main loop.

New measurement: 6257 (median of 6 runs). About the same (+0.5%).

```diff
diff --git a/include/kernelHandler.h b/include/kernelHandler.h
--- a/include/kernelHandler.h
+++ b/include/kernelHandler.h
@@ -123,6 +123,11 @@
 int vh_launch_linear_p3(vh_stream_t s, void *output, int output_planes, const void *weight_planes,
                         const void *input_planes, const float *bias, int rowA, int colA, int colB,
                         int doGelu, const float *residual);
+int vh_launch_linear_a32(vh_stream_t s, void *output, int output_form, const void *weight_planes3, const void *input,
+                         int input_a32, const float *bias, int rowA, int colA, int colB, int doGelu, const float *residual);
+int vh_launch_layer_norm_a32(vh_stream_t s, const float *input, const float *weight, const float *bias,
+                             void *out_planes, int rows, int embed_dim, long in_row_stride, double eps);
+int vh_launch_a32_rows(vh_stream_t s, const float *input, float *output, int rows, int cols, int to_planes);
 
 int vh_launch_split2h_planes(vh_stream_t s, const float *weight, void *planes, int rows, int cols, float scale);
 int vh_launch_linear_h2(vh_stream_t s, float *output, const void *weight_planes, float weight_scale,
diff --git a/vit-with-opencl_amd/csrc/ViT_hip.c b/vit-with-opencl_amd/csrc/ViT_hip.c
--- a/vit-with-opencl_amd/csrc/ViT_hip.c
+++ b/vit-with-opencl_amd/csrc/ViT_hip.c
@@ -34,6 +34,9 @@
 
 enum { MAX_DEPTH = 256, MAX_TENSORS = 4 + 12 * MAX_DEPTH + 4 };
 
+#define VIT_A32_LN_DEFAULT 0
+#define VIT_A32_HID_DEFAULT 1
+
 enum { DESC_RING = 8, RESIZE_MAX_SIDE = 16384 };
 
 enum { FEAT_NONE, FEAT_DEVICE, FEAT_HOST };
@@ -58,6 +61,7 @@
     int ln_fold;
     int use_p3;
     int cls_only_last;
+    int a32_ln, a32_hid;
     int attn_form;
     int fp32_native;
     int attn_rows_streaming;
@@ -477,6 +481,12 @@
     ctx->ln_fold = ln_fold ? 1 : 0;
     ctx->use_p3 = use_p3;
     ctx->cls_only_last = use_p3 && !ln_fold && env_ll && strcmp(env_ll, "cls") == 0;
+    {
+        const char *env_ln = getenv("VIT_HIP_A32_LN"), *env_hid = getenv("VIT_HIP_A32_HID");
+        const int a32_fits = use_p3 && !ln_fold && (size_t)max_batch * (size_t)T * 128 <= 0xffffffffull;
+        ctx->a32_ln = a32_fits && (env_ln ? env_ln[0] == '1' : VIT_A32_LN_DEFAULT);
+        ctx->a32_hid = a32_fits && (env_hid ? env_hid[0] == '1' : VIT_A32_HID_DEFAULT);
+    }
     ctx->attn_form = !(use_p3 || reduced) ? ATTN_STREAMING
               : (long_wanted && long_hd) ? ATTN_LONG
               : (E == 64 * H && T <= 208) ? ATTN_HD64
@@ -937,10 +947,12 @@
     float **lw = layer_tensors(ctx, l);
     const struct operand *op = ctx->op + 4 * l;
     const int planes_attn = ctx->attn_form == ATTN_HD64 || ctx->attn_form == ATTN_LONG;
+    const int y32 = ctx->a32_ln, h32 = ctx->a32_hid;
     if (!fold)
-        OP(VIT_OP_LAYER_NORM, vh_launch_layer_norm_p3(s, ctx->x, lw[0], lw[1], ctx->y, rows, E, E, c->eps));
+        OP(VIT_OP_LAYER_NORM, y32 ? vh_launch_layer_norm_a32(s, ctx->x, lw[0], lw[1], ctx->y, rows, E, E, c->eps)
+                                  : vh_launch_layer_norm_p3(s, ctx->x, lw[0], lw[1], ctx->y, rows, E, E, c->eps));
     OP(VIT_OP_QKV, fold ? vh_launch_linear_p3_norm(s, ctx->qkv, planes_attn, op[0].w, ctx->y, ctx->stats, op[0].colsum, op[0].bias_folded, c->eps, rows, E, 3 * E, 0)
-                        : vh_launch_linear_p3(s, ctx->qkv, planes_attn, op[0].w, ctx->y, lw[3], rows, E, 3 * E, 0, NULL));
+                        : vh_launch_linear_a32(s, ctx->qkv, planes_attn, op[0].w, ctx->y, y32, lw[3], rows, E, 3 * E, 0, NULL));
     TRY(attention_tap(ctx, s, n, l));
     OP(VIT_OP_ATTENTION, ctx->attn_form == ATTN_HD64 ? vh_launch_attention_planes(s, ctx->qkv, ctx->attn, n, T, E, c->num_heads)
                          : (rc = ctx->attn_form == ATTN_LONG ? vh_launch_attention_long(s, ctx->qkv, 3, ctx->hid, n, T, E, c->num_heads)
@@ -955,20 +967,22 @@
         OP(VIT_OP_OUT_PROJ, (rc = vh_launch_gather_rows(s, ctx->attn, attn_cls, 3 * (E / 32), rows, n, 64, T)) != 0 ? rc :
                             (rc = vh_launch_gather_rows(s, ctx->x, x_cls, 1, rows, n, 4 * E, T)) != 0 ? rc :
                             vh_launch_linear_p3(s, x_cls, 0, op[1].w, attn_cls, lw[5], n, E, E, 0, x_cls));
-        OP(VIT_OP_LAYER_NORM, vh_launch_layer_norm_p3(s, x_cls, lw[6], lw[7], y_cls, n, E, E, c->eps));
-        OP(VIT_OP_FC1, vh_launch_linear_p3(s, hid_cls, 1, op[2].w, y_cls, lw[9], n, E, F, 1, NULL));
-        OP(VIT_OP_FC2, vh_launch_linear_p3(s, x_cls, 0, op[3].w, hid_cls, lw[11], n, F, E, 0, x_cls));
+        OP(VIT_OP_LAYER_NORM, y32 ? vh_launch_layer_norm_a32(s, x_cls, lw[6], lw[7], y_cls, n, E, E, c->eps)
+                                  : vh_launch_layer_norm_p3(s, x_cls, lw[6], lw[7], y_cls, n, E, E, c->eps));
+        OP(VIT_OP_FC1, vh_launch_linear_a32(s, hid_cls, h32 ? 2 : 1, op[2].w, y_cls, y32, lw[9], n, E, F, 1, NULL));
+        OP(VIT_OP_FC2, vh_launch_linear_a32(s, x_cls, 0, op[3].w, hid_cls, h32, lw[11], n, F, E, 0, x_cls));
         *cls_rows = 1;
         return 0;
     }
     OP(VIT_OP_OUT_PROJ, fold ? vh_launch_linear_p3_resid_norm(s, ctx->x, op[1].w, ctx->attn, lw[5], ctx->x, rows, E, E, ctx->y, ctx->stats)
                              : vh_launch_linear_p3(s, ctx->x, 0, op[1].w, ctx->attn, lw[5], rows, E, E, 0, ctx->x));
     if (!fold)
-        OP(VIT_OP_LAYER_NORM, vh_launch_layer_norm_p3(s, ctx->x, lw[6], lw[7], ctx->y, rows, E, E, c->eps));
+        OP(VIT_OP_LAYER_NORM, y32 ? vh_launch_layer_norm_a32(s, ctx->x, lw[6], lw[7], ctx->y, rows, E, E, c->eps)
+                                  : vh_launch_layer_norm_p3(s, ctx->x, lw[6], lw[7], ctx->y, rows, E, E, c->eps));
     OP(VIT_OP_FC1, fold ? vh_launch_linear_p3_norm(s, ctx->hid, 1, op[2].w, ctx->y, ctx->stats, op[2].colsum, op[2].bias_folded, c->eps, rows, E, F, 1)
-                        : vh_launch_linear_p3(s, ctx->hid, 1, op[2].w, ctx->y, lw[9], rows, E, F, 1, NULL));
+                        : vh_launch_linear_a32(s, ctx->hid, h32 ? 2 : 1, op[2].w, ctx->y, y32, lw[9], rows, E, F, 1, NULL));
     OP(VIT_OP_FC2, fold && !last ? vh_launch_linear_p3_resid_norm(s, ctx->x, op[3].w, ctx->hid, lw[11], ctx->x, rows, F, E, ctx->y, ctx->stats)
-                                 : vh_launch_linear_p3(s, ctx->x, 0, op[3].w, ctx->hid, lw[11], rows, F, E, 0, ctx->x));
+                                 : vh_launch_linear_a32(s, ctx->x, 0, op[3].w, ctx->hid, h32, lw[11], rows, F, E, 0, ctx->x));
     return 0;
 fail:
     return rc;
diff --git a/vit-with-opencl_amd/csrc/gemm_p3.hip b/vit-with-opencl_amd/csrc/gemm_p3.hip
--- a/vit-with-opencl_amd/csrc/gemm_p3.hip
+++ b/vit-with-opencl_amd/csrc/gemm_p3.hip
@@ -18,7 +18,7 @@
 #define P1_KG 2
 #endif
 enum { EPI_NONE = 0, EPI_GELU = 1, EPI_RESID = 2, EPI_PATCH = 3, EPI_NORM = 4, EPI_NORM_GELU = 5 };
-enum { OUT_F32 = 0, OUT_PLANES = 1, OUT_PLANES_H = 2, OUT_F32_OPER = 3, OUT_F32_OPER_MX = 4 };
+enum { OUT_F32 = 0, OUT_PLANES = 1, OUT_PLANES_H = 2, OUT_F32_OPER = 3, OUT_F32_OPER_MX = 4, OUT_PLANES_F32 = 5 };
 
 struct P3Params {
     const char *A;
@@ -40,8 +40,15 @@
     int c_rows;
 };
 
-template <int NW, int BN, int EPI, int OUTK, int NPL = 3>
-__global__ __launch_bounds__(64 * NW, 2) void gemm_p3_kernel(const P3Params p)
+struct P3ParamsA32 : P3Params {};
+struct P3ParamsC32 : P3Params {};
+struct P3ParamsA32C32 : P3Params {};
+template <class P> struct P3Form { static constexpr bool C32 = false; };
+template <> struct P3Form<P3ParamsC32> { static constexpr bool C32 = true; };
+template <> struct P3Form<P3ParamsA32C32> { static constexpr bool C32 = true; };
+
+template <int NW, int BN, int EPI, int OUTK, int NPL, bool A32>
+__device__ __forceinline__ void gemm_p3_body(const P3Params &p)
 {
     constexpr int BM = 32 * NW, JT = BN / 16;
     constexpr int KG = NPL == 3 ? 1 : P1_KG;
@@ -55,6 +62,7 @@
     constexpr bool GELU = EPI == EPI_GELU || EPI == EPI_NORM_GELU;
     constexpr bool OPER = OUTK == OUT_F32_OPER || OUTK == OUT_F32_OPER_MX;
     static_assert(NPL == 1 || NPL == 3, "parts per value");
+    static_assert((!A32 && OUTK != OUT_PLANES_F32) || NPL == 3, "fp32 planes: the exact path only");
     static_assert(JT % 2 == 0 && (KG * NPL * BN / 16) % NW == 0 && F % RING == 0, "tile shape");
     static_assert(OUTK != OUT_F32_OPER_MX || NPL == 1, "an MX operand follows one-part operands only");
     static_assert(!OPER || (BN % 128 == 0 && (EPI == EPI_RESID || EPI == EPI_PATCH)), "operand producers: residual-stream epilogues");
@@ -72,7 +80,7 @@
     unsigned aoff[2];
 #pragma unroll
     for (int i = 0; i < 2; ++i)
-        aoff[i] = (unsigned)min(m0 + 32 * wave + 16 * i + l15, p.row_end - 1) * 64u + 16u * q;
+        aoff[i] = (unsigned)min(m0 + 32 * wave + 16 * i + l15, p.row_end - 1) * (A32 ? 128u : 64u) + (A32 ? 32u : 16u) * q;
     const size_t a_plane = (size_t)p.a_rows * 64, w_plane = (size_t)p.N * 64;
 
     const unsigned wlane = (unsigned)(lane >> 2) * 64u + 16u * ((lane & 3) ^ swz64(lane >> 4));
@@ -121,6 +129,29 @@
                     a[kg][i][pl] = __builtin_bit_cast(frag_t, *reinterpret_cast<gvec_t>(base + aoff[i]));
             }
     };
+    f32x4 raw[2][2];
+    auto load_raw = [&](int kt) {
+        gchar_t base = (gchar_t)p.A + (size_t)kt * (2 * a_plane);
+        asm volatile("" : "+s"(base));
+#pragma unroll
+        for (int i = 0; i < 2; ++i)
+#pragma unroll
+            for (int h = 0; h < 2; ++h)
+                raw[i][h] = *reinterpret_cast<gvec_t>(base + aoff[i] + 16 * h);
+    };
+    auto split_piece = [&](frag_t (&a)[KG][2][NPL], int pc) {
+        const int i = pc >> 1, h = pc & 1;
+        bf16x4 part[3];
+        split4(raw[i][h], part[0], part[1], part[2]);
+#pragma unroll
+        for (int pl = 0; pl < NPL; ++pl)
+#pragma unroll
+            for (int e = 0; e < 4; ++e)
+                a[0][i][pl][4 * h + e] = part[pl][e];
+#pragma unroll
+        for (int pl = 0; pl < NPL; ++pl)
+            asm volatile("" : "+v"(a[0][i][pl]));
+    };
     auto dma_w = [&](int stage, int kt) {
 #pragma unroll
         for (int i = 0; i < PW; ++i) {
@@ -157,17 +188,40 @@
             __builtin_amdgcn_sched_group_barrier(0x008, 2 * NT - 2 * NPL, 0);
         __builtin_amdgcn_sched_barrier(0);
     };
+    constexpr int A32_VALU = 4;
+    auto interleave_split = [&]() {
+#pragma unroll
+        for (int r = 0; r < NPL; ++r) {
+            __builtin_amdgcn_sched_group_barrier(0x100, 1, 0);
+            __builtin_amdgcn_sched_group_barrier(0x008, 2, 0);
+            __builtin_amdgcn_sched_group_barrier(0x002, A32_VALU, 0);
+        }
+#pragma unroll
+        for (int r = NPL; r < NT; ++r) {
+            __builtin_amdgcn_sched_group_barrier(0x008, 2, 0);
+            __builtin_amdgcn_sched_group_barrier(0x002, A32_VALU, 0);
+        }
+        __builtin_amdgcn_sched_barrier(0);
+    };
 
     const int nk = p.K / (32 * KG);
     auto step = [&](const frag_t (&au)[KG][2][NPL], frag_t (&al)[KG][2][NPL], int kt) {
         const char *cur = smem + (kt & 1) * STAGE, *nxt = smem + ((kt + 1) & 1) * STAGE;
         const bool more1 = kt + 1 < nk, more2 = kt + 2 < nk;
-        load_a(al, more1 ? kt + 1 : kt);
+        if (A32)
+            load_raw(more1 ? kt + 1 : kt);
+        else
+            load_a(al, more1 ? kt + 1 : kt);
 #pragma unroll
         for (int f = 0; f <= F - RING; ++f) {
             read_w(w[(f + RING - 1) % RING], cur, f + RING - 1);
             mfma_frag(au, w[f % RING], f);
-            interleave();
+            if (A32 && f > F - RING - 4) {
+                split_piece(al, f - (F - RING - 3));
+                interleave_split();
+            } else {
+                interleave();
+            }
         }
         __syncthreads();
         if (more2)
@@ -182,7 +236,14 @@
     };
 
     dma_w(0, 0);
-    load_a(a0, 0);
+    if (A32) {
+        load_raw(0);
+#pragma unroll
+        for (int pc = 0; pc < 4; ++pc)
+            split_piece(a0, pc);
+    } else {
+        load_a(a0, 0);
+    }
     float *const ncol = reinterpret_cast<float *>(smem + 2 * STAGE);
     if (NORM && tid < 2 * BN / 4) {
         const int which = tid / (BN / 4), c4 = tid - which * (BN / 4);
@@ -257,6 +318,10 @@
 #pragma unroll
             for (int pl = 0; pl < NPL; ++pl)
                 *reinterpret_cast<f32x4 *>(dst + pl * a_plane) = __builtin_bit_cast(f32x4, part[pl]);
+        } else if (OUTK == OUT_PLANES_F32) {
+            char *dst = static_cast<char *>(p.C) + ((size_t)((n0 >> 5) + s) * p.a_rows + row) * 128 + 32 * q;
+            *reinterpret_cast<f32x4 *>(dst) = lo;
+            *reinterpret_cast<f32x4 *>(dst + 16) = hi;
         } else {
             float *cp = static_cast<float *>(p.C) + orow_[i] * p.N;
             *reinterpret_cast<f32x4 *>(cp + col) = lo;
@@ -341,20 +406,44 @@
     }
 }
 
-template <int NW, int BN, int EPI, int OUTK, int NPL>
-int launch_p3_tile(hipStream_t st, P3Params p)
+template <int NW, int BN, int EPI, int OUTK, int NPL = 3>
+__global__ __launch_bounds__(64 * NW, 2) void gemm_p3_kernel(const P3Params p)
+{
+    gemm_p3_body<NW, BN, EPI, OUTK, NPL, false>(p);
+}
+template <int NW, int BN, int EPI, int OUTK, int NPL = 3>
+__global__ __launch_bounds__(64 * NW, 2) void gemm_p3_kernel(const P3ParamsA32 p)
+{
+    gemm_p3_body<NW, BN, EPI, OUTK, NPL, true>(p);
+}
+template <int NW, int BN, int EPI, int OUTK, int NPL = 3>
+__global__ __launch_bounds__(64 * NW, 2) void gemm_p3_kernel(const P3ParamsC32 p)
+{
+    static_assert(OUTK == OUT_PLANES, "C32: a planes output written as fp32 planes");
+    gemm_p3_body<NW, BN, EPI, OUT_PLANES_F32, NPL, false>(p);
+}
+template <int NW, int BN, int EPI, int OUTK, int NPL = 3>
+__global__ __launch_bounds__(64 * NW, 2) void gemm_p3_kernel(const P3ParamsA32C32 p)
+{
+    static_assert(OUTK == OUT_PLANES, "C32: a planes output written as fp32 planes");
+    gemm_p3_body<NW, BN, EPI, OUT_PLANES_F32, NPL, true>(p);
+}
+
+template <int NW, int BN, int EPI, int OUTK, int NPL, class P>
+int launch_p3_tile(hipStream_t st, P p)
 {
     constexpr int LDS = 2 * (NPL == 3 ? 1 : P1_KG) * NPL * BN * 64 + ((EPI == EPI_NORM || EPI == EPI_NORM_GELU) ? 2 * BN * 4 : 0);
-    VH_SET_LDS_ONCE((gemm_p3_kernel<NW, BN, EPI, OUTK, NPL>), LDS);
+    void (*const kernel)(const P) = gemm_p3_kernel<NW, BN, EPI, OUTK, NPL>;
+    VH_SET_LDS_ONCE(kernel, LDS);
     p.mtiles = (p.row_end - p.row_begin + 32 * NW - 1) / (32 * NW);
     p.ntiles = p.N / BN;
-    hipLaunchKernelGGL((gemm_p3_kernel<NW, BN, EPI, OUTK, NPL>), dim3(p.mtiles * p.ntiles), dim3(64 * NW), LDS, st, p);
+    hipLaunchKernelGGL(kernel, dim3(p.mtiles * p.ntiles), dim3(64 * NW), LDS, st, p);
     VH_LAUNCH_CHECK("gemm_p3_kernel");
     return 0;
 }
 
-template <int EPI, int OUTK, int NPL>
-int launch_p3(hipStream_t st, const P3Params &p, int small_only)
+template <int EPI, int OUTK, int NPL, class P>
+int launch_p3(hipStream_t st, const P &p, int small_only)
 {
     const int rows = p.row_end - p.row_begin;
     const int num_cus = vh_device_cus(vh_current_device());
@@ -366,10 +455,10 @@
         return launch_p3_tile<4, 128, EPI, OUTK, NPL>(st, p);
     const long full = tiles / num_cus, rem = tiles % num_cus;
     const int rows_big = (int)(full * num_cus / ntiles) * 256;
-    auto big_tiles = [&](const P3Params &q) { return launch_p3_tile<8, 256, EPI, OUTK, NPL>(st, q); };
+    auto big_tiles = [&](const P &q) { return launch_p3_tile<8, 256, EPI, OUTK, NPL>(st, q); };
     if (rem == 0 || 4 * rem > 3 * num_cus || rows_big <= 0 || rows_big >= rows)
         return big_tiles(p);
-    P3Params big = p, rest = p;
+    P big = p, rest = p;
     big.row_end = p.row_begin + rows_big;
     rest.row_begin = big.row_end;
     const int rc = big_tiles(big);
@@ -516,6 +605,85 @@
 {
     return vh_launch_linear_planes(s, output, output_planes, weight_planes, input_planes, 3, bias, rowA, colA, colB,
                                    doGelu, residual);
+}
+
+namespace {
+template <class P>
+int linear_a32_form(hipStream_t st, void *output, int output_form, const void *weight_planes3, const void *input, const float *bias,
+                    int rowA, int colA, int colB, int doGelu, const float *residual)
+{
+    P p = {};
+    p.A = static_cast<const char *>(input);
+    p.W = static_cast<const char *>(weight_planes3);
+    p.bias = bias; p.R = residual; p.C = output;
+    p.row_begin = 0; p.row_end = rowA; p.a_rows = rowA;
+    p.N = colB; p.K = colA;
+    const int small_only = residual && colA < 2048;
+    if constexpr (P3Form<P>::C32) {
+        return launch_p3<EPI_GELU, OUT_PLANES, 3>(st, p, small_only);
+    } else {
+        if (doGelu)
+            return launch_p3<EPI_GELU, OUT_PLANES, 3>(st, p, small_only);
+        if (residual)
+            return launch_p3<EPI_RESID, OUT_F32, 3>(st, p, small_only);
+        return output_form ? launch_p3<EPI_NONE, OUT_PLANES, 3>(st, p, small_only) : launch_p3<EPI_NONE, OUT_F32, 3>(st, p, small_only);
+    }
+}
+}
+
+extern "C" int vh_launch_linear_a32(vh_stream_t s, void *output, int output_form, const void *weight_planes3, const void *input,
+                                    int input_a32, const float *bias, int rowA, int colA, int colB, int doGelu, const float *residual)
+{
+    if (output_form < 0 || output_form > 2 || (input_a32 != 0 && input_a32 != 1))
+        return vh_fail(1, "vh_launch_linear_a32: output_form is 0, 1 or 2 and input_a32 0 or 1");
+    if (!input_a32 && output_form != 2)
+        return vh_launch_linear_p3(s, output, output_form, weight_planes3, input, bias, rowA, colA, colB, doGelu, residual);
+    if (!output || !weight_planes3 || !input || !bias)
+        return vh_fail(1, "vh_launch_linear_a32: null pointer argument");
+    if (rowA <= 0 || colA <= 0 || colB <= 0 || colA % 64 != 0 || colB % 128 != 0)
+        return vh_fail(1, "vh_launch_linear_a32: needs colA %% 64 == 0 and colB %% 128 == 0 (%d,%d,%d)", rowA, colA, colB);
+    if ((doGelu && residual) || (residual && output_form) || (output_form == 2 && !doGelu) || (doGelu && !output_form))
+        return vh_fail(1, "vh_launch_linear_a32: unsupported epilogue combination (fp32 planes out: the GELU epilogue; GELU: planes out)");
+    if ((((uintptr_t)output | (uintptr_t)weight_planes3 | (uintptr_t)input | (uintptr_t)bias | (uintptr_t)residual) & 15) != 0)
+        return vh_fail(1, "vh_launch_linear_a32: pointers must be 16-byte aligned");
+    if ((size_t)rowA * 128 > 0xffffffffull)
+        return vh_fail(1, "vh_launch_linear_a32: rowA=%d too large", rowA);
+    hipStream_t st = (hipStream_t)s;
+    if (output_form == 2)
+        return input_a32 ? linear_a32_form<P3ParamsA32C32>(st, output, output_form, weight_planes3, input, bias, rowA, colA, colB, doGelu, residual)
+                         : linear_a32_form<P3ParamsC32>(st, output, output_form, weight_planes3, input, bias, rowA, colA, colB, doGelu, residual);
+    return linear_a32_form<P3ParamsA32>(st, output, output_form, weight_planes3, input, bias, rowA, colA, colB, doGelu, residual);
+}
+
+namespace {
+template <bool TO_PLANES>
+__global__ void a32_rows_kernel(const float *__restrict__ in, float *__restrict__ out, int rows, int K)
+{
+    const size_t idx = (size_t)blockIdx.x * blockDim.x + threadIdx.x;
+    const int k8 = K >> 3;
+    if (idx >= (size_t)rows * k8)
+        return;
+    const int row = (int)(idx / k8), c8 = (int)(idx - (size_t)row * k8);
+    const size_t r = (size_t)row * K + 8 * c8, pl = ((size_t)(c8 >> 2) * rows + row) * 32 + 8 * (c8 & 3);
+    const float *src = in + (TO_PLANES ? r : pl);
+    float *dst = out + (TO_PLANES ? pl : r);
+    *reinterpret_cast<f32x4 *>(dst) = *reinterpret_cast<const f32x4 *>(src);
+    *reinterpret_cast<f32x4 *>(dst + 4) = *reinterpret_cast<const f32x4 *>(src + 4);
+}
+}
+
+extern "C" int vh_launch_a32_rows(vh_stream_t s, const float *input, float *output, int rows, int cols, int to_planes)
+{
+    if (!input || !output || rows <= 0 || cols <= 0 || cols % 32 != 0 || (((uintptr_t)input | (uintptr_t)output) & 15))
+        return vh_fail(1, "vh_launch_a32_rows: bad argument (cols %% 32 == 0, 16-byte aligned pointers)");
+    const size_t threads = (size_t)rows * (cols / 8);
+    const dim3 grid((unsigned)((threads + 255) / 256));
+    if (to_planes)
+        hipLaunchKernelGGL(a32_rows_kernel<true>, grid, dim3(256), 0, (hipStream_t)s, input, output, rows, cols);
+    else
+        hipLaunchKernelGGL(a32_rows_kernel<false>, grid, dim3(256), 0, (hipStream_t)s, input, output, rows, cols);
+    VH_LAUNCH_CHECK("a32_rows_kernel");
+    return 0;
 }
 
 
diff --git a/vit-with-opencl_amd/csrc/rowops.hip b/vit-with-opencl_amd/csrc/rowops.hip
--- a/vit-with-opencl_amd/csrc/rowops.hip
+++ b/vit-with-opencl_amd/csrc/rowops.hip
@@ -113,6 +113,10 @@
 #pragma unroll
                 for (int e = 0; e < 4; ++e)
                     y[e] = (x[c][e] - mean) * inv_std * g[e] + bb[e];
+                if (NPL == 0) {
+                    *reinterpret_cast<f32x4 *>(ln_lds + ((size_t)(idx >> 3) * LN3_ROWS + wave) * 128 + 16 * (idx & 7)) = y;
+                    continue;
+                }
                 bf16x4 part[3];
                 if (NPL == 3)
                     split4(y, part[0], part[1], part[2]);
@@ -125,6 +129,14 @@
             }
         }
         lds_barrier();
+        if (NPL == 0) {
+            for (int pc = wave; pc < (E >> 5) * 2; pc += LN3_ROWS)
+                if (row0 + 8 * (pc & 1) + (lane >> 3) < rows)
+                    *reinterpret_cast<f32x4 *>(planes + ((size_t)(pc >> 1) * rows + row0) * 128 + (pc & 1) * 1024 + 16 * lane) =
+                        *reinterpret_cast<const f32x4 *>(ln_lds + pc * 1024 + 16 * lane);
+            lds_barrier();
+            return;
+        }
         const int pieces = (E >> 5) * NPL;
         if (row0 + (lane >> 2) < rows)
             for (int pc = wave; pc < pieces; pc += LN3_ROWS)
@@ -366,24 +378,24 @@
     return by_lds < 2048 ? by_lds : 2048;
 }
 
-extern "C" int vh_launch_layer_norm_planes(vh_stream_t s, const float *input, const float *weight, const float *bias,
-                                           void *out_planes, int parts, int rows, int embed_dim, long in_row_stride,
-                                           double eps)
+static int layer_norm_planes(vh_stream_t s, const float *input, const float *weight, const float *bias,
+                             void *out_planes, int parts, int rows, int embed_dim, long in_row_stride,
+                             double eps)
 {
     if (!input || !weight || !bias || !out_planes)
         return vh_fail(1, "vh_launch_layer_norm_planes: null pointer argument");
     if (rows <= 0 || embed_dim <= 0 || embed_dim % 32 != 0 || embed_dim > 2048 || ((uintptr_t)out_planes & 15) ||
-        (parts != 1 && parts != 3))
+        (parts != 0 && parts != 1 && parts != 3))
         return vh_fail(1, "vh_launch_layer_norm_planes: embed_dim=%d must be a multiple of 32, <= 2048 with one part and "
                           "<= 1696 with three, planes 16-byte aligned, parts 1 or 3", embed_dim);
-    if (embed_dim > vh_layer_norm_planes_max_embed(parts))
+    if (parts && embed_dim > vh_layer_norm_planes_max_embed(parts))
         return vh_fail(1, "vh_launch_layer_norm_planes: embed_dim=%d with %d parts needs %d bytes of LDS for its 16-row image, "
                           "a CU has %d: the largest embed_dim with %d parts is %d", embed_dim, parts,
                        32 * parts * embed_dim, LN3_LDS_LIMIT, parts, vh_layer_norm_planes_max_embed(parts));
     if (in_row_stride % 4 != 0 || in_row_stride < embed_dim)
         return vh_fail(1, "vh_launch_layer_norm_planes: row stride must be a multiple of 4 floats and >= embed_dim");
     const int nv = (embed_dim / 4 + 63) / 64;
-    const size_t lds = (size_t)(embed_dim / 32) * parts * LN3_ROWS * 64;
+    const size_t lds = (size_t)(embed_dim / 32) * (parts ? parts : 2) * LN3_ROWS * 64;
     const int ngroups = (rows + LN3_ROWS - 1) / LN3_ROWS;
     const int resident = LN3_LDS_LIMIT / (int)lds < 2 ? 1 : 2;
     const int cap = resident * vh_device_cus(vh_current_device());
@@ -406,6 +418,8 @@
     do {                                                                                                  \
         if (parts == 3)                                                                                   \
             VH_LN3_K(NV, 3);                                                                              \
+        else if (parts == 0)                                                                              \
+            VH_LN3_K(NV, 0);                                                                              \
         else                                                                                              \
             VH_LN3_K(NV, 1);                                                                              \
     } while (0)
@@ -418,6 +432,21 @@
 #undef VH_LN3_F
     VH_LAUNCH_CHECK("layernorm_p3_kernel");
     return 0;
+}
+
+extern "C" int vh_launch_layer_norm_planes(vh_stream_t s, const float *input, const float *weight, const float *bias,
+                                           void *out_planes, int parts, int rows, int embed_dim, long in_row_stride,
+                                           double eps)
+{
+    if (parts != 1 && parts != 3)
+        return vh_fail(1, "vh_launch_layer_norm_planes: parts must be 1 or 3, not %d", parts);
+    return layer_norm_planes(s, input, weight, bias, out_planes, parts, rows, embed_dim, in_row_stride, eps);
+}
+
+extern "C" int vh_launch_layer_norm_a32(vh_stream_t s, const float *input, const float *weight, const float *bias,
+                                        void *out_planes, int rows, int embed_dim, long in_row_stride, double eps)
+{
+    return layer_norm_planes(s, input, weight, bias, out_planes, 0, rows, embed_dim, in_row_stride, eps);
 }
 
 extern "C" int vh_launch_layer_norm_p3(vh_stream_t s, const float *input, const float *weight, const float *bias,
diff --git a/vit-with-opencl_amd/host/binding.py b/vit-with-opencl_amd/host/binding.py
--- a/vit-with-opencl_amd/host/binding.py
+++ b/vit-with-opencl_amd/host/binding.py
@@ -32,7 +32,7 @@
     "vh_launch_split2h_planes", "vh_launch_linear_h2", "vh_launch_attention_h2", "vh_launch_attention_f16",
     "vh_launch_absmax",
     "vh_launch_split3_rows", "vh_launch_merge3_rows", "vh_launch_layer_norm_p3", "vh_launch_attention_p3",
-    "vh_launch_linear_p3", "vh_launch_split_rows", "vh_launch_merge_rows", "vh_launch_layer_norm_planes", "vh_layer_norm_planes_max_embed",
+    "vh_launch_linear_p3", "vh_launch_linear_a32", "vh_launch_layer_norm_a32", "vh_launch_a32_rows", "vh_launch_split_rows", "vh_launch_merge_rows", "vh_launch_layer_norm_planes", "vh_layer_norm_planes_max_embed",
     "vh_launch_attention_planes_bf16", "vh_launch_linear_planes", "vh_launch_attention_planes",
     "vh_launch_quantize_mx_rows", "vh_launch_quantize_mx_act", "vh_mx_act_scale_bytes", "vh_launch_linear_mx", "vh_launch_layer_norm_mx",
     "vh_launch_attention_planes_f16", "vh_launch_linear_mx_planes_f16", "vh_launch_attention_planes_f16_mx",
@@ -359,6 +359,9 @@
     L.vh_launch_layer_norm_p3.argtypes = [voidp] + [voidp] * 4 + [i, i, C.c_long, C.c_double]
     L.vh_launch_attention_p3.argtypes = [voidp, voidp, voidp, i, i, i, i]
     L.vh_launch_linear_p3.argtypes = [voidp, voidp, i, voidp, voidp, voidp, i, i, i, i, voidp]
+    L.vh_launch_linear_a32.argtypes = [voidp, voidp, i, voidp, voidp, i, voidp, i, i, i, i, voidp]
+    L.vh_launch_layer_norm_a32.argtypes = [voidp] + [voidp] * 4 + [i, i, C.c_long, C.c_double]
+    L.vh_launch_a32_rows.argtypes = [voidp, voidp, voidp, i, i, i]
     L.vh_launch_split_rows.argtypes = [voidp, voidp, voidp, i, i, i]
     L.vh_launch_merge_rows.argtypes = [voidp, voidp, voidp, i, i, i]
     L.vh_launch_layer_norm_planes.argtypes = [voidp] + [voidp] * 4 + [i, i, i, C.c_long, C.c_double]
```
